# facebookresearch/robust_cvd

Hardware: AMD Instinct MI355X
Metric: GN/LM iterations/sec (and ms/iter) on 300-frame 384x224 video, 1/2/4/8 GPU (higher is better)
Workload: dtype f64

## Files before the change

include/cvd_hip_debug.h:

```cpp
#ifndef CVD_HIP_DEBUG_H
#define CVD_HIP_DEBUG_H

#include "cvd_hip.h"

#ifdef __cplusplus
extern "C" {
#endif

typedef struct cvd_debug_options {
  uint64_t struct_size;
  int32_t force_iterations;
  int32_t force_sharded_path;
  int32_t pcg_lockstep;
  int32_t stall_fused_tail_once;
  int32_t tail_no_row_staging;
} cvd_debug_options;
void cvd_debug_options_default(cvd_debug_options* o);
int32_t cvd_set_debug_options(cvd_handle* h, const cvd_debug_options* o);

int32_t cvd_set_generic_kernels(cvd_handle* h, int32_t enabled);

int32_t cvd_comm_init_local_group(cvd_handle* h, int32_t rank, int32_t world, uint64_t group_key);
int32_t cvd_comm_init_phantom(cvd_handle* h, int32_t rank, int32_t world);

int32_t cvd_block_inverse_debug(cvd_handle* h, int32_t num_blocks, int32_t block_size, const double* a, int32_t variant,
                                float* inverse, int32_t* failed);

int32_t cvd_epipolar_debug(cvd_handle* h, int32_t num_pairs, const int64_t* offsets, const float* loc, double pixel_scale,
                           double threshold_px, int32_t iterations, uint64_t seed, uint8_t* is_static_out,
                           double* fundamental_out, int32_t* best_out, int32_t* counts_out, double* hypotheses_out);
int32_t cvd_flow_masks_debug(cvd_handle* h, int32_t num_frames, int32_t height, int32_t width, int32_t channels,
                             const float* color, int32_t num_pairs, const int32_t* pair_frames, const float* flow_ab,
                             const float* flow_ba, float flow_thresh, float color_thresh, uint8_t* mask_ab, uint8_t* mask_ba,
                             int32_t* kept, float* errors, double* kernel_ms, int32_t pixels_per_thread);
int32_t cvd_dense_inverse_debug(cvd_handle* h, int32_t n, const double* a, double* inverse, int32_t* failed);
int32_t cvd_coarse_debug(cvd_handle* h, int32_t* num_unknowns, double* a_c, double* a_c_inverse, int32_t* failed);
int32_t cvd_temporal_debug(cvd_handle* h, int32_t* dims6, double* a_t, double* a_t_inverse, double* lam, int32_t* failed);
int32_t cvd_product_launch_debug(cvd_handle* h, int32_t* out6);
int32_t cvd_assembly_launch_debug(cvd_handle* h, int32_t* out6, double* cost_frame);

#ifdef __cplusplus
}
#endif
#endif
```

robust_cvd_amd/api.py:

```python
import ctypes as C
import os
import sys

from . import build as _build
from .binding import Binding
from .ctypes_types import OptParams, SolveSummary, XformDesc

_lib = None
_variant = None


class SolverOptions(C.Structure):
    _fields_ = [
        ("struct_size", C.c_uint64),
        ("pcg_relative_tolerance", C.c_double),
        ("pcg_max_iterations", C.c_int32),
        ("verbose", C.c_int32),
        ("coarse_level", C.c_int32),
        ("robust_loss", C.c_int32),
        ("dense_matrix_free", C.c_int32),
        ("block_inverse_variant", C.c_int32),
        ("coarse_dense_max_unknowns", C.c_int32),
        ("coarse_rebuild_excess", C.c_int32),
        ("coarse_update_budget", C.c_int64),
        ("coarse_dense_shift", C.c_double),
        ("constraint_order", C.c_int32),
        ("coarse_rebuild_excess_dense", C.c_int32),
        ("pcg_fused_tail", C.c_int32),
        ("coarse_dense_row_split", C.c_int32),
        ("dist_owner_update", C.c_int32),
        ("temporal_level", C.c_int32),
        ("temporal_step", C.c_int32),
        ("temporal_grid_x", C.c_int32),
        ("temporal_grid_y", C.c_int32),
        ("coarse_temporal_step", C.c_int32),
        ("coarse_over_budget", C.c_int32),
        ("coarse_temporal_min_frames", C.c_int32),
        ("temporal_weight", C.c_double),
    ]


class DebugOptions(C.Structure):
    _fields_ = [
        ("struct_size", C.c_uint64),
        ("force_iterations", C.c_int32),
        ("force_sharded_path", C.c_int32),
        ("pcg_lockstep", C.c_int32),
        ("stall_fused_tail_once", C.c_int32),
        ("tail_no_row_staging", C.c_int32),
    ]


class ConsistencyDesc(C.Structure):
    _fields_ = [
        ("struct_size", C.c_uint64),
        ("precision", C.c_int32),
        ("num_frames", C.c_int32),
        ("num_pairs", C.c_int32),
        ("height", C.c_int32),
        ("width", C.c_int32),
        ("distance_type", C.c_int32),
        ("have_warp", C.c_int32),
        ("reserved", C.c_int32),
        ("lambda_reprojection", C.c_double),
        ("lambda_disparity", C.c_double),
        ("lambda_depth_ratio", C.c_double),
        ("distance_scale", C.c_double),
        ("distance_alpha", C.c_double),
    ]


class SceneFlowDesc(C.Structure):
    _fields_ = [
        ("struct_size", C.c_uint64),
        ("precision", C.c_int32),
        ("num_frames", C.c_int32),
        ("num_pairs", C.c_int32),
        ("height", C.c_int32),
        ("width", C.c_int32),
        ("distance_type_static", C.c_int32),
        ("distance_type_smooth", C.c_int32),
        ("have_warp", C.c_int32),
        ("lambda_static", C.c_double),
        ("lambda_smooth_reprojection", C.c_double),
        ("lambda_smooth_disparity", C.c_double),
        ("lambda_smooth_depth_ratio", C.c_double),
        ("distance_scale", C.c_double),
        ("distance_alpha", C.c_double),
    ]


class SpatialDesc(C.Structure):
    _fields_ = [
        ("struct_size", C.c_uint64),
        ("precision", C.c_int32),
        ("num_frames", C.c_int32),
        ("frames_per_sample", C.c_int32),
        ("height", C.c_int32),
        ("width", C.c_int32),
        ("reserved", C.c_int32),
        ("lambda_disparity_smooth", C.c_double),
        ("sigma_color_grad", C.c_double),
        ("lambda_contrast_loss", C.c_double),
        ("contrast_thresh", C.c_double),
    ]


class ParamDesc(C.Structure):
    _fields_ = [
        ("struct_size", C.c_uint64),
        ("precision", C.c_int32),
        ("num_tensors", C.c_int32),
    ]


class ParamRecord(C.Structure):
    _fields_ = [
        ("beta1", C.c_double),
        ("beta2", C.c_double),
        ("eps", C.c_double),
        ("grad_decay", C.c_double),
        ("param_decay", C.c_double),
        ("step", C.c_double),
        ("denom_scale", C.c_double),
        ("rule", C.c_int32),
        ("reserved", C.c_int32),
    ]


class DatasetDesc(C.Structure):
    _fields_ = [
        ("struct_size", C.c_uint64),
# ... 1416 lines not shown
        with _DeviceArrays() as dev:
            dx, dw2, db2, dw4, db4 = (dev.upload(np.ascontiguousarray(v)) for v in arrays)
            do = dev.alloc(out.nbytes)
            self._check(self._fn("midas_head_device")(
                self._h, C.c_int32(B), C.c_int32(H), C.c_int32(W), C.c_int32(Cin), C.c_int32(MIDAS_HEAD_MID), dx, dw2, db2, dw4, db4,
                C.c_int32(1 if non_negative else 0), do, None))
            if _hip_runtime().hipDeviceSynchronize() != 0:
                raise RuntimeError("midas_head: the device reported an error")
            dev.download(do, out)
        return out

    def midas_decoder(self, maps, weights, biases, non_negative=True, kernel_ms=None):
        import numpy as np
        maps = [np.asarray(v) for v in maps]
        weights, biases = [np.asarray(v) for v in weights], [np.asarray(v) for v in biases]
        self._midas_f32("midas_decoder", maps + weights + biases)
        B, features, channels, heights, widths = midas_check_decoder([v.shape for v in maps], [v.shape for v in weights],
                                                                     [v.shape for v in biases])
        out = np.zeros((B, 4 * heights[0], 4 * widths[0]), np.float32)
        with _DeviceArrays() as dev:
            dm = (C.c_void_p * 4)(*[dev.upload(np.ascontiguousarray(v)).value for v in maps])
            dw = (C.c_void_p * 21)(*[dev.upload(np.ascontiguousarray(v)).value for v in weights])
            db = (C.c_void_p * 17)(*[dev.upload(np.ascontiguousarray(v)).value for v in biases])
            do = dev.alloc(out.nbytes)
            args = (self._h, C.c_int32(B), C.c_int32(features), (C.c_int32 * 4)(*channels), (C.c_int32 * 4)(*heights),
                    (C.c_int32 * 4)(*widths), dm, dw, db, C.c_int32(1 if non_negative else 0), do, None)
            if kernel_ms is None:
                self._check(self._fn("midas_decoder_device")(*args))
            else:
                ms = (C.c_double * MIDAS_TIMED_SLOTS)()
                self._check(self._fn("midas_decoder_timed")(*args, ms))
                kernel_ms[:] = list(ms)
            if _hip_runtime().hipDeviceSynchronize() != 0:
                raise RuntimeError("midas_decoder: the device reported an error")
            dev.download(do, out)
        return out

    def num_active_constraints(self):
        return int(self._lib.cvd_num_active_constraints(self._h))

    def block_inverse_debug(self, blocks, variant=0):
        import numpy as np
        a = np.ascontiguousarray(blocks, dtype=np.float64)
        n, B, B2 = a.shape
        assert B == B2
        out = np.zeros((n, B, B), dtype=np.float32)
        fl = C.c_int32(0)
        self._check(self._fn("block_inverse_debug")(self._h, C.c_int32(n), C.c_int32(B), a.ctypes.data_as(C.POINTER(C.c_double)),
                                                    C.c_int32(variant), out.ctypes.data_as(C.POINTER(C.c_float)), C.byref(fl)))
        return out, fl.value

    def dense_inverse_debug(self, a):
        import numpy as np
        a = np.ascontiguousarray(a, dtype=np.float64)
        n = a.shape[0]
        assert a.shape == (n, n)
        out = np.zeros((n, n), dtype=np.float64)
        fl = C.c_int32(0)
        self._check(self._fn("dense_inverse_debug")(self._h, C.c_int32(n), a.ctypes.data_as(C.POINTER(C.c_double)),
                                                    out.ctypes.data_as(C.POINTER(C.c_double)), C.byref(fl)))
        return out, fl.value

    def temporal_debug(self):
        import numpy as np
        dims = (C.c_int32 * 6)()
        self._check(self._fn("temporal_debug")(self._h, dims, None, None, None, None))
        if dims[0] == 0:
            return None
        n = dims[0]
        a = np.zeros((n, n))
        ai = np.zeros((n, n))
        lam = np.zeros(self.num_frames * self.block_size())
        fl = C.c_int32(0)
        dp = lambda x: x.ctypes.data_as(C.POINTER(C.c_double))
        self._check(self._fn("temporal_debug")(self._h, dims, dp(a), dp(ai), dp(lam), C.byref(fl)))
        return {"NT": n, "S": dims[1], "nn": dims[2], "step": dims[3], "Sx": dims[4], "Sy": dims[5], "a_t": a, "a_t_inverse": ai,
                "lam": lam, "failed": fl.value}

    def path_info(self):
        out = (C.c_int32 * 8)()
        self._check(self._fn("path_info")(self._h, out))
        form = {-1: "none", 0: "exact sparse factor", 1: "exact dense inverse", 2: "temporal pose level"}[out[1]]
        return {"pose_graph_level": form, "depth_grid_level": bool(out[2]), "fused_tail": bool(out[3] & 1), "tail_rows_staged": bool(out[3] & 2),
                "tail_disabled": bool(out[4]),
                "taps": out[5], "work_items": out[6], "cross_blocks": bool(out[7])}

    def product_launch_debug(self):
        out = (C.c_int32 * 6)()
        self._check(self._fn("product_launch_debug")(self._h, out))
        kind = {-1: "none", 0: "generic list", 1: "fast list", 2: "fast dense", 3: "cross blocks"}[out[3]]
        return {"threads": out[0], "spec": out[1], "kd": out[2], "kind": out[3], "kind_name": kind, "work_items": out[4],
                "num_cu": out[5]}

    def assembly_launch_debug(self):
        import numpy as np
        out = (C.c_int32 * 6)()
        cost = np.zeros(self.num_frames, dtype=np.float64)
        self._check(self._fn("assembly_launch_debug")(self._h, out, cost.ctypes.data_as(C.POINTER(C.c_double))))
        kind = {-1: "none", 0: "generic", 1: "fast list", 2: "fast dense", 3: "dense fold"}[out[3]]
        return {"threads": out[0], "spec": out[1], "kd": out[2], "kind": out[3], "kind_name": kind, "workgroups": out[4],
                "split_parts": out[5], "cost_frame": cost}

    def coarse_debug(self):
        import numpy as np
        n = C.c_int32(0)
        self._check(self._fn("coarse_debug")(self._h, C.byref(n), None, None, None))
        if n.value == 0:
            return None
        a = np.zeros((n.value, n.value))
        ai = np.zeros((n.value, n.value))
        fl = C.c_int32(0)
        self._check(self._fn("coarse_debug")(self._h, C.byref(n), a.ctypes.data_as(C.POINTER(C.c_double)),
                                             ai.ctypes.data_as(C.POINTER(C.c_double)), C.byref(fl)))
        return {"a_c": a, "a_c_inverse": ai, "failed": fl.value}
```

robust_cvd_amd/csrc/cvd_api.hip:

```cpp
#include "cvd_host.h"
#include "cvd_coarse.h"

namespace cvd {

static void poseOptimizationStep(cvd_handle* h, const cvd_opt_params& p, double depthDeformReg) {
  solve(h, p, depthDeformReg, PK_POSE_STEP);
  paramsToPoses(h, p);
}

static void poseOptimization(cvd_handle* h, const cvd_opt_params& p) {
  posesToParams(h);
  h->records.clear();
  int ctfRows = p.ctf_long, ctfCols = p.ctf_short;
  int dsoRows = p.dso_long, dsoCols = p.dso_short;
  if (h->aspect >= 1.f) {
    std::swap(ctfCols, ctfRows);
    std::swap(dsoCols, dsoRows);
  }
  int initGrid[3] = {1, 1, 1};
  if (h->ddesc.depth_type == CVD_DEPTH_GRID)
    for (int i = 0; i < 3; ++i) initGrid[i] = h->ddesc.grid_size[i];
  const int Nval = (h->ddesc.depth_type == CVD_DEPTH_IDENTITY) ? 0 : valueNumParams(h->ddesc.value_xform);
  size_t nDmax = static_cast<size_t>(h->nD());
  if (p.coarse_to_fine && h->ddesc.depth_type != CVD_DEPTH_IDENTITY && p.num_steps > 1)
// ... 172 lines not shown
  p->depth_deform_reg_initial = 1.0;
  p->depth_deform_reg_final = 0.1;
  p->spatial_deform_reg = 1.0;
  p->focal_reg = 1.0;
  p->coarse_to_fine = 1;
  p->ctf_long = 17;
  p->ctf_short = 10;
  p->dso_long = 4;
  p->dso_short = 3;
  p->focal_long = 0.3461538376301239;
  p->intr_opt = CVD_INTR_PER_FRAME;
  p->normalize_depth_from_first_frame = 1;
}

void cvd_solver_options_default(cvd_solver_options* o) {
  o->struct_size = CVD_STRUCT_STAMP(cvd_solver_options);
  o->pcg_relative_tolerance = 1e-3;
  o->pcg_max_iterations = 300;
  o->verbose = 0;
  o->coarse_level = 1;
  o->robust_loss = 0;
  o->dense_matrix_free = 0;
  o->block_inverse_variant = 0;
  o->coarse_dense_max_unknowns = 4096;
  o->coarse_rebuild_excess = 16;
  o->coarse_update_budget = 40000;
  o->coarse_dense_shift = 1e-5;
  o->constraint_order = 1;
  o->coarse_rebuild_excess_dense = 0;
  o->pcg_fused_tail = 1;
  o->coarse_dense_row_split = 5;
  o->dist_owner_update = 1;
  o->temporal_level = 1;
  o->temporal_step = 32;
  o->temporal_grid_x = 0;
  o->temporal_grid_y = 0;
  o->coarse_temporal_step = 8;
  o->coarse_over_budget = 0;
  o->coarse_temporal_min_frames = 128;
  o->temporal_weight = 0.7;
}
int32_t cvd_set_solver_options(cvd_handle* h, const cvd_solver_options* o) {
  CVD_TRY(h, {
    if (o->struct_size != CVD_STRUCT_STAMP(cvd_solver_options))
      throw std::runtime_error(fmt("cvd_solver_options: struct_size %#llx != %#llx = sizeof | revision << 32 (caller built against "
                                   "another cvd_hip.h; start from cvd_solver_options_default)",
                                   static_cast<unsigned long long>(o->struct_size),
                                   static_cast<unsigned long long>(CVD_STRUCT_STAMP(cvd_solver_options))));
    if (o->pcg_fused_tail < 0 || o->pcg_fused_tail > 1) throw std::runtime_error("pcg_fused_tail in {0, 1}");
    if (!(o->pcg_relative_tolerance > 0.0 && o->pcg_relative_tolerance < 1.0)) throw std::runtime_error("pcg_relative_tolerance must lie in (0, 1)");
    if (o->pcg_max_iterations < 1) throw std::runtime_error("pcg_max_iterations must be >= 1");
    if (!(o->coarse_dense_shift >= 0.0 && o->coarse_dense_shift < 1.0)) throw std::runtime_error("coarse_dense_shift must lie in [0, 1)");
    if (o->coarse_rebuild_excess < 0 || o->coarse_rebuild_excess_dense < -1 || o->coarse_update_budget < 0)
      throw std::runtime_error("coarse_rebuild_excess / coarse_update_budget must be >= 0, coarse_rebuild_excess_dense >= -1");
    if (o->coarse_dense_max_unknowns < 0 || o->coarse_dense_max_unknowns > kDenseCoarseMaxUnknowns)
      throw std::runtime_error(fmt("coarse_dense_max_unknowns must lie in [0, %d] (what k_dense_spd_inverse holds in registers)",
                                   kDenseCoarseMaxUnknowns));
    if (o->coarse_level < 0 || o->coarse_level > 3 || o->coarse_temporal_step < 2 || o->robust_loss < 0 || o->robust_loss > 1 || o->block_inverse_variant < 0 ||
        o->block_inverse_variant > 2)
      throw std::runtime_error("coarse_level in {0, 1, 2, 3}, coarse_temporal_step >= 2, robust_loss in {0, 1}, block_inverse_variant in {0, 1, 2}");
    if (o->coarse_over_budget < 0 || o->coarse_over_budget > 1) throw std::runtime_error("coarse_over_budget in {0, 1}");
    if (o->coarse_temporal_min_frames < 0) throw std::runtime_error("coarse_temporal_min_frames must be >= 0");
    if (!(o->temporal_weight > 0.0 && o->temporal_weight <= 2.0)) throw std::runtime_error("temporal_weight must lie in (0, 2]");
    if (o->coarse_dense_row_split < 0 || o->coarse_dense_row_split > 8) throw std::runtime_error("coarse_dense_row_split must lie in [0, 8]");
    if (o->temporal_level < 0 || o->temporal_level > 2 || o->temporal_step < 2 || o->temporal_grid_x < 0 || o->temporal_grid_y < 0 ||
        o->temporal_grid_x == 1 || o->temporal_grid_y == 1)
      throw std::runtime_error("temporal_level in {0, 1, 2}, temporal_step >= 2, temporal_grid_x / _y 0 (automatic) or >= 2");
    if (o->coarse_update_budget != h->opt.coarse_update_budget || o->coarse_dense_max_unknowns != h->opt.coarse_dense_max_unknowns ||
        (o->coarse_level == 3) != (h->opt.coarse_level == 3) || o->coarse_temporal_step != h->opt.coarse_temporal_step ||
        o->coarse_over_budget != h->opt.coarse_over_budget || o->coarse_temporal_min_frames != h->opt.coarse_temporal_min_frames ||
        o->pcg_fused_tail != h->opt.pcg_fused_tail)
      h->tableValid = false;
    if (o->constraint_order != h->opt.constraint_order) h->orderGx = h->orderGy = -1;
    h->opt = *o;
  });
}
void cvd_debug_options_default(cvd_debug_options* o) {
  o->struct_size = CVD_STRUCT_STAMP(cvd_debug_options);
  o->force_iterations = 0;
  o->force_sharded_path = 0;
  o->pcg_lockstep = 0;
  o->stall_fused_tail_once = 0;
  o->tail_no_row_staging = 0;
}
int32_t cvd_set_debug_options(cvd_handle* h, const cvd_debug_options* o) {
  CVD_TRY(h, {
    if (o->struct_size != CVD_STRUCT_STAMP(cvd_debug_options))
      throw std::runtime_error("cvd_debug_options: struct_size does not match this library's cvd_hip_debug.h (start from cvd_debug_options_default)");
    h->dbg = *o;
    h->distForced = h->world == 1 && (h->comm != nullptr || h->localGroup || h->phantom) && o->force_sharded_path != 0;
  });
}
void cvd_comm_unique_id(uint8_t* out128) {
  ncclUniqueId id;
  std::memset(&id, 0, sizeof(id));
  (void)ncclGetUniqueId(&id);
  std::memcpy(out128, &id, sizeof(id));
}
int32_t cvd_comm_init(cvd_handle* h, int32_t rank, int32_t world, const uint8_t* id128) {
  CVD_TRY(h, {
    if (world < 1 || rank < 0 || rank >= world) throw std::runtime_error("invalid rank / world size");
    if (h->comm) { NCCL_CHECK(ncclCommDestroy(h->comm)); h->comm = nullptr; }
    ncclUniqueId id;
    std::memcpy(&id, id128, sizeof(id));
    NCCL_CHECK(ncclCommInitRank(&h->comm, world, id, rank));
    h->rank = rank;
    h->world = world;
    h->localGroup.reset();
    h->distForced = world == 1 && h->dbg.force_sharded_path != 0;
    h->tableValid = false;
  });
}
int32_t cvd_comm_init_local_group(cvd_handle* h, int32_t rank, int32_t world, uint64_t group_key) {
  CVD_TRY(h, {
    if (world < 1 || rank < 0 || rank >= world) throw std::runtime_error("invalid rank / world size");
    if (h->comm) { NCCL_CHECK(ncclCommDestroy(h->comm)); h->comm = nullptr; }
    h->localGroup = joinLocalGroup(group_key, world);
    h->rank = rank;
    h->world = world;
    h->distForced = world == 1 && h->dbg.force_sharded_path != 0;
    h->tableValid = false;
  });
}
int32_t cvd_comm_init_phantom(cvd_handle* h, int32_t rank, int32_t world) {
  CVD_TRY(h, {
    if (world < 1 || rank < 0 || rank >= world) throw std::runtime_error("invalid rank / world size");
    if (h->comm) { NCCL_CHECK(ncclCommDestroy(h->comm)); h->comm = nullptr; }
    if (h->localGroup) { leaveLocalGroup(*h->localGroup); h->localGroup.reset(); }
    h->phantom = true;
    h->rank = rank;
    h->world = world;
    h->distForced = world == 1;
    h->tableValid = false;
  });
}
int32_t cvd_set_generic_kernels(cvd_handle* h, int32_t enabled) { CVD_TRY(h, h->forceGeneric = enabled != 0); }

int32_t cvd_set_video(cvd_handle* h, int32_t numFrames, int32_t width, int32_t height, float aspect, float invAspect) {
  CVD_TRY(h, {
    if (numFrames <= 0 || width <= 0 || height <= 0) throw std::runtime_error("invalid video dimensions");
    h->F = numFrames; h->W = width; h->H = height; h->aspect = aspect; h->invAspect = invAspect;
    h->haveDynMasks = false;
    h->adaptGx = h->adaptGy = 0;
    h->dDepth.ensure(static_cast<size_t>(numFrames) * width * height);
    HIP_CHECK(hipMemsetAsync(h->dDepth.p, 0, static_cast<size_t>(numFrames) * width * height * sizeof(float), h->stream));
    h->median.assign(numFrames, 0.f);
    h->medianDirty = true;
    h->poses.assign(numFrames, cvd_frame_pose{{0, 0, 0}, {0, 0, 0, 1}, 0.f, 0.f});
    h->poseParamsValid = false;
    cvd_xform_desc dd{};
    dd.type = CVD_XFORM_DEPTH;
    dd.depth_type = CVD_DEPTH_IDENTITY;
    cvd_xform_desc sd{};
    sd.type = CVD_XFORM_SPATIAL;
    sd.spatial_type = CVD_SPATIAL_IDENTITY;
    resetXforms(h, dd, false);
    resetXforms(h, sd, true);
    h->tableValid = false;
    h->P = 0;
    h->C = 0;
    h->dense = false;
    h->denseListValid = false;
    h->haveTriplets = false;
    h->tripCenter.clear();
    h->tripOff.clear();
    h->tripC = 0;
// ... 596 lines not shown
    if (num_blocks <= 0 || block_size <= 0 || block_size > kMaxFrameBlock) throw std::runtime_error("block_inverse_debug: bad sizes");
    if (variant < 0 || variant > 2) throw std::runtime_error("block_inverse_debug: variant must be 0, 1 or 2");
    const size_t n = static_cast<size_t>(num_blocks) * block_size * block_size;
    DevBuf<double> dA;
    DevBuf<double> dL;
    DevBuf<float> dM;
    DevBuf<int> dF;
    dA.ensure(n);
    dL.ensure(static_cast<size_t>(num_blocks) * block_size);
    dM.ensure(n);
    dF.ensure(1);
    hipStream_t s = h->stream;
    dA.upload(a, n, s);
    HIP_CHECK(hipMemsetAsync(dL.p, 0, static_cast<size_t>(num_blocks) * block_size * sizeof(double), s));
    HIP_CHECK(hipMemsetAsync(dM.p, 0, n * sizeof(float), s));
    HIP_CHECK(hipMemsetAsync(dF.p, 0, sizeof(int), s));
    Layout L{};
    L.F = num_blocks;
    L.B = block_size;
    launchBlockInverseRaw(h, L, dA.p, dL.p, dM.p, dF.p, variant);
    int fl = 0;
    dM.download(inverse, n, s);
    dF.download(&fl, 1, s);
    HIP_CHECK(hipStreamSynchronize(s));
    if (failed) *failed = fl;
  });
}

int32_t cvd_epipolar_debug(cvd_handle* h, int32_t num_pairs, const int64_t* offsets, const float* loc, double pixel_scale,
                           double threshold_px, int32_t iterations, uint64_t seed, uint8_t* is_static_out,
                           double* fundamental_out, int32_t* best_out, int32_t* counts_out, double* hypotheses_out) {
  CVD_TRY(h, epipolarStaticFlags(h, num_pairs, offsets, loc, pixel_scale, threshold_px, iterations, seed, is_static_out,
                                 fundamental_out, best_out, nullptr, counts_out, hypotheses_out));
}

int32_t cvd_dense_inverse_debug(cvd_handle* h, int32_t n, const double* a, double* inverse, int32_t* failed) {
  CVD_TRY(h, {
    if (n <= 0 || n > 8192) throw std::runtime_error("dense_inverse_debug: bad size");
    const size_t nn = static_cast<size_t>(n) * n;
    DevBuf<double> dA;
    DevBuf<double> dM;
    DevBuf<int> dF;
    dA.ensure(nn);
    dM.ensure(nn);
    dF.ensure(2);
    hipStream_t s = h->stream;
    dA.upload(a, nn, s);
    HIP_CHECK(hipMemsetAsync(dM.p, 0, nn * sizeof(double), s));
    HIP_CHECK(hipMemsetAsync(dF.p, 0, 2 * sizeof(int), s));
    launchDenseSpdInverse(h, n, dA.p, dM.p, dF.p, s, dF.p + 1);
    int fl[2] = {0, 0};
    dM.download(inverse, nn, s);
    dF.download(fl, 2, s);
    HIP_CHECK(hipStreamSynchronize(s));
    if (failed) *failed = fl[0];
  });
}

int32_t cvd_temporal_debug(cvd_handle* h, int32_t* dims6, double* a_t, double* a_t_inverse, double* lam, int32_t* failed) {
  CVD_TRY(h, {
    auto& T = h->temporal;
    hipStream_t s = h->stream;
    const bool on = T.on && T.built;
    const int dims[6] = {on ? T.NT : 0, T.S, T.nn, T.step, T.Sx, T.Sy};
    for (int i = 0; i < 6; ++i) dims6[i] = dims[i];
    if (on) {
      const size_t n2 = static_cast<size_t>(T.NT) * T.NT;
      if (a_t) T.A.download(a_t, n2, s);
      if (a_t_inverse) T.Ainv.download(a_t_inverse, n2, s);
      if (lam) h->dLam.download(lam, static_cast<size_t>(h->F) * h->Bsz(), s);
      int fl = 0;
      T.fail.download(&fl, 1, s);
      HIP_CHECK(hipStreamSynchronize(s));
      if (failed) *failed = fl;
    }
  });
}
int32_t cvd_path_info(cvd_handle* h, int32_t* out8) {
  CVD_TRY(h, {
    out8[0] = h->coarseOn ? 1 : 0;
    out8[1] = !h->coarseOn ? -1 : (h->coarse.temporalPose ? 2 : (h->coarse.denseMode ? 1 : 0));
    out8[2] = h->temporal.on ? 1 : 0;
    out8[3] = h->lastFusedTail ? (h->tailStageRows ? 3 : 1) : 0;
    out8[4] = h->tailDisabled ? 1 : 0;
    out8[5] = h->lastKD;
    out8[6] = static_cast<int32_t>(h->itemFa.size());
    out8[7] = h->lastCross ? 1 : 0;
  });
}
int32_t cvd_product_launch_debug(cvd_handle* h, int32_t* out6) {
  CVD_TRY(h, {
    for (int i = 0; i < 6; ++i) out6[i] = h->lastProduct[i];
  });
}
int32_t cvd_assembly_launch_debug(cvd_handle* h, int32_t* out6, double* cost_frame) {
  CVD_TRY(h, {
    for (int i = 0; i < 6; ++i) out6[i] = h->lastAssembly[i];
    const size_t F = static_cast<size_t>(h->F);
    if (cost_frame && h->lastAssembly[3] >= 0 && h->dCostFrame.n >= F) {
      h->dCostFrame.download(cost_frame, F, h->stream);
      HIP_CHECK(hipStreamSynchronize(h->stream));
    }
  });
}
int32_t cvd_coarse_debug(cvd_handle* h, int32_t* num_unknowns, double* a_c, double* a_c_inverse, int32_t* failed) {
  CVD_TRY(h, {
    auto& C = h->coarse;
    if (!C.valid || !h->coarseOn) {
      *num_unknowns = 0;
    } else if (C.temporalPose) {
      const size_t n = static_cast<size_t>(C.ptN);
      *num_unknowns = static_cast<int32_t>(n);
      hipStream_t s = h->stream;
      int fl = 0;
      C.fail.download(&fl, 1, s);
      if (a_c) C.ptMat.download(a_c, n * n, s);
      if (a_c_inverse) C.ptInv.download(a_c_inverse, n * n, s);
      HIP_CHECK(hipStreamSynchronize(s));
      if (failed) *failed = fl;
    } else {
      const int F = h->F;
      const size_t n = static_cast<size_t>(F) * kCB;
      *num_unknowns = static_cast<int32_t>(n);
      hipStream_t s = h->stream;
      int fl = 0;
      C.fail.download(&fl, 1, s);
      if (a_c_inverse) {
        std::vector<double> save(n), unit(n, 0.0);
        C.rc.download(save.data(), n, s);
        HIP_CHECK(hipStreamSynchronize(s));
        DevBuf<double> scalTmp;
        scalTmp.ensure(S_COUNT);
        HIP_CHECK(hipMemsetAsync(scalTmp.p, 0, S_COUNT * sizeof(double), s));
        for (size_t k = 0; k < n; ++k) {
          unit[k] = 1.0;
          C.rc.upload(unit.data(), n, s);
          if (C.denseMode) {
            hipLaunchKernelGGL(k_coarse_dense_apply, dim3(F), dim3(256), 0, s, F, C.denseInv.p, C.rc.p, C.c.p, C.modeActive.p,
                               C.dotPart.p, scalTmp.p, h->dCounters.p + 3, C.fail.p, 1, 0.0, static_cast<double*>(nullptr));
          } else {
            hipLaunchKernelGGL(k_coarse_apply_w, dim3(F), dim3(1024), 0, s, C.plan, C.Wb.p, C.rc.p, C.y.p, C.dotPart.p,
                               scalTmp.p, h->dCounters.p + 3, C.fail.p, 1, 0.0, static_cast<double*>(nullptr));
            hipLaunchKernelGGL(k_coarse_apply_wt, dim3(F), dim3(256), 0, s, coarseView(h, true, true), F, C.c.p,
                               scalTmp.p, 1);
          }
          C.c.download(a_c_inverse + k * n, n, s);
          HIP_CHECK(hipStreamSynchronize(s));
          unit[k] = 0.0;
        }
        C.rc.upload(save.data(), n, s);
        HIP_CHECK(hipStreamSynchronize(s));
      }
      std::vector<double> diag(static_cast<size_t>(F) * kCBB), edges(static_cast<size_t>(std::max(C.nEdges, 1)) * kCBB);
      std::vector<unsigned char> act(n);
      std::vector<int> efa(C.nEdges), efb(C.nEdges);
      C.diag.download(diag.data(), diag.size(), s);
      C.edges.download(edges.data(), static_cast<size_t>(C.nEdges) * kCBB, s);
      C.modeActive.download(act.data(), n, s);
      C.edgeFa.download(efa.data(), efa.size(), s);
      C.edgeFb.download(efb.data(), efb.size(), s);
      HIP_CHECK(hipStreamSynchronize(s));
      if (failed) *failed = fl;
      if (a_c) {
        std::fill(a_c, a_c + n * n, 0.0);
        for (int f = 0; f < F; ++f)
          for (int i = 0; i < kCB; ++i)
// ... 16 lines not shown
```

robust_cvd_amd/csrc/cvd_host.h:

```cpp
#pragma once

#include <hip/hip_runtime.h>
#include <hip/hip_ext.h>
#include <rccl/rccl.h>
#include <rocblas/rocblas.h>
#include <rocsolver/rocsolver.h>

#include <algorithm>
#include <array>
#include <atomic>
#include <chrono>
#include <condition_variable>
#include <cmath>
#include <cstdarg>
#include <cstdint>
#include <cstdio>
#include <cstdlib>
#include <cstring>
#include <functional>
#include <limits>
#include <map>
#include <memory>
#include <mutex>
#include <set>
// ... 242 lines not shown
  DevBuf<double> dStatPart;
  DevBuf<unsigned char> dDynMask;
  DevBuf<double> dAdaptW;
  int dynW = 0, dynH = 0, adaptGx = 0, adaptGy = 0;
  bool haveDynMasks = false;
  std::shared_ptr<Frontend> frontend;

  struct CoarseHost {
    bool valid = false;
    int nEdges = 0, nBlocks = 0, nLevels = 0;
    std::vector<int> itemEdge;
    DevBuf<int> order, pos, levelPtr, levelCols, lvlBlkPtr, lvlBlks, blkCol, blkRow, colPtr, rowPtr, rowBlk, updPtr, updBlk,
        updA, updB, edgeBlk, edgeFa, edgeFb, wPtr, wRow, wtPtr, wtBlk, wtCol, wtFrame, wuPtr, wuL, wuW, itemEdgeDev, wSlot;
    DevBuf<double> edges, diag, Lb, Linv, Wb, rc, qc, y, c, dotPart, fdotY, wq, dropDiag;
    bool sparsified = false;
    bool temporalPose = false;
    int ptNn = 0, ptStepFrames = 0, ptN = 0, ptBlocks = 0;
    std::vector<int> edgeFaHost, edgeFbHost;
    DevBuf<int> ptA, ptB, ptPtr, ptList;
    DevBuf<double> ptMat, ptInv, ptR, ptT, ptDot, ptRec;
    DevBuf<TlStep> ptStepDev;
    std::vector<unsigned char> ptStepHost;
    DevBuf<unsigned int> ptCounter;
    bool denseMode = false;
    int denseForB = 0;
    bool denseReady = false;
    DevBuf<double> denseA, densePanel;
    DevBuf<double> denseInv;
    DevBuf<int> denseValid;
    int nW = 0;
    DevBuf<unsigned char> modeActive;
    DevBuf<int> fail;
    DevBuf<unsigned int> barrier;
    bool ptInvPending = false;
    int* ptInvFail = nullptr;
    DevBuf<double> Wb2;
    DevBuf<int> fail2;
    CoarsePlan plan{};
  } coarse;
  bool coarseOn = false;
  struct TemporalHost {
    bool on = false;
    bool built = false;
    int S = 0, Sx = 0, Sy = 0, nn = 0, step = 0, NT = 0, width = 0, nGroups = 0, nBlocks = 0;
    std::vector<unsigned char> stepHost;
    int tabGx = 0, tabGy = 0, tabSx = 0, tabSy = 0;
    int grpF = 0, grpStep = 0;
    std::vector<int> grpFa, grpFb;
    DevBuf<float> hx, hy, elW;
    DevBuf<int> bx, by, gOff, gItems, blkA, blkB, gPtr, gather, fail, valid;
    DevBuf<float4> vW;
    DevBuf<unsigned int> vIdx, counter;
    DevBuf<unsigned char> elV;
    DevBuf<double> Cf, E, part, A, Ainv, sq, rT, t, tl, dotPart, rec;
    DevBuf<double> invPanel;
    DevBuf<unsigned int> invBarrier;
    DevBuf<TlStep> stepDev;
    hipEvent_t evIn = nullptr, evDone = nullptr;
    bool sidePending = false;
    double* sqPtr = nullptr;
  } temporal;
  hipEvent_t evRebuild[2] = {nullptr, nullptr};
  bool rebuildTimed = false;
  double coarseRebuildMs = 0.0, pcgIterMs = 0.0;
  std::vector<std::pair<int, int>> globalEdges;
  bool haveGlobalEdges = false;
  DevBuf<double> dRegJac;
  DevBuf<unsigned short> dRegCol;
  DevBuf<unsigned char> dRegCnt;
  RegCache regCache{};
  DevBuf<FrameConst> dFc;
  DevBuf<int> dFail;
  DevBuf<unsigned long long> dCount;
  double* hScal = nullptr;
  double* hStage[2] = {nullptr, nullptr};
  size_t hStageN[2] = {0, 0};
  double* hPcg = nullptr;
  hipEvent_t pcgEvent[2] = {nullptr, nullptr};

  cvd_solve_summary summary{};
  std::vector<cvd_iteration_record> records;

  bool lastFusedTail = false, lastCross = false;
  bool tailStageRows = false;
  int lastKD = 0;
  int lastProduct[6] = {0, 0, 0, -1, 0, 0};
  int lastAssembly[6] = {0, 0, 0, -1, 0, 0};
  bool tailDisabled = false;
  bool forceGeneric = false;

  int timing = 0;
  int timingStride = 1;
  long long timingCounter = 0;
  long long timingCounterKc[16] = {0};
  std::vector<std::pair<hipEvent_t, hipEvent_t>> evPool;
  std::vector<int> evClass;
  std::vector<int> evIter;
  int curPcgIter = -1;
  size_t evUsed = 0;
  double kcMs[KC_TOTAL] = {0};
  long long kcN[KC_TOTAL] = {0};

  ~cvd_handle_t() {
    for (auto& e : evPool) { (void)hipEventDestroy(e.first); (void)hipEventDestroy(e.second); }
    if (rbMain) (void)rocblas_destroy_handle(rbMain);
    if (comm) (void)ncclCommDestroy(comm);
    if (localGroup) leaveLocalGroup(*localGroup);
    if (hScal) (void)hipHostFree(hScal);
    for (auto& p : hStage) if (p) (void)hipHostFree(p);
    if (hPcg) (void)hipHostFree(hPcg);
    for (auto& e : pcgEvent) if (e) (void)hipEventDestroy(e);
    for (auto& e : evRebuild) if (e) (void)hipEventDestroy(e);
    if (temporal.evIn) (void)hipEventDestroy(temporal.evIn);
    if (temporal.evDone) (void)hipEventDestroy(temporal.evDone);
    if (evCoarseIn) (void)hipEventDestroy(evCoarseIn);
    if (evCoarseDone) (void)hipEventDestroy(evCoarseDone);
    if (evInvIn) (void)hipEventDestroy(evInvIn);
    if (evInvDone) (void)hipEventDestroy(evInvDone);
    if (stream3) (void)hipStreamDestroy(stream3);
    if (stream2) (void)hipStreamDestroy(stream2);
    if (stream) (void)hipStreamDestroy(stream);
  }

  int nD() const { return xformNumBlocks(ddesc) * xformBlockSize(ddesc); }
  int nS() const { return xformNumBlocks(sdesc) * xformBlockSize(sdesc); }
  int Bsz() const { return 7 + nD() + nS(); }

  int tBegin(int kc) {
    if (kc >= KC_COUNT ? timing == 0 : !(timing & (1 << kc))) return -1;
    if (timingStride > 1 && kc < KC_DENSE_WALK && (timingCounterKc[kc]++ % timingStride) != 0) return -1;
    if (evUsed == evPool.size()) {
      hipEvent_t a, b;
      HIP_CHECK(hipEventCreate(&a));
      HIP_CHECK(hipEventCreate(&b));
      evPool.emplace_back(a, b);
      evClass.push_back(kc);
      evIter.push_back(-1);
    }
    evClass[evUsed] = kc;
    evIter[evUsed] = curPcgIter;
    HIP_CHECK(hipEventRecord(evPool[evUsed].first, stream));
    return static_cast<int>(evUsed++);
  }
  void tEnd(int slot) {
    if (slot >= 0) HIP_CHECK(hipEventRecord(evPool[slot].second, stream));
  }
  int tReserve(int kc, hipEvent_t& start, hipEvent_t& stop) {
    start = nullptr;
    stop = nullptr;
    if (!(timing & (1 << kc))) return -1;
    if (timingStride > 1 && (timingCounter++ % timingStride) != 0) return -1;
    if (evUsed == evPool.size()) {
      hipEvent_t a, b;
      HIP_CHECK(hipEventCreate(&a));
      HIP_CHECK(hipEventCreate(&b));
      evPool.emplace_back(a, b);
      evClass.push_back(kc);
      evIter.push_back(-1);
    }
    evClass[evUsed] = kc;
    evIter[evUsed] = curPcgIter;
    start = evPool[evUsed].first;
    stop = evPool[evUsed].second;
    return static_cast<int>(evUsed++);
  }
  void tDropFrom(size_t firstSlot, int firstDeadIter) {
// ... 91 lines not shown
    } catch (...) {
      sl.m.unlock();
      throw;
    }
  }
  ~PersistentGate() {
    sl.recorded = hipEventRecord(sl.ev, s) == hipSuccess;
    sl.m.unlock();
  }
};

void commAllReduce(cvd_handle* h, void* buf, size_t count, CommType t, hipStream_t s);
void commReduceScatter(cvd_handle* h, const void* send, void* recv, size_t recvCount, CommType t, hipStream_t s);
void commAllGather(cvd_handle* h, const void* send, void* recv, size_t sendCount, CommType t, hipStream_t s);
void commGroupStart(cvd_handle* h);
void commGroupEnd(cvd_handle* h);
std::vector<int> rangeOf(const cvd_opt_params& p, int F);
void posesToParams(cvd_handle* h);
void paramsToPoses(cvd_handle* h, const cvd_opt_params& params);
void resetXforms(cvd_handle* h, const cvd_xform_desc& d, bool spatial);
void gridXformSplit(cvd_handle* h, const cvd_xform_desc& nd);
Layout makeLayout(cvd_handle* h, const cvd_opt_params& p, double depthDeformReg, ProblemKind kind);
void checkFrameBlock(size_t B, const char* what);
void tapCounts(const Layout& L, int& KD, int& KS);
bool fastLoss(const Layout& L);
Table makeTable(cvd_handle* h);
void checkDenseScope(cvd_handle* h, const Layout& L, int KS, bool trip);
bool denseFastScope(const cvd_handle* h, const Layout& L, int KS, bool trip);
bool denseFastBlockFits(long long B);
struct DenseListScope {
  cvd_handle* h;
  bool entered = false;
  DenseListScope(cvd_handle* h, bool needList);
  ~DenseListScope();
};
bool denseModeSupported(const cvd_opt_params& p, const cvd_xform_desc& dd, const cvd_xform_desc& sd, bool haveTriplets, int world,
                        bool normalize);
AsmPanels makePanels(int B, size_t capDoubles, int& panelCap);
void compileTable(cvd_handle* h, const std::vector<int>& range, bool withTriplets = false, bool ignoreStatic = false);
void orderTable(cvd_handle* h, const Layout& L, int KD);
double* pinnedStage(cvd_handle* h, int which, size_t n);
void uploadState(cvd_handle* h, const Layout& L, DevBuf<double>& dst);
void downloadState(cvd_handle* h, const Layout& L, const DevBuf<double>& src);
void buildMask(cvd_handle* h, const Layout& L, const cvd_opt_params& p, ProblemKind kind, const std::vector<int>& range);
void ensureBuffers(Ctx& c);
void refreshMedians(cvd_handle* h);
void launchFrameConsts(const Layout& L, const double* x, FrameConst* fc, hipStream_t s);
void launchFrameConsts(Ctx& c, const double* x);
void launchFlagToBool(int* flag, hipStream_t s);
void launchTlRowsInit(cvd_handle* h, const TlStep* tsp, int NT, int groups, int F, unsigned int* counter, int closeScalars, double tol2,
                      hipStream_t s);
void spinStream(hipStream_t s);
void spinEvent(hipEvent_t ev);
void readScalars(Ctx& c);
void enqueueCost(Ctx& c, const double* x);
double evalCost(Ctx& c, const double* x);
void enqueueStats(Ctx& c);
bool crossScope(cvd_handle* h, const Ctx& c);
CrossPairs crossPairs(cvd_handle* h);
void launchCrossAssemble(Ctx& c, const double* x);
double evalFull(Ctx& c, const double* x, bool withStats = false, bool noReadBack = false);
bool coarseFusedConsumers();
bool fusedExchange(cvd_handle* h, bool withCoarse);
size_t exchangeOffsetQc(const Ctx& c);
size_t exchangeOffsetPq(const Ctx& c, bool withDenseCoarse);
size_t exchangeTemporalCount(cvd_handle* h, bool withCoarse);
bool ownerShardedUpdate(cvd_handle* h, bool withCoarse);
inline int denseRowSplit(const cvd_handle* h) { return std::min(kCB, std::max(0, h->opt.coarse_dense_row_split)); }
void launchDenseSpdInverse(cvd_handle* h, int n, const double* A, double* out, int* fail, hipStream_t s, int* outValid,
                           DevBuf<double>* panelBuf = nullptr, DevBuf<unsigned int>* barrierBuf = nullptr);
struct DinvRequest {
  int n = 0;
  const double* A = nullptr;
  double* out = nullptr;
  int* fail = nullptr;
  int* outValid = nullptr;
  DevBuf<double>* panelBuf = nullptr;
  DevBuf<unsigned int>* barrierBuf = nullptr;
};
void launchDenseSpdInversePair(cvd_handle* h, const DinvRequest& a, const DinvRequest& b, hipStream_t s);
CoarseView coarseView(cvd_handle* h, bool on, bool walk);
void prepareMatvec(Ctx& c, const double* x);
void launchMatvec(Ctx& c, const double* x, const double* z, const double* pOld, double* pNew, int useBeta, const double* lam,
                  double* q, bool withCoarse = false, bool tailFused = false);
bool pcgTailScope(Ctx& c, bool coarse, int nThreads, size_t& lds, int& ldsFinish, int& ldsScratch);
void launchPcgTail(Ctx& c, const double* x, const double* pOld, double* pNew, int useBeta, const double* lam, double* q,
                   bool withCoarse, int nThreads, size_t lds, int ldsFinish, int ldsScratch, double tol2);
void launchBlockInverseRaw(cvd_handle* h, const Layout& L, const double* dH, const double* dLam, float* dMinv, int* dFail, int variant,
                           hipStream_t onStream = nullptr);
void launchBlockInverse(Ctx& c, hipStream_t onStream = nullptr);
void launchCoarseSetup(Ctx& c, const double* x, int side = 0);
bool temporalScope(const Ctx& c);
bool temporalPrepare(Ctx& c);
void launchTemporalSetup(Ctx& c, const double* x, int half);
void launchTemporalInit(Ctx& c, bool closeScalars, double tol2);
TlStep temporalStep(cvd_handle* h);
const TlStep* temporalStepDev(cvd_handle* h);
void poseTemporalPlan(cvd_handle* h);
void poseTemporalPrepare(Ctx& c);
void launchPoseTemporalBuild(Ctx& c, hipStream_t s, int* failOut, bool deferInverse = false);
void launchPoseTemporalInit(Ctx& c, double tol2);
const TlStep* poseTemporalStepDev(cvd_handle* h);
void coarseDebug(cvd_handle* h, int32_t* num_unknowns, double* a_c, double* a_c_inverse, int32_t* failed);
int runPcg(Ctx& c, const double* x, const std::function<void()>& tail = nullptr);
bool wantsTriplets(const cvd_opt_params& p, ProblemKind kind);
void bindTriplets(Ctx& c, const cvd_opt_params& p, ProblemKind kind);
void solve(cvd_handle* h, const cvd_opt_params& p, double depthDeformReg, ProblemKind kind);
void evaluate(cvd_handle* h, const cvd_opt_params& p, double depthDeformReg, const double* pose7, double* cost, int32_t* nres,
              double* gradient, double* hdiag, double* hfull);
void sampleConstraints(cvd_handle* h, bool triplet, int num, const int32_t* keyFrames, const float* corner, const float* flow,
                       const uint8_t* mask, const float* flow2, const uint8_t* mask2, const float* dyn, int dw, int dh,
                       int matchSeparation, float minDynamicDistance, int64_t* offsets);
void getSampledConstraints(cvd_handle* h, bool triplet, float* out);
void denseMaps(cvd_handle* h, int kind, int first, int count, int w, int hh, void* out, double* kernelMs);
void imageOps(cvd_handle* h, int kind, int n, int w, int hh, const void* in, float* out, double* kernelMs);
void touchModule_setup();
void touchModule_eval();
void touchModule_matvec();
void touchModule_precond();
void touchModule_solve();
void touchModule_frontend();
void touchModule_temporal();
void flowGuidedFilter(cvd_handle* h, int n, int first, int count, int w, int hh, int dw, int dh, float invAspect, const float* depth,
                      const float* cameras, const float* flowF, const uint8_t* maskF, const float* flowB, const uint8_t* maskB,
                      int frameRadius, int spatialRadius, int median, float* out, double* kernelMs);
void bilateralFilter(cvd_handle* h, int n, int first, int count, int w, int hh, const float* depth, const float* color,
                     int frameRadius, int spatialRadius, float depthSigma, float colorSigma, int median, float* out,
                     double* kernelMs);
void epipolarStaticFlags(cvd_handle* h, int numPairs, const int64_t* offsets, const float* loc, double pixelScale,
                         double thresholdPx, int iterations, uint64_t seed, uint8_t* isStatic, double* fundamental,
                         int32_t* best, double* kernelMs, int32_t* counts, double* hypotheses);
void computeTracks(cvd_handle* h, int F, int H, int W, float invAspect, const uint8_t* active, int first, int last,
                   const float* corner, const float* dyn, int dh, int dw, const float* flow, const uint8_t* mask,
                   const uint8_t* pairPresent, int spawnDistance, int pruneDistance, float minDynamicDistance,
                   int minTrackLength, int64_t* counts, double* kernelMs);
void getTracks(cvd_handle* h, int32_t* startFrame, int32_t* length, uint8_t* kept, float* loc);
void flowConsistencyMasks(cvd_handle* h, int numFrames, int hh, int w, int channels, const float* color, int numPairs,
                          const int32_t* pairFrames, const float* flowAB, const float* flowBA, float flowThresh,
                          float colorThresh, uint8_t* maskAB, uint8_t* maskBA, int32_t* kept, float* errors, double* kernelMs,
                          int pixelsPerThread);
void consistencyLoss(cvd_handle* h, const cvd_consistency_desc* d, const void* depth, const void* ext, const void* intr,
                     const void* warp, const int32_t* pairFrames, const void* flowAB, const void* flowBA, const void* weightAB,
                     const void* weightBA, double* total, double* terms, void* grad, double* kernelMs);
void consistencyLossDevice(cvd_handle* h, const cvd_consistency_desc* d, const void* depth, const void* ext, const void* intr,
                           const void* warp, const int32_t* pairFrames, const void* flowAB, const void* flowBA,
                           const void* weightAB, const void* weightBA, double* total, double* terms, void* grad, hipStream_t s);
void sceneFlowLoss(cvd_handle* h, const cvd_scene_flow_desc* d, const void* depth, const void* ext, const void* intr,
                   const void* warp, const int32_t* pairFrames, const void* const* flows, const void* const* masks,
                   const int32_t* neighborFrames, const void* const* nflows, const void* const* nmasks, const void* valid,
                   double* total, double* terms, void* grad, void* maps, double* kernelMs);
void sceneFlowLossDevice(cvd_handle* h, const cvd_scene_flow_desc* d, const void* depth, const void* ext, const void* intr,
                         const void* warp, const int32_t* pairFrames, const void* const* flows, const void* const* masks,
                         const int32_t* neighborFrames, const void* const* nflows, const void* const* nmasks, const void* valid,
                         double* total, double* terms, void* grad, void* maps, hipStream_t s);
void spatialLosses(cvd_handle* h, const cvd_spatial_desc* d, const void* depth, const void* depthOrig, const void* image,
                   double* total, double* smooth, double* contrast, void* grad, double* kernelMs);
void spatialLossesDevice(cvd_handle* h, const cvd_spatial_desc* d, const void* depth, const void* depthOrig, const void* image,
                         double* total, double* smooth, double* contrast, void* grad, hipStream_t s);
void parameterL1(cvd_handle* h, const cvd_param_desc* d, const int64_t* offsets, const int64_t* counts, int64_t flatCount,
                 const void* p, const void* p0, double lambda, double* total, void* grad, double gradOut, int accumulate,
                 double* kernelMs);
void parameterL1Device(cvd_handle* h, const cvd_param_desc* d, const void* const* p, const void* const* p0, const int64_t* counts,
                       double lambda, double* total, void* const* grad, const void* gradOut, int accumulate, hipStream_t s);
void paramStep(cvd_handle* h, const cvd_param_desc* d, const int64_t* offsets, const int64_t* counts, int64_t flatCount, void* p,
               const void* g, void* m, void* v, const cvd_param_record* records, double* kernelMs);
void paramStepDevice(cvd_handle* h, const cvd_param_desc* d, void* const* p, const void* const* g, void* const* m, void* const* v,
                     const int64_t* counts, const cvd_param_record* records, hipStream_t s);
long long paramChunkElements();
void datasetCreate(cvd_handle* h, const cvd_dataset_desc* d, const int32_t* pairFrames, const int32_t* samples);
void datasetClear(cvd_handle* h);
// ... 44 lines not shown
```

robust_cvd_amd/csrc/cvd_kernels.h:

```cpp
#pragma once

#include "cvd_device.h"

namespace cvd {

struct Table {
  const float4* ndc;
  const float2* dsrc;
  const int* pairA;
  const int* pairB;
  const long long* pairOff;
  const float2* flow;
  const unsigned char* fmask;
  const float* depth;
  int W, H;
  float sx, sy, invAspect;
};

__device__ __forceinline__ int densePixelOfLoc(const Table& T, float lx, float ly) {
  int px = static_cast<int>(__fmul_rn(lx, static_cast<float>(T.W)));
  int py = static_cast<int>(__fmul_rn(__fdiv_rn(ly, T.invAspect), static_cast<float>(T.H)));
  px = min(max(px, 0), T.W - 1);
  py = min(max(py, 0), T.H - 1);
  return py * T.W + px;
// ... 95 lines not shown
  bool candCur;
  __device__ __forceinline__ bool request(const Table& T, int pix, int fa, int fb, float2 f, float4& n, float2& d) const {
    return denseConstraintRequest(T, pix, fa, fb, f, n, d);
  }
  __device__ __forceinline__ void prime(const Table& T, long long base, int i, int step, int n, long long pixBase, int fa, int fb) {
    unsigned int m0 = 0u;
    float2 f0 = make_float2(0.f, 0.f);
    fNext = make_float2(0.f, 0.f);
    mNext = 0u;
    if (i < n) { m0 = (T.fmask + base)[i]; f0 = (T.flow + base)[i]; }
    if (i + step < n) { mNext = (T.fmask + base)[i + step]; fNext = (T.flow + base)[i + step]; }
    ndCur = make_float4(0.f, 0.f, 0.f, 0.f);
    candCur = m0 != 0u && request(T, static_cast<int>(base - pixBase) + i, fa, fb, f0, ndCur, dCur);
  }
  __device__ __forceinline__ bool take(const Table& T, long long base, int i, int step, int n, long long pixBase, int fa, int fb,
                                       float4& nd, float2& d) {
    nd = ndCur;
    d = dCur;
    const bool cand = candCur;
    const unsigned int m1 = mNext;
    const float2 f1 = fNext;
    mNext = 0u;
    if (i + 2 * step < n) { mNext = (T.fmask + base)[i + 2 * step]; fNext = (T.flow + base)[i + 2 * step]; }
    candCur = m1 != 0u && request(T, static_cast<int>(base - pixBase) + i + step, fa, fb, f1, ndCur, dCur);
    return cand && denseDepthsValid(d);
  }
};

struct alignas(64) ItemRecord {
  int fa, fb;
  int slotA, slotB;
  long long b0, e0;
  long long b1, e1;
  long long pad[2];
};
static_assert(sizeof(ItemRecord) == 64, "one record per 64-byte line");
struct Items {
  const int* fa;
  const int* fb;
  const long long* range;
  const int* slot;
  int count;
  const ItemRecord* rec;
};

constexpr int kDenseFramesPerGroup = 2;
constexpr int kAsmUnit = 128;
constexpr int kAsmUnitDense = 1024;
constexpr int kDenseRun = 16;

#ifndef CVD_DETERMINISTIC
#define CVD_DETERMINISTIC 0
#endif
constexpr int kAtomicWalkers256 = CVD_DETERMINISTIC ? 64 : 256;
constexpr int kAsmThreads = CVD_DETERMINISTIC ? 64 : 512;
struct AsmPart {
  int frame;
  int u0, u1;
  int part;
  int nParts;
  int slot0;
};
struct AsmWork {
  const AsmPart* parts;
  const int2* units;
  double* scratch;
  unsigned int* counters;
};

__host__ __device__ inline int dwRecordDoubles(int G) { return 256 + 40 * G + 8; }
struct DenseRecords {
  const double* records;
  const int* recOff;
  const int* fpOff;
  const int* fpList;
};

enum : int { S_RZ = 0, S_RZOLD = 1, S_BETA = 2, S_PQ = 3, S_ALPHA = 4, S_RR = 5, S_RZ0 = 6, S_COST = 7,
             S_DG = 8, S_DR = 9, S_DLD = 10, S_DD = 11, S_XX = 12, S_NVALID = 13, S_GMAX = 14,
             S_DONE = 15, S_TARGET = 16, S_ITERS = 17,
             S_RZPART = 18,
             S_NACTIVE = 19,
             S_COUNT = 20 };

__device__ __forceinline__ double blockSumArray(const double* __restrict__ a, int n, double* red) {
  double acc = 0.0;
  for (int i = threadIdx.x; i < n; i += blockDim.x) acc += a[i];
  acc = waveSum(acc);
  __syncthreads();
  if ((threadIdx.x & 63) == 0) red[threadIdx.x >> 6] = acc;
  __syncthreads();
  double t = 0.0;
  for (int w = 0; w < (blockDim.x >> 6); ++w) t += red[w];
  __syncthreads();
  return t;
}

__device__ __forceinline__ bool lastBlockArrives(unsigned int* counter, unsigned int total, int* flag) {
  __syncthreads();
  if (threadIdx.x == 0) {
    __builtin_amdgcn_fence(__ATOMIC_RELEASE, "agent");
    asm volatile("s_waitcnt vmcnt(0)" ::: "memory");
    const unsigned int t = __hip_atomic_fetch_add(counter, 1u, __ATOMIC_RELAXED, __HIP_MEMORY_SCOPE_AGENT);
    const bool last = (t == total - 1);
    if (last) {
      __builtin_amdgcn_fence(__ATOMIC_ACQUIRE, "agent");
      __hip_atomic_store(counter, 0u, __ATOMIC_RELAXED, __HIP_MEMORY_SCOPE_AGENT);
    }
    *flag = last ? 1 : 0;
  }
  __syncthreads();
  return *flag != 0;
}

#if defined(__HIP_DEVICE_COMPILE__) && !defined(__gfx950__) && !defined(__gfx942__)
#error "the fence-free inter-workgroup hand-off (publishPartial / readPartial / lastBlockArrivesLite) is written for gfx942 / gfx950"
#endif
__device__ __forceinline__ void publishPartial(double* p, double v) {
  __hip_atomic_store(reinterpret_cast<unsigned long long*>(p), static_cast<unsigned long long>(__double_as_longlong(v)),
                     __ATOMIC_RELAXED, __HIP_MEMORY_SCOPE_AGENT);
}
__device__ __forceinline__ double readPartial(const double* p) {
  return __longlong_as_double(static_cast<long long>(__hip_atomic_load(
      reinterpret_cast<const unsigned long long*>(p), __ATOMIC_RELAXED, __HIP_MEMORY_SCOPE_AGENT)));
}
__device__ __forceinline__ bool lastBlockArrivesLite(unsigned int* counter, unsigned int total, int* flag) {
  asm volatile("s_waitcnt vmcnt(0)" ::: "memory");
  __syncthreads();
  if (threadIdx.x == 0) {
    const unsigned int t = __hip_atomic_fetch_add(counter, 1u, __ATOMIC_RELAXED, __HIP_MEMORY_SCOPE_AGENT);
    const bool last = (t == total - 1);
    if (last) __hip_atomic_store(counter, 0u, __ATOMIC_RELAXED, __HIP_MEMORY_SCOPE_AGENT);
    *flag = last ? 1 : 0;
  }
  __syncthreads();
  return *flag != 0;
}
__device__ __forceinline__ double blockSumPartials(const double* __restrict__ a, int n, double* red) {
  double acc = 0.0;
  for (int i = threadIdx.x; i < n; i += blockDim.x) acc += readPartial(a + i);
  acc = waveSum(acc);
  __syncthreads();
  if ((threadIdx.x & 63) == 0) red[threadIdx.x >> 6] = acc;
  __syncthreads();
  double t = 0.0;
  for (int w = 0; w < (blockDim.x >> 6); ++w) t += red[w];
  __syncthreads();
  return t;
}

constexpr size_t kCoarseMaxUnknowns = 65536;
constexpr int kCBB = kCB * kCB;
struct CoarsePlan {
  int F, nBlocks, nLevels, nEdges;
  const int* order;
  const int* pos;
  const int* levelPtr;
  const int* levelCols;
  const int* lvlBlkPtr;
  const int* lvlBlks;
  const int* blkCol;
  const int* blkRow;
  const int* colPtr;
  const int* rowPtr;
  const int* rowBlk;
  const int* updPtr;
// ... 298 lines not shown
                                        double (&Rca)[3]) {
  ca[0] = pax * fxa;
  ca[1] = pay * fya;
  ca[2] = -1.0;
  Rca[0] = dot3(Ra, ca);
  Rca[1] = dot3(Ra + 3, ca);
  Rca[2] = dot3(Ra + 6, ca);
}

template <bool FAST>
__device__ __forceinline__ void fastProject(const Layout& L, const double* Rb, const double (&v)[3], double ifxb, double ifyb,
                                            double pbx, double pby, double& zz, double& iz, double& u, double& vv, double& r0,
                                            double& r1) {
  const double q0 = Rb[0] * v[0] + Rb[3] * v[1] + Rb[6] * v[2];
  const double q1 = Rb[1] * v[0] + Rb[4] * v[1] + Rb[7] * v[2];
  const double q2 = Rb[2] * v[0] + Rb[5] * v[1] + Rb[8] * v[2];
  zz = -q2;
  iz = fastRcp<FAST>(zz);
  u = q0 * iz * ifxb;
  vv = q1 * iz * ifyb;
  r0 = (u - pbx) * L.ws;
  r1 = (vv - pby) * L.ws;
}

template <bool FAST>
__device__ __forceinline__ void fastDepthResidual(const Layout& L, int lossType, double zz, double iz, double Db, double& r2,
                                                  double& dr2dA, double& dr2dDb) {
  constexpr double eps = 1e-6;
  if (lossType == kLossDisparity) {
    const bool zo = !(zz < eps), bo = !(Db < eps);
    const double bc = bo ? Db : eps;
    const double izc = zo ? iz : 1.0 / eps, ibc = fastRcp<FAST>(bc);
    r2 = (izc - ibc) * L.wd;
    dr2dA = zo ? (-L.wd * izc * izc) : 0.0;
    dr2dDb = bo ? (L.wd * ibc * ibc) : 0.0;
  } else {
    const bool zIsMax = !(zz < Db), zIsMin = !(Db < zz);
    const double mx = zIsMax ? zz : Db, mn = zIsMin ? zz : Db;
    if (lossType == kLossRatio) {
      r2 = (mx / mn - 1.0) * L.wd;
      const double dmx = 1.0 / mn, dmn = -mx / (mn * mn);
      dr2dA = ((zIsMax ? dmx : 0.0) + (zIsMin ? dmn : 0.0)) * L.wd;
      dr2dDb = ((zIsMax ? 0.0 : dmx) + (zIsMin ? 0.0 : dmn)) * L.wd;
    } else {
      r2 = log(mn / mx) * L.wd;
      const double dmn = 1.0 / mn, dmx = -1.0 / mx;
      dr2dA = ((zIsMax ? dmx : 0.0) + (zIsMin ? dmn : 0.0)) * L.wd;
      dr2dDb = ((zIsMax ? 0.0 : dmx) + (zIsMin ? 0.0 : dmn)) * L.wd;
    }
  }
}

template <int SPEC>
__device__ __forceinline__ double fastRobustRho1(const Layout& L, double sq) {
  if constexpr (SPEC == 1) return rcpFast(1.0 + sq * L.cauchyC);
  else if constexpr (SPEC == 2) {
    const bool outer = sq > L.cauchyB;
    const double irt = rsqrtFast(outer ? sq : 1.0);
    return outer ? fmax(2.2250738585072014e-308, L.robustA * irt) : 1.0;
  }
  else return robustRho1(L, sq);
}
template <int SPEC>
__device__ __forceinline__ double fastRobustRho0(const Layout& L, double sq) {
  static_assert(SPEC == 1 || SPEC == 2, "the runtime choice goes through robustRho");
  if constexpr (SPEC == 1) {
    return L.cauchyB * log(1.0 + sq * L.cauchyC);
  } else {
    const bool outer = sq > L.cauchyB;
    const double irt = rsqrtFast(outer ? sq : 1.0);
    return outer ? (2.0 * L.robustA * (sq * irt) - L.cauchyB) : sq;
  }
}

__device__ __forceinline__ void fastRows(const Layout& L, double iz, double u, double vv, double ifxb, double ifyb, double& m00,
                                         double& m11, double& m02, double& m12) {
  const double wiz = L.ws * iz;
  m00 = wiz * ifxb;
  m11 = wiz * ifyb;
  m02 = wiz * u;
  m12 = wiz * vv;
}

#ifdef CVD_MV_PROFILE
__device__ unsigned long long g_mvProf[4096 * 8];
#define MV_STAMP(slot) do { if ((threadIdx.x & 63) == 0) g_mvProf[(blockIdx.x & 4095) * 8 + (slot)] = wall_clock64(); } while (0)
#else
#define MV_STAMP(slot) do {} while (0)
#endif
constexpr int kRedVals = 15;
constexpr int kRedStride = 4 * 33 + 1;

#ifndef CVD_MV_WAVES
#define CVD_MV_WAVES 4
#endif
#ifndef CVD_MV_EARLY
#define CVD_MV_EARLY 1
#endif
template <int KD, int NT, int SPEC = 0, bool DENSE = false>
inline __global__ __launch_bounds__(NT) __attribute__((amdgpu_waves_per_eu(SPEC ? ((KD <= 4 && !DENSE) ? CVD_MV_WAVES : 3) : 2))) void k_matvec_pairs_fast(Layout L, Table T, Items it, const double* __restrict__ x,
                                                           const FrameConst* __restrict__ fc,
                                                           const double* __restrict__ mask,
                                                           const double* __restrict__ z, const double* __restrict__ pOld,
                                                           const double* __restrict__ scal, int useBeta,
                                                           double* __restrict__ qPart, CoarseView V) {
  const double sDone = scal[S_DONE];
  extern __shared__ __attribute__((aligned(16))) double sm[];
  constexpr int NV = KD == 1 ? kRedVals : 11;
  const int B = L.B;
  if (threadIdx.x == 0) MV_STAMP(0);
  double* xa = sm;
  double* xb = xa + B;
  double* pa = xb + B;
  double* pb = pa + B;
  double* qa = pb + B;
  double* qb = qa + B;
  double* fix = qb + B;
  double* red = fix + 2 * sizeof(FrameConst) / 8;
  double* W = red + 32;
  constexpr int kPriv = DENSE ? 8 : 1;
  constexpr bool kUsePriv = kPriv > 1;
  double* qpriv = W + static_cast<size_t>(kRedVals) * kRedStride;
  double* cl = W;
  const int item = blockIdx.x;
  const int tid = threadIdx.x;
  const ItemRecord* __restrict__ recp = it.rec + item;
  const int fa = recp->fa, fb = recp->fb;
  const int slotA = recp->slotA, slotB = recp->slotB;
  const long long cbD[2] = {recp->b0, recp->b1}, ceD[2] = {recp->e0, recp->e1};
  const double beta = useBeta ? scal[S_BETA] : 0.0;
  const FrameConst* __restrict__ fcF[2] = {fc + fa, fc + fb};
  constexpr bool kEarlyPrime = KD <= 4 && CVD_MV_EARLY;
  RecordStream<DENSE> rs;
  if constexpr (kEarlyPrime) rs.primeClamped(T, cbD[0], tid, static_cast<int>(ceD[0] - cbD[0]));
  constexpr int EPT = 256 / NT;
  constexpr int TLE = (2 * kTlMaxS + NT - 1) / NT;
  const bool fusedCoarse = V.Wb != nullptr;
  const bool tlOn = V.tl != nullptr;
  const size_t rowA = static_cast<size_t>(fa) * B, rowB = static_cast<size_t>(fb) * B;
  double vcf;
  {
    const int k = tid & (2 * kCB - 1);
    vcf = *(V.cF != nullptr ? V.cF + static_cast<size_t>(k < kCB ? fa : fb) * kCB + (k & (kCB - 1)) : x);
  }
  double* tls = cl + 2 * kCB;
  double vtl[TLE];
#pragma unroll
  for (int e = 0; e < TLE; ++e) {
    const int i = tid + e * NT;
    const int ic = (tlOn && i < 2 * V.tlS) ? i : 0;
    const int which = ic >= V.tlS ? 1 : 0;
    vtl[e] = *(tlOn ? V.tl + static_cast<size_t>(which ? fb : fa) * V.tlS + (ic - which * V.tlS) : x);
  }
  TlTaps tt[EPT];
#pragma unroll
  for (int e = 0; e < EPT; ++e) {
    const int i = tid + e * NT;
    const bool in = i >= 7 && i < 7 + L.nD;
    const int v = in ? i - 7 : 0;
    tt[e].w = *(tlOn ? V.tlW + v : reinterpret_cast<const float4*>(x));
    tt[e].idx = *(tlOn ? V.tlIdx + v : reinterpret_cast<const unsigned int*>(x));
    if (!in) tt[e].w = make_float4(0.f, 0.f, 0.f, 0.f);
  }
  constexpr int kFix = 13;
  static_assert(offsetof(FrameConst, fy) == offsetof(FrameConst, t) + 24 && offsetof(FrameConst, Jl) == offsetof(FrameConst, t) + 32,
                "t, fy, Jl are consecutive");
  const int fixK = NT - 1 - tid;
  double vfix;
  {
    const int k = fixK < 2 * kFix ? fixK : 0;
    vfix = (reinterpret_cast<const double*>(fc + (k >= kFix ? fb : fa)) + offsetof(FrameConst, t) / 8)[k >= kFix ? k - kFix : k];
  }
  double vxa[EPT], vxb[EPT], vza[EPT], vzb[EPT], vpa[EPT], vpb[EPT], vma[EPT], vmb[EPT];
  const double* __restrict__ pOldOrZ = useBeta ? pOld : z;
#pragma unroll
  for (int e = 0; e < EPT; ++e) {
    const int i = tid + e * NT;
    const size_t ia = rowA + (i < B ? i : 0), ib = rowB + (i < B ? i : 0);
    vxa[e] = x[ia];
    vxb[e] = x[ib];
    vza[e] = z[ia];
    vzb[e] = z[ib];
    vpa[e] = pOldOrZ[ia];
    vpb[e] = pOldOrZ[ib];
    vma[e] = mask[ia];
    vmb[e] = mask[ib];
  }
  const double z6 = z[6], po6 = pOldOrZ[6], m6 = mask[6];
  if (fusedCoarse) {
    if (tid < 64) coarseFrameCorrection(V, fa, tid, cl);
    if (NT == 64) coarseFrameCorrection(V, fb, tid, cl + kCB);
    else if (tid >= 64 && tid < 128) coarseFrameCorrection(V, fb, tid - 64, cl + kCB);
  }
  if (!fusedCoarse && tid < 2 * kCB) cl[tid] = (V.cF != nullptr) ? vcf : 0.0;
#pragma unroll
  for (int e = 0; e < TLE; ++e) {
    const int i = tid + e * NT;
    if (tlOn && i < 2 * V.tlS) tls[i] = vtl[e];
  }
  if (fixK < 2 * kFix) fix[fixK] = vfix;
#pragma unroll
  for (int e = 0; e < EPT; ++e) {
    const int i = tid + e * NT;
    if (i < B) {
      xa[i] = vxa[e];
      xb[i] = vxb[e];
      qa[i] = 0.0;
      qb[i] = 0.0;
    }
  }
  if constexpr (kUsePriv)
    for (int i = tid; i < kPriv * 2 * B; i += NT) qpriv[i] = 0.0;
  __syncthreads();
  if (sDone != 0.0) return;
#pragma unroll
  for (int e = 0; e < EPT; ++e) {
    const int i = tid + e * NT;
    if (i < B) {
      double ca = coarseAtLds(cl, L, i), cb2 = coarseAtLds(cl + kCB, L, i);
      if (tlOn) {
        ca += tlAt(tls, tt[e]);
        cb2 += tlAt(tls + V.tlS, tt[e]);
      }
      pa[i] = (vza[e] + ca + (useBeta ? beta * vpa[e] : 0.0)) * vma[e];
      pb[i] = (vzb[e] + cb2 + (useBeta ? beta * vpb[e] : 0.0)) * vmb[e];
    }
  }
  if (L.intrOpt == kIntrShared) {
    __syncthreads();
    if (tid == 0) {
      const double p06 = (z6 + (useBeta ? beta * po6 : 0.0)) * m6;
      pa[6] = p06;
      pb[6] = p06;
    }
  }
  __syncthreads();
  if (threadIdx.x == 0) MV_STAMP(1);

  const int N = SPEC ? 1 : L.N;
  const int lossType = SPEC ? static_cast<int>(kLossDisparity) : L.lossType;
  const double A = L.aspect;
  double aT[3] = {0, 0, 0}, aT0[3] = {0, 0, 0};
  double Cx[3] = {0, 0, 0};
  double aFa = 0.0, aFb = 0.0;
  double gDa[2] = {0.0, 0.0}, gDb[2] = {0.0, 0.0};
  const long long units0 = (ceD[0] - cbD[0] + 63) >> 6;
  for (int dir = 0; dir < 2; ++dir) {
  const long long cb = cbD[dir], ce = ceD[dir];
  const FrameConst& Fa = *fcF[dir];
  const FrameConst& Fb = *fcF[dir ^ 1];
  if (dir) {
    double* t;
    t = xa; xa = xb; xb = t;
    t = pa; pa = pb; pb = t;
    t = qa; qa = qb; qb = t;
#pragma unroll
    for (int i = 0; i < 3; ++i) { aT0[i] = aT[i]; aT[i] = 0.0; Cx[i] = -Cx[i]; }
    { const double o = aFa; aFa = aFb; aFb = o; }
#pragma unroll
    for (int n = 0; n < 2; ++n) { const double o = gDa[n]; gDa[n] = gDb[n]; gDb[n] = o; }
  }
  const int firstUnit = dir == 0 ? (tid >> 6) : static_cast<int>(((tid >> 6) - units0) & (NT / 64 - 1));
  const int nDir = static_cast<int>(ce - cb);
  const int iFirst = firstUnit * 64 + (tid & 63);
  if (dir || !kEarlyPrime) rs.prime(T, cb, iFirst, nDir);
  double RaU[9], RbU[9], dTU[3];
#pragma unroll
  for (int i = 0; i < 9; ++i) { RaU[i] = uniformValue(Fa.R[i]); RbU[i] = uniformValue(Fb.R[i]); }
#pragma unroll
  for (int i = 0; i < 3; ++i) dTU[i] = uniformValue(Fa.t[i] - Fb.t[i]);
  double eaU[3], ebU[3], dptU[3];
  {
    const double pwa[3] = {uniformValue(pa[3]), uniformValue(pa[4]), uniformValue(pa[5])};
    const double pwb[3] = {uniformValue(pb[3]), uniformValue(pb[4]), uniformValue(pb[5])};
#pragma unroll
    for (int k = 0; k < 3; ++k) {
      eaU[k] = uniformValue(pwa[0] * Fa.Jl[k] + pwa[1] * Fa.Jl[3 + k] + pwa[2] * Fa.Jl[6 + k]);
      ebU[k] = uniformValue(pwb[0] * Fb.Jl[k] + pwb[1] * Fb.Jl[3 + k] + pwb[2] * Fb.Jl[6 + k]);
      dptU[k] = uniformValue(pa[k] - pb[k]);
    }
  }
  const double fya = uniformValue(Fa.fy), fxa = fya * A;
  const double fyb = uniformValue(Fb.fy);
  const double ifyb = uniformValue(1.0 / fyb), ifxb = uniformValue(1.0 / (fyb * A));
  const double pfaU = uniformValue(pa[6] / fya);
  const double pfrU = uniformValue(L.ws * pb[6] * ifyb);

  const int fsrc = dir ? fb : fa, ftgt = dir ? fa : fb;
  const long long pixBase = DENSE ? (cb / (static_cast<long long>(T.W) * T.H)) * (static_cast<long long>(T.W) * T.H) : 0;
  for (int ci = iFirst; ci < nDir; ci += NT) {
    float4 nd;
    float2 d;
    if (!rs.take(T, cb, ci, NT, nDir, pixBase, fsrc, ftgt, nd, d)) continue;
    const double da = static_cast<double>(d.x), db = static_cast<double>(d.y);
    FastTaps<KD> ta, tb;
    fastGather<KD>(L, nd.x, nd.y, ta);
    fastGather<KD>(L, nd.z, nd.w, tb);
// ... 197 lines not shown
```

robust_cvd_amd/csrc/cvd_matvec.hip:

```cpp
#include "cvd_host.h"
#include "cvd_pcg.h"
#include "cvd_cross.h"
#include "cvd_triplets.h"

namespace cvd {

bool coarseFusedConsumers() {
  return false;
}
bool fusedExchange(cvd_handle* h, bool withCoarse) { return !withCoarse || h->coarse.denseMode; }
size_t exchangeOffsetQc(const Ctx& c) { return c.h->dist() ? static_cast<size_t>(c.h->framesPadded()) * c.L.B : c.n; }
size_t exchangeOffsetPq(const Ctx& c, bool withDenseCoarse) {
  return exchangeOffsetQc(c) + (withDenseCoarse ? static_cast<size_t>(c.L.F) * kCB : 0);
}
size_t exchangeTemporalCount(cvd_handle* h, bool withCoarse) {
  const TlStep ts = temporalStep(h);
  return (ts.Ainv != nullptr && h->dist() && fusedExchange(h, withCoarse)) ? static_cast<size_t>(h->F) * ts.S : 0;
}
bool ownerShardedUpdate(cvd_handle* h, bool withCoarse) {
  return h->dist() && fusedExchange(h, withCoarse) && h->opt.dist_owner_update != 0;
}
CoarseView coarseView(cvd_handle* h, bool on, bool walk) {
  auto& C = h->coarse;
  CoarseView v = on ? CoarseView{C.pos.p, C.wPtr.p, C.wRow.p, walk ? C.Wb.p : nullptr, C.y.p, C.modeActive.p, C.fail.p, C.c.p}
                    : CoarseView{nullptr, nullptr, nullptr, nullptr, nullptr, nullptr, nullptr, nullptr};
  if (h->temporal.on && h->temporal.built) {
    v.tl = h->temporal.tl.p;
    v.tlW = h->temporal.vW.p;
    v.tlIdx = h->temporal.vIdx.p;
    v.tlS = h->temporal.S;
  }
  return v;
}

void prepareMatvec(Ctx& c, const double* x) {
  cvd_handle* h = c.h;
  const Layout& L = c.L;
  launchFrameConsts(c, x);
  int nr = 0;
  if (L.scaleRegSqrt > 0.0) nr += L.sregX * L.sregY;
  if (L.focalRegSqrt > 0.0) nr += 1;
  if (L.depthDeformW > 0.0 && L.depthType == CVD_DEPTH_GRID) nr += gridNumEdges(L.gx, L.gy, L.gz) * L.N;
  if (L.spatialDeformW > 0.0) nr += L.nS;
  const int stride = std::max(2, c.KD * std::max(1, L.N));
  const size_t entries = static_cast<size_t>(L.F) * stride * std::max(nr, 1);
  h->dRegJac.ensure(entries);
  h->dRegCol.ensure(entries);
  h->dRegCnt.ensure(static_cast<size_t>(L.F) * std::max(nr, 1));
  h->regCache = RegCache{h->dRegJac.p, h->dRegCol.p, h->dRegCnt.p, nr, stride};
  HIP_CHECK(hipMemsetAsync(h->dScal.p + S_DONE, 0, sizeof(double), h->stream));
  if (nr == 0) return;
  CVD_DISPATCH_KD(c.KD, {
    hipLaunchKernelGGL((k_reg_cache<KD>), dim3(L.F), dim3(256), static_cast<size_t>(L.B) * 8, h->stream, L, x, h->dMedian.p, h->dRegOwner.p,
                       h->regCache);
  });
  HIP_CHECK(hipGetLastError());
}

void launchMatvec(Ctx& c, const double* x, const double* z, const double* pOld, double* pNew, int useBeta,
                         const double* lam, double* q, bool withCoarse, bool tailFused) {
  cvd_handle* h = c.h;
  hipStream_t s = h->stream;
  const CoarseView cF = coarseView(h, withCoarse, coarseFusedConsumers());
  const size_t B = c.L.B;
  auto recordLaunch = [h](int threads, int spec, int kd, int kind, int items) {
    const int launched[6] = {threads, spec, kd, kind, items, h->numCU};
    std::copy(launched, launched + 6, h->lastProduct);
  };
  if (c.cross) {
    hipEvent_t evStart, evStop;
    (void)h->tReserve(KC_MATVEC_PAIRS, evStart, evStop);
    const size_t ldsX = (3 * B + (kCrossThreads / 64) * B + 2 * kCB + 2 * kTlMaxS) * 8;
    const unsigned nP = static_cast<unsigned>(h->xFa.size()) + (h->xDiagRows ? static_cast<unsigned>(c.L.F) : 0u);
    const int* diagSlot = h->xDiagRows ? h->dXDiagSlot.p : nullptr;
    recordLaunch(kCrossThreads, 0, c.KD, 3, static_cast<int>(nP));
    if (evStart)
      hipExtLaunchKernelGGL(k_cross_matvec, dim3(nP), dim3(kCrossThreads), ldsX, s, evStart, evStop, 0, c.L, crossPairs(h),
                            h->dXBlocks.p, h->dH.p, diagSlot, h->dMask.p, z, pOld, h->dScal.p, useBeta, h->dQPart.p, cF);
    else
      hipLaunchKernelGGL(k_cross_matvec, dim3(nP), dim3(kCrossThreads), ldsX, s, c.L, crossPairs(h), h->dXBlocks.p, h->dH.p, diagSlot,
                         h->dMask.p, z, pOld, h->dScal.p, useBeta, h->dQPart.p, cF);
    HIP_CHECK(hipGetLastError());
  } else if (c.L.includeStatic && c.nItems > 0) {
    const size_t lds = 6 * B * 8 + 2 * sizeof(FrameConst) + (18 + 4 * 24 + 8 + 2 * kCB) * 8;
    const size_t ldsFast = 6 * B * 8 + 2 * sizeof(FrameConst) + (32 + static_cast<size_t>(kRedVals) * kRedStride) * 8;
    hipEvent_t evStart, evStop;
    (void)h->tReserve(KC_MATVEC_PAIRS, evStart, evStop);
    const bool fast = !h->forceGeneric && c.KS == 0 && fastLoss(c.L);
    const FrameConst* fcp = h->dFc.p;
    const double* maskp = h->dMask.p;
    const double* scalp = h->dScal.p;
    if (fast) {
      const int spec = (c.L.N == 1 && c.L.lossType == CVD_STATIC_REPRO_DISPARITY) ? (c.L.robustKind == 0 ? 1 : 2) : 0;
      const int wavesPerSimd = spec ? ((c.KD <= 4) ? CVD_MV_WAVES : 3) : 2;
      const long long slots256 = static_cast<long long>(wavesPerSimd) * h->numCU;
      const long long slots128 = std::min<long long>(2 * slots256, static_cast<long long>(kMaxLds / std::max<size_t>(ldsFast, 1)) * h->numCU);
#ifndef CVD_MV_NT_RULE
#define CVD_MV_NT_RULE 1
#endif
      const int nt = CVD_MV_NT_RULE ? ((c.nItems <= slots256 || c.nItems > slots128) ? 256 : 128)
                                    : (c.nItems > 2 * h->numCU && c.nItems <= 4 * h->numCU ? 128 : 256);
#define CVD_LAUNCH_PAIRS_FAST_S(NTV, SPECV)                                                                              \
      CVD_DISPATCH_KD(c.KD, {                                                                                            \
        recordLaunch(NTV, SPECV, KD, 1, c.nItems);                                                                       \
        allowLds((k_matvec_pairs_fast<KD, NTV, SPECV>), ldsFast);                                                        \
        if (evStart)                                                                                                     \
          hipExtLaunchKernelGGL((k_matvec_pairs_fast<KD, NTV, SPECV>), dim3(c.nItems), dim3(NTV), ldsFast, s, evStart, evStop, 0, \
                                c.L, c.T, c.it, x, fcp, maskp, z, pOld, scalp, useBeta, h->dQPart.p, cF);                \
        else                                                                                                             \
          hipLaunchKernelGGL((k_matvec_pairs_fast<KD, NTV, SPECV>), dim3(c.nItems), dim3(NTV), ldsFast, s, c.L, c.T, c.it, x, \
                             fcp, maskp, z, pOld, scalp, useBeta, h->dQPart.p, cF);                                      \
      })
#define CVD_LAUNCH_PAIRS_FAST(NTV) do { if (spec == 1) CVD_LAUNCH_PAIRS_FAST_S(NTV, 1); else if (spec == 2) CVD_LAUNCH_PAIRS_FAST_S(NTV, 2); else CVD_LAUNCH_PAIRS_FAST_S(NTV, 0); } while (0)
      if (h->dense) {
        const size_t ldsDense = ldsFast + 8 * 2 * B * 8;
#define CVD_LAUNCH_PAIRS_DENSE(SPECV)                                                                                     \
        CVD_DISPATCH_KD(c.KD, {                                                                                          \
          if constexpr (KD <= 4) {                                          \
            recordLaunch(256, SPECV, KD, 2, c.nItems);                                                                   \
            allowLds((k_matvec_pairs_fast<KD, 256, SPECV, true>), ldsDense);                                             \
            if (evStart)                                                                                                 \
              hipExtLaunchKernelGGL((k_matvec_pairs_fast<KD, 256, SPECV, true>), dim3(c.nItems), dim3(256), ldsDense, s, evStart, \
                                    evStop, 0, c.L, c.T, c.it, x, fcp, maskp, z, pOld, scalp, useBeta, h->dQPart.p, cF); \
            else                                                                                                         \
              hipLaunchKernelGGL((k_matvec_pairs_fast<KD, 256, SPECV, true>), dim3(c.nItems), dim3(256), ldsDense, s, c.L, c.T, \
                                 c.it, x, fcp, maskp, z, pOld, scalp, useBeta, h->dQPart.p, cF);                         \
          }                                                                                                              \
        })
        if (spec == 1) CVD_LAUNCH_PAIRS_DENSE(1);
        else if (spec == 2) CVD_LAUNCH_PAIRS_DENSE(2);
        else CVD_LAUNCH_PAIRS_DENSE(0);
#undef CVD_LAUNCH_PAIRS_DENSE
      }
#if CVD_DETERMINISTIC
      else { (void)nt; CVD_LAUNCH_PAIRS_FAST(64); }
#else
      else if (nt == 128) CVD_LAUNCH_PAIRS_FAST(128);
      else CVD_LAUNCH_PAIRS_FAST(256);
#endif
#undef CVD_LAUNCH_PAIRS_FAST_S
#undef CVD_LAUNCH_PAIRS_FAST
    } else {
      recordLaunch(256, 0, c.KD, 0, c.nItems);
      CVD_DISPATCH(c.KD, c.KS, {
        allowLds(k_matvec_pairs<KD, KS>, lds);
        if (evStart)
          hipExtLaunchKernelGGL((k_matvec_pairs<KD, KS>), dim3(c.nItems), dim3(256), lds, s, evStart, evStop, 0, c.L, c.T,
                                c.it, x, fcp, maskp, z, pOld, scalp, useBeta, h->dQPart.p, cF);
        else
          hipLaunchKernelGGL((k_matvec_pairs<KD, KS>), dim3(c.nItems), dim3(256), lds, s, c.L, c.T, c.it, x, fcp, maskp, z,
                             pOld, scalp, useBeta, h->dQPart.p, cF);
      });
    }
    HIP_CHECK(hipGetLastError());
  }
  if (c.trip && c.TT.nGroups > 0) {
    const size_t ldsT = (9 * B + 3 * kCB) * 8;
    CVD_DISPATCH(c.KD, c.KS, {
      allowLds(k_matvec_triplets<KD, KS>, ldsT);
      hipLaunchKernelGGL((k_matvec_triplets<KD, KS>), dim3(c.TT.nGroups), dim3(256), ldsT, s, c.L, c.TT, x, h->dFc.p,
                         h->dMask.p, z, pOld, h->dScal.p, useBeta, h->dQPart.p, cF);
    });
    HIP_CHECK(hipGetLastError());
  }
  if (!tailFused) {
    if (B > 512) throw std::runtime_error("frame block larger than 512 unknowns is not supported by k_matvec_finish");
    const TlStep ts = temporalStep(h);
    const size_t lds = 3 * B * 8 + (8 + kCB) * 8 + (ts.Ainv != nullptr ? (kTlMaxS + static_cast<size_t>(ts.S) * ts.width) * 8 : 0);
    const bool fusedCoarse = withCoarse && !h->coarse.denseMode;
    const bool denseFused = withCoarse && h->coarse.denseMode;
    const bool fusedX = h->dist() && fusedExchange(h, withCoarse);
    double* qcX = q + exchangeOffsetQc(c);
    double* pqX = q + exchangeOffsetPq(c, denseFused);
    const CoarseColumns cc{h->coarse.pos.p, h->coarse.wPtr.p, h->coarse.wSlot.p, fusedCoarse ? h->coarse.Wb.p : nullptr,
                           h->coarse.wq.p};
    const int slot = h->tBegin(KC_MATVEC_FINISH);
    CVD_DISPATCH_KD(c.KD, {
      hipLaunchKernelGGL((k_matvec_finish<KD>), dim3(c.L.F), dim3(256), lds, s, c.L, x, h->dMask.p, lam,
                         h->dMedian.p, h->dRegOwner.p, h->dInRange.p, c.cross ? h->dXFiOff.p : h->dFiOff.p, h->dFiList.p,
                         h->dQPart.p, z, pOld, pNew, h->dScal.p, h->dCounters.p, useBeta, q, h->dFdot.p,
                         h->dist() ? (h->rank == 0 ? 1 : 2) : 0, c.cross ? static_cast<int>(h->xFa.size()) * 2 : h->qRows,
                         h->regCache, cF,
                         fusedX ? (denseFused ? qcX : nullptr) : (((fusedCoarse || denseFused) && !h->dist()) ? h->coarse.qc.p : nullptr), cc,
                         c.cross ? h->dH.p : nullptr, fusedX ? pqX : nullptr, h->dist() ? h->ownFirst() : 0,
                         h->dist() ? h->ownCount() : ((c.cross && h->xDiagRows) ? 0 : c.L.F), ts.Ainv != nullptr ? temporalStepDev(h) : static_cast<const TlStep*>(nullptr));
    });
    HIP_CHECK(hipGetLastError());
    if (fusedX && ownerShardedUpdate(h, withCoarse)) {
      const int ct = h->tBegin(KC_COMM_PRODUCT);
      const size_t chunk = static_cast<size_t>(h->ownChunk()) * B;
      commGroupStart(h);
      commReduceScatter(h, q, q + static_cast<size_t>(h->rank) * chunk, chunk, CT_F64, s);
      commAllReduce(h, qcX, exchangeOffsetPq(c, denseFused) - exchangeOffsetQc(c) + 1 + exchangeTemporalCount(h, withCoarse), CT_F64, s);
      commGroupEnd(h);
      h->tEnd(ct);
    } else if (fusedX) {
      const int ct = h->tBegin(KC_COMM_PRODUCT);
      commAllReduce(h, q, exchangeOffsetPq(c, denseFused) + 1 + exchangeTemporalCount(h, withCoarse), CT_F64, s);
      h->tEnd(ct);
    } else if (h->dist()) {
      const int ct = h->tBegin(KC_COMM_PRODUCT);
      commAllReduce(h, q, c.n, CT_F64, s);
      h->tEnd(ct);
      hipLaunchKernelGGL(k_dot_pq, dim3(c.L.F), dim3(256), 0, s, c.L, pNew, q, h->dScal.p, h->dCounters.p, h->dFdot.p,
                         withCoarse ? h->coarse.qc.p : nullptr, h->coarse.modeActive.p, cc,
                         ts.Ainv != nullptr ? temporalStepDev(h) : static_cast<const TlStep*>(nullptr));
      HIP_CHECK(hipGetLastError());
    }
    h->tEnd(slot);
  }
}

bool pcgTailScope(Ctx& c, bool coarse, int nThreads, size_t& lds, int& ldsFinish, int& ldsScratch) {
  cvd_handle* h = c.h;
  const int F = c.L.F, B = c.L.B;
  h->tailStageRows = false;
  if (!h->opt.pcg_fused_tail || h->tailDisabled || h->dist() || B > 256 || h->forceGeneric) return false;
  if (coarse && !h->coarse.denseMode) return false;
  const int split = denseRowSplit(h);
  const TlStep ts = temporalStep(h);
  if (ts.Ainv != nullptr && (ts.S * ts.width > cgUpdatePartDoubles(B, nThreads) || tlRowsLds(ts.NT) > B + cgUpdatePartDoubles(B, nThreads)))
    return false;
  const bool poseT = coarse && h->coarse.temporalPose;
  if (poseT && tlRowsLds(h->coarse.ptN) > B + cgUpdatePartDoubles(B, nThreads)) return false;
  const int grid = F + (coarse && !poseT && split > 0 ? (F + kDenseFramesPerGroup - 1) / kDenseFramesPerGroup : 0) +
                   (ts.Ainv != nullptr ? ts.S * ts.parts : 0) + (poseT ? kCB * tlParts(h->coarse.ptNn) : 0);
  const int update = B + cgUpdatePartDoubles(B, nThreads) + 48 + 17 * kCB;
  const int finish = 3 * B + 8 + kCB + (nThreads / 256 - 1) * 256 + kTlMaxS;
  const int denseEnd = (coarse && !poseT) ? F * kCB + nThreads + 16 : 0;
  ldsFinish = update;
  const int unstaged = std::max(update + finish + (coarse && split < kCB ? denseEnd : 0), denseEnd);
  int stagedEnd = 0;
  if (ts.Ainv != nullptr) stagedEnd = std::max(stagedEnd, tlStagedLds(ts.NT));
  if (poseT) stagedEnd = std::max(stagedEnd, tlStagedLds(h->coarse.ptN));
  static std::map<std::tuple<int, int, int, size_t>, int> perCuCache;
  static std::mutex cacheMutex;
  auto resident = [&](size_t bytes) {
    if (bytes > kMaxLds) return false;
    int perCu = 0;
    std::lock_guard<std::mutex> lock(cacheMutex);
    const auto key = std::make_tuple(h->device, c.KD, nThreads, bytes);
    auto it = perCuCache.find(key);
    if (it == perCuCache.end()) {
      CVD_DISPATCH_KD(c.KD, {
        allowLds((k_pcg_tail<KD>), bytes);
        HIP_CHECK(hipOccupancyMaxActiveBlocksPerMultiprocessor(&perCu, reinterpret_cast<const void*>(&k_pcg_tail<KD>), nThreads, bytes));
      });
      perCuCache[key] = perCu;
    } else {
      perCu = it->second;
    }
    return static_cast<long long>(perCu) * h->numCU >= grid;
  };
  if (stagedEnd > 0 && h->dbg.tail_no_row_staging == 0) {
    ldsScratch = std::max(unstaged, stagedEnd);
    lds = static_cast<size_t>(ldsScratch + 24) * sizeof(double);
    if (resident(lds)) {
      h->tailStageRows = true;
      return true;
    }
  }
  ldsScratch = unstaged;
  lds = static_cast<size_t>(ldsScratch + 24) * sizeof(double);
  return resident(lds);
}

void launchPcgTail(Ctx& c, const double* x, const double* pOld, double* pNew, int useBeta, const double* lam, double* q,
                   bool withCoarse, int nThreads, size_t lds, int ldsFinish, int ldsScratch, double tol2) {
  cvd_handle* h = c.h;
  hipStream_t s = h->stream;
  const int F = c.L.F;
  const CoarseView cF = coarseView(h, withCoarse, false);
  const int split = denseRowSplit(h);
  const int finishDoubles = 3 * static_cast<int>(c.L.B) + 8 + kCB + (nThreads / 256 - 1) * 256 + kTlMaxS;
  const TlStep ts = temporalStep(h);
  const bool poseT = withCoarse && h->coarse.temporalPose;
  const DenseStep ds = (withCoarse && !poseT) ? DenseStep{h->coarse.denseInv.p, h->coarse.qc.p, h->coarse.rc.p, h->coarse.c.p, h->coarse.dotPart.p,
                                               h->coarse.modeActive.p, h->coarse.fail.p, split, ldsFinish + finishDoubles,
                                               h->coarse.dotPart.p + F}
                                  : DenseStep{nullptr, nullptr, nullptr, nullptr, nullptr, nullptr, nullptr, kCB, 0, nullptr};
  double* fd = h->dFdot.p;
  const TailUpdate U{h->dMinv.p, h->dDx.p, h->dR.p, h->dZ.p, fd + F, fd + 2 * F, tol2, h->coarse.modeActive.p, h->hPcg,
                     h->dCounters.p + 1, h->dTailBar.p, h->dFdot.p + 4 * static_cast<size_t>(F) + 32, ldsFinish, ldsScratch, ds,
                     ts.Ainv != nullptr ? temporalStepDev(h) : static_cast<const TlStep*>(nullptr),
                     poseT ? poseTemporalStepDev(h) : static_cast<const TlStep*>(nullptr),
                     (c.cross && h->xDiagRows) ? 1 : 0, h->tailStageRows ? 1 : 0};
  const int grid = F + (withCoarse && !poseT && split > 0 ? (F + kDenseFramesPerGroup - 1) / kDenseFramesPerGroup : 0) +
                   (ts.Ainv != nullptr ? ts.S * ts.parts : 0) + (poseT ? kCB * tlParts(h->coarse.ptNn) : 0);
  const int slot = h->tBegin(KC_CG_UPDATE);
  {
    std::unique_ptr<PersistentGate> gate;
    std::unique_lock<std::mutex> alone(PersistentGate::slot(h->device).m);
    if (liveHandles(h->device) > 1) {
      alone.unlock();
      gate.reset(new PersistentGate(h->device, s));
    }
    CVD_DISPATCH_KD(c.KD, {
      hipLaunchKernelGGL((k_pcg_tail<KD>), dim3(grid), dim3(nThreads), lds, s, c.L, x, h->dMask.p, lam, h->dMedian.p, h->dRegOwner.p,
                         h->dInRange.p, c.cross ? h->dXFiOff.p : h->dFiOff.p, h->dFiList.p, h->dQPart.p, pOld, pNew, h->dScal.p,
                         useBeta, q, fd, c.cross ? static_cast<int>(h->xFa.size()) * 2 : h->qRows, h->regCache, cF,
                         withCoarse ? h->coarse.qc.p : static_cast<double*>(nullptr),
                         c.cross ? static_cast<const double*>(h->dH.p) : static_cast<const double*>(nullptr), U);
    });
    HIP_CHECK(hipGetLastError());
  }
  h->tEnd(slot);
}

void touchModule_matvec() {
  hipFuncAttributes a;
  (void)hipFuncGetAttributes(&a, reinterpret_cast<const void*>(k_dot_pq));
}

}

#ifdef CVD_TAIL_PROFILE
extern "C" int32_t cvd_debug_tail_profile(unsigned long long* out) {
  (void)hipDeviceSynchronize();
  return hipMemcpyFromSymbol(out, HIP_SYMBOL(cvd::g_tailProf), sizeof(unsigned long long) * 1024 * 16) == hipSuccess ? 0 : 1;
}
#endif
#ifdef CVD_MV_PROFILE
extern "C" int32_t cvd_debug_mv_profile(unsigned long long* out) {
  (void)hipDeviceSynchronize();
  return hipMemcpyFromSymbol(out, HIP_SYMBOL(cvd::g_mvProf), sizeof(unsigned long long) * 4096 * 8) == hipSuccess ? 0 : 1;
}
#endif
```

robust_cvd_amd/csrc/cvd_pcg.h:

```cpp
#pragma once

#include "cvd_kernels.h"

namespace cvd {

inline __global__ void k_lm_diag(Layout L, const double* __restrict__ hdiag, double* __restrict__ scale,
                          int computeScale, double radius, double* __restrict__ lam) {
  const size_t n = static_cast<size_t>(L.F) * L.B;
  const size_t i = static_cast<size_t>(blockIdx.x) * blockDim.x + threadIdx.x;
  if (i >= n) return;
  const double h = hdiag[i];
  if (computeScale) scale[i] = 1.0 / (1.0 + sqrt(h));
  const double s = scale[i];
  if (h == 0.0) {
    lam[i] = 1.0;
  } else {
    const double d = fmin(fmax(s * s * h, 1e-6), 1e32);
    lam[i] = d / (radius * s * s);
  }
}

template <int KD>
inline __global__ __launch_bounds__(256) void k_reg_cache(Layout L, const double* __restrict__ x,
                                                   const float* __restrict__ median,
// ... 261 lines not shown
  }
  return true;
}

template <int KD>
inline __global__ __launch_bounds__(256) void k_matvec_finish(Layout L, const double* __restrict__ x,
                                                       const double* __restrict__ mask,
                                                       const double* __restrict__ lam, const float* __restrict__ median,
                                                       const unsigned char* __restrict__ inRange,
                                                       const unsigned char* __restrict__ rangeFlags,
                                                       const int* __restrict__ fiOff, const int* __restrict__ fiList,
                                                       const double* __restrict__ qPart, const double* __restrict__ z,
                                                       const double* __restrict__ pOld, double* __restrict__ pNew,
                                                       double* __restrict__ scal, unsigned int* __restrict__ counter,
                                                       int useBeta, double* __restrict__ q, double* __restrict__ fdot,
                                                       int distMode, int nRows, RegCache rc, CoarseView V,
                                                       double* __restrict__ qc, CoarseColumns cc,
                                                       const double* __restrict__ Hdiag, double* __restrict__ pqOut,
                                                       int ownFirst, int ownCount, const TlStep* __restrict__ tsp) {
  extern __shared__ __attribute__((aligned(16))) double sm[];
  TailCarry carry;
  (void)matvecFinishBody<KD, false>(L, x, mask, lam, median, inRange, rangeFlags, fiOff, fiList, qPart, z, pOld, pNew, scal, counter,
                                    useBeta, q, fdot, distMode, nRows, rc, V, qc, cc, Hdiag, pqOut, ownFirst, ownCount, sm, carry, tsp,
                                    sm + 3 * L.B + 8 + kCB + kTlMaxS);
}

inline __global__ __launch_bounds__(256) void k_dot_pq(Layout L, const double* __restrict__ p, const double* __restrict__ q,
                                                double* __restrict__ scal, unsigned int* __restrict__ counter,
                                                double* __restrict__ fdot, double* __restrict__ qc,
                                                const unsigned char* __restrict__ modeActive, CoarseColumns cc,
                                                const TlStep* __restrict__ tsp) {
  if (scal[S_DONE] != 0.0) return;
  __shared__ double red[8];
  __shared__ double prod[kTlMaxS * kTlMaxWidth];
  const int f = blockIdx.x, tid = threadIdx.x;
  const size_t base = static_cast<size_t>(f) * L.B;
  if (tsp != nullptr) {
    const TlStep ts = *tsp;
    const int nE = ts.S * ts.width;
    for (int e = tid; e < nE; e += 256) prod[e] = static_cast<double>(ts.elW[e]) * q[base + 7 + ts.elV[e]];
    __syncthreads();
    if (tid < ts.S) {
      double a = 0.0;
      for (int k = 0; k < ts.width; ++k) a += prod[k * ts.S + tid];
      ts.sq[static_cast<size_t>(f) * ts.S + tid] = a;
    }
  }
  if (qc != nullptr) {
    coarseRestrict(L, q + base, f, tid, modeActive, qc);
    __syncthreads();
    coarseColumnProducts(cc, qc + f * kCB, f, tid, 256);
  }
  double dot = 0.0;
  for (int i = tid; i < L.B; i += 256) dot += p[base + i] * q[base + i];
  dot = waveSum(dot);
  if ((tid & 63) == 0) red[tid >> 6] = dot;
  __syncthreads();
  if (tid == 0) publishPartial(fdot + f, red[0] + red[1] + red[2] + red[3]);
  if (lastBlockArrivesLite(counter, L.F, reinterpret_cast<int*>(red + 6))) {
    const double pq = blockSumPartials(fdot, L.F, red);
    if (tid == 0) {
      scal[S_PQ] = pq;
      scal[S_ALPHA] = scal[S_RZ] / pq;
    }
  }
}

__host__ __device__ inline int cgUpdatePartDoubles(int B, int nThreads) {
  return B > 256 ? nThreads : max(nThreads, 16 * ((B + 3) & ~3));
}

#ifdef CVD_TAIL_PROFILE
__device__ unsigned long long g_tailProf[1024 * 16];
#define TAIL_STAMP(slot) do { if (threadIdx.x == 0) g_tailProf[(blockIdx.x & 1023) * 16 + (slot)] = wall_clock64(); } while (0)
#else
#define TAIL_STAMP(slot) do {} while (0)
#endif

struct NoMid {
  __device__ bool first(double&, double&) { return true; }
  __device__ bool second(double&) { return true; }
  __device__ unsigned int generation() { return 0u; }
  __device__ bool stageRows() { return false; }
};
__host__ __device__ inline int tlStagedLds(int NT) { return tlRowsLds(NT) + (kTlSpan + 1) * NT; }
typedef unsigned int cvd_u32x4 __attribute__((ext_vector_type(4)));
template <bool FUSED, typename Mid>
__device__ __forceinline__ bool tlLevelRows(const TlStep* __restrict__ tsp, int wg, int F, double& alpha, int init, double sDone,
                                            const double* __restrict__ scal, double* __restrict__ sm, Mid& mid) {
  const TlStep ts = *tsp;
  const int tid = threadIdx.x, nThreads = blockDim.x;
  const int wv = tid >> 6, lane = tid & 63, nW = nThreads >> 6;
  const int s = wg / ts.parts, part = wg - s * ts.parts;
  const int aLo = part * ts.span, aHi = min(ts.nn - 1, aLo + ts.span), nA = aHi - aLo + 1;
  const bool ownsLast = part == ts.parts - 1;
  const int par = init ? 1 : (static_cast<int>(scal[S_ITERS]) & 1);
  const double* tin = ts.t + static_cast<size_t>(par) * ts.NT;
  double* tout = ts.t + static_cast<size_t>(par ^ 1) * ts.NT;
  double* qT = sm;
  double* tn = qT + ts.NT;
  double* red = tn + ts.span + 1;
  double rOldPre = 0.0, tOldPre = 0.0;
  if (lane == 0 && !init) {
    const int e = s * ts.nn + aLo + (wv < nA ? wv : 0);
    rOldPre = ts.rT[e];
    tOldPre = tin[e];
  }
  double* stage = sm + tlRowsLds(ts.NT);
  bool staged = false;
  if constexpr (FUSED) {
    staged = mid.stageRows();
    if (staged) {
      constexpr int kStageBatch = 8;
      for (int k = wv; k < nA; k += nW) {
        const double* row = ts.Ainv + static_cast<size_t>(s * ts.nn + aLo + k) * ts.ld;
        double* dst = stage + static_cast<size_t>(k) * ts.NT;
        for (int c0 = 0; c0 < ts.NT; c0 += 64 * kStageBatch) {
          double v[kStageBatch];
#pragma unroll
          for (int u = 0; u < kStageBatch; ++u) {
            const int c = c0 + u * 64 + lane;
            v[u] = row[min(c, ts.NT - 1)];
          }
#pragma unroll
          for (int u = 0; u < kStageBatch; ++u) {
            const int c = c0 + u * 64 + lane;
            if (c < ts.NT) dst[c] = v[u];
          }
        }
      }
    }
    TAIL_STAMP(8);
  }
  bool on = false;
  if constexpr (FUSED) {
    on = *ts.fail == 0;
    if (!mid.second(alpha)) return false;
  }
  const double inv = 1.0 / static_cast<double>(ts.step);
  bool direct = true;
  if constexpr (FUSED) {
    if (ts.rec != nullptr) {
      direct = false;
      const unsigned int gen = mid.generation() + 1u;
      cvd_u32x4* rec = reinterpret_cast<cvd_u32x4*>(ts.rec);
      for (int a = wv; a < ts.nn; a += nW) {
        const int f = (a - 1) * ts.step + 1 + lane;
        const bool in = lane < 2 * ts.step - 1 && f >= 0 && f < F;
        double v = in ? readPartial(ts.sq + static_cast<size_t>(f) * ts.S + s) : 0.0;
        v *= 1.0 - fabs(static_cast<double>(f - a * ts.step)) * inv;
        v = waveSum(in ? v : 0.0);
        if (lane == 0 && part == 0) {
          cvd_u32x4 r4;
          r4.x = gen;
          r4.y = static_cast<unsigned int>(__double2loint(v));
          r4.z = static_cast<unsigned int>(__double2hiint(v));
          r4.w = gen;
          *reinterpret_cast<volatile cvd_u32x4*>(rec + s * ts.nn + a) = r4;
        }
      }
      int* bad = reinterpret_cast<int*>(red + ts.span + 1);
      if (tid == 0) *bad = 0;
      __syncthreads();
      for (int e = tid; e < ts.NT; e += nThreads) {
        const volatile cvd_u32x4* src = reinterpret_cast<const volatile cvd_u32x4*>(rec + e);
        cvd_u32x4 r4;
        unsigned int spins = 0;
        for (;;) {
          r4 = *src;
          if (r4.x == gen && r4.w == gen) break;
          __builtin_amdgcn_s_sleep(4);
          if (++spins > (1u << 20)) {
            *bad = 1;
            break;
          }
        }
        qT[e] = __hiloint2double(static_cast<int>(r4.z), static_cast<int>(r4.y));
      }
      __syncthreads();
      if (*bad) return false;
    }
  }
  if (direct) {
    for (int e = tid; e < ts.NT; e += nThreads) {
      const int a = e / ts.S, sp = e - a * ts.S;
      const int fLo = max(0, (a - 1) * ts.step + 1), fHi = min(F - 1, (a + 1) * ts.step - 1);
      constexpr int kTlBatch = 8;
      double acc[4] = {0.0, 0.0, 0.0, 0.0};
      for (int f = fLo; f <= fHi; f += kTlBatch) {
        double v[kTlBatch];
#pragma unroll
        for (int u = 0; u < kTlBatch; ++u) {
          const double* src = ts.sq + static_cast<size_t>(min(f + u, fHi)) * ts.S + sp;
          v[u] = FUSED ? readPartial(src) : *src;
        }
#pragma unroll
        for (int u = 0; u < kTlBatch; ++u) {
          const double w = 1.0 - fabs(static_cast<double>(f + u - a * ts.step)) * inv;
          acc[u & 3] += (f + u <= fHi) ? w * v[u] : 0.0;
        }
      }
      qT[sp * ts.nn + a] = (acc[0] + acc[1]) + (acc[2] + acc[3]);
    }
    __syncthreads();
  }
  if (sDone != 0.0) return false;
  if constexpr (FUSED) TAIL_STAMP(5);
  if constexpr (!FUSED) on = *ts.fail == 0;
  for (int k = wv; k < nA; k += nW) {
    const int a = aLo + k, e = s * ts.nn + a;
    const double* row = ts.Ainv + static_cast<size_t>(e) * ts.ld;
    const bool owned = ownsLast || a < aHi;
    double rOld = rOldPre, tOld = tOldPre;
    double acc0 = 0.0, acc1 = 0.0;
    int c = lane;
    if (k != wv && lane == 0 && !init) {
      rOld = ts.rT[e];
      tOld = tin[e];
    }
    if (staged) {
      const double* srow = stage + static_cast<size_t>(k) * ts.NT;
      for (; c + 64 < ts.NT; c += 128) {
        acc0 += srow[c] * qT[c];
        acc1 += srow[c + 64] * qT[c + 64];
      }
      if (c < ts.NT) acc0 += srow[c] * qT[c];
    } else {
      for (; c + 64 < ts.NT; c += 128) {
        acc0 += row[c] * qT[c];
        acc1 += row[c + 64] * qT[c + 64];
      }
      if (c < ts.NT) acc0 += row[c] * qT[c];
    }
    const double d = ts.weight * waveSum(acc0 + acc1);
    if (lane == 0) {
      const double rn = init ? qT[e] : rOld - alpha * qT[e];
      const double tv = on ? (init ? d : tOld - alpha * d) : 0.0;
      if (owned) {
        ts.rT[e] = rn;
        tout[e] = tv;
      }
      tn[k] = tv;
      red[k] = owned ? tv * rn : 0.0;
    }
  }
  __syncthreads();
  if constexpr (FUSED) TAIL_STAMP(6);
  const int fLo = aLo * ts.step, fHi = ownsLast ? F : min(F, aHi * ts.step);
  for (int f = fLo + tid; f < fHi; f += nThreads) {
    const int a0 = f / ts.step, k0 = a0 - aLo;
    const double tau = static_cast<double>(f - a0 * ts.step) * inv;
    ts.tl[static_cast<size_t>(f) * ts.S + s] = (1.0 - tau) * tn[k0] + tau * tn[min(k0 + 1, nA - 1)];
  }
  if (tid == 0) {
    double d = 0.0;
    for (int k = 0; k < nA; ++k) d += red[k];
    publishPartial(ts.dotPart + wg, d);
  }
  if constexpr (FUSED) TAIL_STAMP(7);
  return true;
}

template <bool FUSED, typename Mid>
__device__ __forceinline__ void cgUpdateBody(const Layout& L, int init, const double* __restrict__ g,
                                             const float* __restrict__ minv, const double* __restrict__ p,
                                             const double* __restrict__ q, double* __restrict__ scal,
                                             unsigned int* __restrict__ counter, double* __restrict__ dx,
                                             double* __restrict__ r, double* __restrict__ z,
                                             double* __restrict__ fdotRZ, double* __restrict__ fdotRR,
                                             double tol2, double* __restrict__ rc,
                                             const unsigned char* __restrict__ modeActive,
                                             double* __restrict__ hostMirror, const CoarseStep& cs, const DenseStep& ds,
                                             const double* __restrict__ pqReduced, double* __restrict__ sm, Mid& mid,
                                             int f0, int nF, double* __restrict__ partOut, const TlStep* __restrict__ tsp,
                                             const TlStep* __restrict__ tpp) {
  const double sDone = (init || FUSED) ? 0.0 : scal[S_DONE];
  const int B = L.B;
  const int nThreads = blockDim.x;
  double* rf = sm;
  double* part = rf + B;
  double* red = part + cgUpdatePartDoubles(B, nThreads);
  double* ypart = red + 48;
  const bool fusedY = !init && cs.Wb != nullptr;
  const bool fusedDense = !init && ds.Ainv != nullptr;
  const int nWaves = nThreads >> 6;
  const int nExtraWg = static_cast<int>(gridDim.x) - nF;
  const int bid = FUSED ? static_cast<int>(blockIdx.x)
                        : (static_cast<int>(blockIdx.x) < nExtraWg ? nF + static_cast<int>(blockIdx.x) : static_cast<int>(blockIdx.x) - nExtraWg);
  const bool denseWg = bid >= nF;
  const int f = denseWg ? L.F + (bid - nF) : f0 + bid;
  const int nDenseWg = (fusedDense && ds.rowSplit > 0) ? (nF + kDenseFramesPerGroup - 1) / kDenseFramesPerGroup : 0;
  const bool tlOn = !init && tsp != nullptr, tpOn = !init && tpp != nullptr;
  const bool tlWg = (tlOn || tpOn) && bid >= nF + nDenseWg;
  const int tid = threadIdx.x;
  const size_t base = static_cast<size_t>(f) * B;
  double alpha = (init || FUSED) ? 0.0 : (pqReduced != nullptr ? scal[S_RZ] / *pqReduced : scal[S_ALPHA]);
  double pvCarry = 0.0, qvCarry = 0.0;
  if constexpr (FUSED) {
    if (!mid.first(pvCarry, qvCarry)) return;
  }
#ifndef CVD_DENSE_LOADS
#define CVD_DENSE_LOADS 4
#endif
  constexpr int kDenseLoads = CVD_DENSE_LOADS;
  const size_t nC = static_cast<size_t>(L.F) * kCB;
  const int n2 = static_cast<int>(nC / 2);
  auto denseRows = [&](int g, int r0, int nR, const double* qcs, double* psum, bool on0, double2 (&w)[kDenseLoads], bool preloaded,
                       double* dotSlot) {
    const int per = nThreads / nR, m = tid / per, part = tid - m * per;
    const bool active = m < nR;
    const double2* row = reinterpret_cast<const double2*>(ds.Ainv + (static_cast<size_t>(g) * kCB + r0 + (active ? m : 0)) * nC);
    const int e = g * kCB + r0 + (tid < nR ? tid : 0);
    const double qcv = qcs[e], rcOld = ds.rc[e], cOld = ds.c[e];
    const bool on = on0 && ds.modeActive[e];
    double acc0 = 0.0, acc1 = 0.0;
    for (int base = 0; base < n2; base += kDenseLoads * per) {
      if (!preloaded || base > 0) {
#pragma unroll
        for (int u = 0; u < kDenseLoads; ++u) {
          const int j = base + part + u * per;
          w[u] = row[j < n2 ? j : 0];
          if (j >= n2 || !active) w[u] = make_double2(0.0, 0.0);
        }
      }
#pragma unroll
      for (int u = 0; u < kDenseLoads; ++u) {
        const int j = base + part + u * per;
        const double2 qq = *reinterpret_cast<const double2*>(qcs + 2 * (j < n2 ? j : 0));
        acc0 += w[u].x * qq.x;
        acc1 += w[u].y * qq.y;
      }
    }
    psum[tid] = active ? acc0 + acc1 : 0.0;
    __syncthreads();
    if (tid < nR * 8) {
      const int r = tid >> 3, l = tid & 7;
      double t = 0.0;
      for (int k = l; k < per; k += 8) t += psum[r * per + k];
      t += __shfl_xor(t, 1, 64);
      t += __shfl_xor(t, 2, 64);
      t += __shfl_xor(t, 4, 64);
      if (l == 0) psum[nThreads + r] = t;
    }
    __syncthreads();
    if (tid < 8) {
      double t = 0.0;
      if (tid < nR) {
        const double d = psum[nThreads + tid];
        const double rcn = rcOld - alpha * qcv;
        const double cn = on ? cOld - alpha * d : 0.0;
        ds.rc[e] = rcn;
        ds.c[e] = cn;
        t = cn * rcn;
      }
      t += __shfl_xor(t, 1, 64);
      t += __shfl_xor(t, 2, 64);
      t += __shfl_xor(t, 4, 64);
      if (tid == 0) publishPartial(dotSlot, t);
    }
    __syncthreads();
  };
  if (f >= L.F) {
    if (tlWg) {
      const int k = bid - nF - nDenseWg, nTl = tlOn ? tsp->S * tsp->parts : 0;
      if (!tlLevelRows<FUSED>(k < nTl ? tsp : tpp, k < nTl ? k : k - nTl, L.F, alpha, 0, sDone, scal, sm, mid)) return;
    } else {
    const int nR = ds.rowSplit;
    double* qcs = sm;
    double* psum = sm + nC;
    const int g0 = f0 + (f - L.F) * kDenseFramesPerGroup;
    double2 w[kDenseLoads];
    {
      const int per = nThreads / nR, m = tid / per, part = tid - m * per;
      const double2* row = reinterpret_cast<const double2*>(ds.Ainv + (static_cast<size_t>(g0) * kCB + (m < nR ? m : 0)) * nC);
#pragma unroll
      for (int u = 0; u < kDenseLoads; ++u) {
        const int j = part + u * per;
        w[u] = row[j < n2 ? j : 0];
        if (j >= n2 || m >= nR) w[u] = make_double2(0.0, 0.0);
      }
    }
    if constexpr (FUSED) {
      if (!mid.second(alpha)) return;
      for (int i = tid; i < static_cast<int>(nC); i += nThreads) qcs[i] = readPartial(ds.qc + i);
    } else {
      for (int i = tid; i < static_cast<int>(nC); i += nThreads) qcs[i] = ds.qc[i];
    }
    const bool on0 = *ds.fail == 0;
    __syncthreads();
    if (sDone != 0.0) return;
    for (int rep = 0; rep < kDenseFramesPerGroup; ++rep) {
      const int g = g0 + rep;
      if (g >= f0 + nF) break;
      denseRows(g, 0, nR, qcs, psum, on0, w, rep == 0, ds.dotPart + g);
    }
    }
  } else {
  struct __attribute__((packed, aligned(4))) F4u { float x, y, z, w; };
  constexpr int kMinvLoads = 8;
  const bool wide = B > 256;
  const float* Mf = minv + static_cast<size_t>(f) * B * B;
  const int nQ = (B + 3) >> 2;
  const int nSeg = min(16, nThreads / nQ);
  const int q4 = tid % nQ, sg = tid / nQ;
  F4u mreg[kMinvLoads];
  if (!wide && sg < nSeg) {
    const float* col = Mf + 4 * q4;
#pragma unroll
    for (int u = 0; u < kMinvLoads; ++u) {
      const int j = sg + u * nSeg;
      if (u * nSeg < B) mreg[u] = *reinterpret_cast<const F4u*>(col + static_cast<size_t>(min(j, B - 1)) * B);
    }
  }
  {
    const int j = tid;
    double pv = 0.0, qv = 0.0, rv = 0.0, dv = 0.0;
    if (j < B) {
      if (init) {
        rv = -g[base + j];
      } else {
        if constexpr (!FUSED) {
          pv = p[base + j];
          qv = q[base + j];
        }
        rv = r[base + j];
        dv = dx[base + j];
      }
    }
    if constexpr (!FUSED) asm volatile("" : "+v"(pv), "+v"(qv), "+v"(rv), "+v"(dv));
    if constexpr (FUSED) {
      pv = pvCarry;
      qv = qvCarry;
      if (!mid.second(alpha)) return;
    } else {
      if (sDone != 0.0) return;
    }
    if (j < B) {
      if (!init) {
        dv += alpha * pv;
        rv -= alpha * qv;
      }
// ... 24 lines not shown
  const int chunk = wide ? tid >> 7 : tid >> 8, row = tid & 63, seg = wide ? (tid >> 6) & 1 : (tid >> 6) & 3;
  const int i = chunk * 64 + row;
  double acc = 0.0;
  if (wide) {
    if (i < B) {
      double a0 = 0.0, a1 = 0.0, a2 = 0.0, a3 = 0.0;
      const float* col = Mf + i;
      int j = seg;
      for (; j + 6 < B; j += 8) {
        a0 += static_cast<double>(col[static_cast<size_t>(j) * B]) * rf[j];
        a1 += static_cast<double>(col[static_cast<size_t>(j + 2) * B]) * rf[j + 2];
        a2 += static_cast<double>(col[static_cast<size_t>(j + 4) * B]) * rf[j + 4];
        a3 += static_cast<double>(col[static_cast<size_t>(j + 6) * B]) * rf[j + 6];
      }
      for (; j < B; j += 2) a0 += static_cast<double>(col[static_cast<size_t>(j) * B]) * rf[j];
      acc = (a0 + a1) + (a2 + a3);
    }
  } else {
    double a0 = 0.0, a1 = 0.0, a2 = 0.0, a3 = 0.0;
    if (sg < nSeg) {
#pragma unroll
      for (int u = 0; u < kMinvLoads; ++u) {
        const int j = sg + u * nSeg;
        if (u * nSeg < B) {
          const double rj = j < B ? rf[j] : 0.0;
          a0 += static_cast<double>(mreg[u].x) * rj;
          a1 += static_cast<double>(mreg[u].y) * rj;
          a2 += static_cast<double>(mreg[u].z) * rj;
          a3 += static_cast<double>(mreg[u].w) * rj;
        }
      }
      if (kMinvLoads * nSeg < B) {
        const float* col = Mf + 4 * q4;
#pragma unroll
        for (int u = 0; u < kMinvLoads; ++u) {
          const int j = sg + (kMinvLoads + u) * nSeg;
          if ((kMinvLoads + u) * nSeg < B) mreg[u] = *reinterpret_cast<const F4u*>(col + static_cast<size_t>(min(j, B - 1)) * B);
        }
#pragma unroll
        for (int u = 0; u < kMinvLoads; ++u) {
          const int j = sg + (kMinvLoads + u) * nSeg;
          if ((kMinvLoads + u) * nSeg < B) {
            const double rj = j < B ? rf[j] : 0.0;
            a0 += static_cast<double>(mreg[u].x) * rj;
            a1 += static_cast<double>(mreg[u].y) * rj;
            a2 += static_cast<double>(mreg[u].z) * rj;
            a3 += static_cast<double>(mreg[u].w) * rj;
          }
        }
      }
      double* dst = part + static_cast<size_t>(sg) * (4 * nQ) + 4 * q4;
      dst[0] = a0; dst[1] = a1; dst[2] = a2; dst[3] = a3;
    }
    __syncthreads();
    if (tid < B) {
      double zv = 0.0;
      for (int k2 = 0; k2 < nSeg; ++k2) zv += part[static_cast<size_t>(k2) * (4 * nQ) + tid];
      acc = zv;
    }
  }
  if (wide) part[tid] = acc;
  __syncthreads();
  double rz = 0.0, rr = 0.0;
  if (wide) {
    if (seg == 0 && i < B) {
      const int b0 = chunk * 128 + row;
      const double zv = part[b0] + part[b0 + 64];
      z[base + i] = zv;
      rz = rf[i] * zv;
      rr = rf[i] * rf[i];
    }
  } else if (tid < B) {
    z[base + tid] = acc;
    rz = rf[tid] * acc;
    rr = rf[tid] * rf[tid];
  }
  rz = waveSum(rz);
  rr = waveSum(rr);
  if ((tid & 63) == 0) { red[tid >> 6] = rz; red[16 + (tid >> 6)] = rr; }
  __syncthreads();
  if (tid == 0) {
    double a = 0.0, b = 0.0;
    for (int w = 0; w < nWaves; ++w) { a += red[w]; b += red[16 + w]; }
    publishPartial(fdotRZ + f, a);
    publishPartial(fdotRR + f, b);
  }
  if (fusedY) {
    if (tid < kCB) {
      double sy = 0.0;
      for (int w = 0; w < nWaves; ++w) sy += ypart[w * kCB + tid];
      const double yn = cs.y[f * kCB + tid] - alpha * sy;
      cs.y[f * kCB + tid] = yn;
      ypart[16 * kCB + tid] = yn * yn;
    }
    __syncthreads();
    if (tid == 0) {
      double t = 0.0;
#pragma unroll
      for (int k = 0; k < kCB; ++k) t += ypart[16 * kCB + k];
      publishPartial(cs.fdotY + f, t);
    }
  }
  if (fusedDense && ds.rowSplit < kCB) {
    double* qcs = sm + ds.ldsPsum;
    double* psum = qcs + nC;
    if constexpr (FUSED) {
      for (int i = tid; i < static_cast<int>(nC); i += nThreads) qcs[i] = readPartial(ds.qc + i);
    } else {
      for (int i = tid; i < static_cast<int>(nC); i += nThreads) qcs[i] = ds.qc[i];
    }
    const bool on0 = *ds.fail == 0;
    __syncthreads();
    double2 w[kDenseLoads];
    denseRows(f, ds.rowSplit, kCB - ds.rowSplit, qcs, psum, on0, w, false, ds.dotPart2 + f);
  }
  }
  if (lastBlockArrivesLite(counter, gridDim.x, reinterpret_cast<int*>(red + 40))) {
    double a = 0.0, b = 0.0, cY = 0.0;
    for (int k = f0 + tid; k < f0 + nF; k += nThreads) {
      a += readPartial(fdotRZ + k);
      b += readPartial(fdotRR + k);
      if (fusedY) cY += readPartial(cs.fdotY + k);
      if (fusedDense && ds.rowSplit > 0) cY += readPartial(ds.dotPart + k);
      if (fusedDense && ds.rowSplit < kCB) cY += readPartial(ds.dotPart2 + k);
    }
    double cT = 0.0;
    if (tlOn)
      for (int k = tid; k < tsp->S * tsp->parts; k += nThreads) cT += readPartial(tsp->dotPart + k);
    if (tpOn)
      for (int k = tid; k < tpp->S * tpp->parts; k += nThreads) cT += readPartial(tpp->dotPart + k);
    a = waveSum(a);
    b = waveSum(b);
    cY = waveSum(cY);
    cT = waveSum(cT);
    __syncthreads();
    if ((tid & 63) == 0) { red[tid >> 6] = a; red[16 + (tid >> 6)] = b; ypart[tid >> 6] = cY; ypart[16 + (tid >> 6)] = cT; }
    __syncthreads();
    if (tid == 0) {
      double rzs = 0.0, rrs = 0.0, ys = 0.0, tls = 0.0;
      for (int w = 0; w < nWaves; ++w) { rzs += red[w]; rrs += red[16 + w]; ys += ypart[w]; tls += ypart[16 + w]; }
      rzs += (partOut == nullptr || f0 == 0) ? tls : 0.0;
      if (partOut != nullptr) {
        partOut[0] = rzs + ((fusedY && *cs.fail != 0) ? 0.0 : ys);
        partOut[1] = rrs;
      } else if (fusedY) {
        pcgFinishScalars(scal, 0, rzs + (*cs.fail == 0 ? ys : 0.0), rrs, tol2, hostMirror);
      } else if (fusedDense) {
        pcgFinishScalars(scal, 0, rzs + ys, rrs, tol2, hostMirror);
      } else if (rc != nullptr || (init && (tsp != nullptr || tpp != nullptr))) {
        scal[S_RZPART] = rzs;
        scal[S_RR] = rrs;
      } else {
        pcgFinishScalars(scal, init, rzs, rrs, tol2, hostMirror);
      }
    }
  }
}

inline __global__ __launch_bounds__(1024) void k_cg_update(Layout L, int init, const double* __restrict__ g,
                                                    const float* __restrict__ minv, const double* __restrict__ p,
                                                    const double* __restrict__ q, double* __restrict__ scal,
                                                    unsigned int* __restrict__ counter, double* __restrict__ dx,
                                                    double* __restrict__ r, double* __restrict__ z,
                                                    double* __restrict__ fdotRZ, double* __restrict__ fdotRR,
                                                    double tol2, double* __restrict__ rc,
                                                    const unsigned char* __restrict__ modeActive,
                                                    double* __restrict__ hostMirror, CoarseStep cs, DenseStep ds,
                                                    const double* __restrict__ pqReduced, int f0, int nF,
                                                    double* __restrict__ partOut, const TlStep* __restrict__ tsp,
                                                    const TlStep* __restrict__ tpp) {
  extern __shared__ __attribute__((aligned(16))) double sm[];
  NoMid mid;
  cgUpdateBody<false>(L, init, g, minv, p, q, scal, counter, dx, r, z, fdotRZ, fdotRR, tol2, rc, modeActive, hostMirror, cs, ds,
                      pqReduced, sm, mid, f0, nF, partOut, tsp, tpp);
}

inline __global__ void k_pcg_scalars_dist(const double* __restrict__ parts, int world, double* __restrict__ scal, double tol2,
                                          double* __restrict__ hostMirror) {
  if (threadIdx.x != 0 || scal[S_DONE] != 0.0) return;
  double rz = 0.0, rr = 0.0;
  for (int r = 0; r < world; ++r) {
    rz += parts[2 * r];
    rr += parts[2 * r + 1];
  }
  pcgFinishScalars(scal, 0, rz, rr, tol2, hostMirror);
}

constexpr int kTailBarCopies = 16;
constexpr int kTailBarStride = 1024;
__device__ __forceinline__ unsigned int tailGeneration(const unsigned int* bar) {
  if (threadIdx.x != 0) return 0u;
  return *reinterpret_cast<const volatile unsigned int*>(bar + kTailBarStride * (1 + (blockIdx.x & (kTailBarCopies - 1))));
}
__device__ __forceinline__ void tailArrive(unsigned int* bar, unsigned int nGroups, unsigned int gen, const double* __restrict__ parts,
                                           int nParts, double* __restrict__ scratch) {
  asm volatile("s_waitcnt vmcnt(0)" ::: "memory");
  __syncthreads();
  if (threadIdx.x >= 64) return;
  unsigned int ticket = 0u;
// ... 1 lines not shown
  ticket = __builtin_amdgcn_readfirstlane(ticket);
  gen = __builtin_amdgcn_readfirstlane(gen);
  const bool last = ticket == nGroups - 1;
  if (last) {
    double a = 0.0;
    for (int k0 = threadIdx.x; k0 < nParts + static_cast<int>(threadIdx.x); k0 += 8 * 64) {
      double w[8];
#pragma unroll
      for (int u = 0; u < 8; ++u) w[u] = k0 + u * 64 < nParts ? readPartial(parts + k0 + u * 64) : 0.0;
#pragma unroll
      for (int u = 0; u < 8; ++u) a += w[u];
    }
    const double v = waveSum(a);
    if (threadIdx.x == 0) __hip_atomic_store(bar, 0u, __ATOMIC_RELAXED, __HIP_MEMORY_SCOPE_AGENT);
    if (threadIdx.x < kTailBarCopies) {
      cvd_u32x4 rec;
      rec.x = gen + 1u;
      rec.y = static_cast<unsigned int>(__double2loint(v));
      rec.z = static_cast<unsigned int>(__double2hiint(v));
      rec.w = gen + 1u;
      *reinterpret_cast<volatile cvd_u32x4*>(bar + kTailBarStride * (1 + threadIdx.x)) = rec;
    }
    if (threadIdx.x == 0) scratch[18] = v;
  }
  if (threadIdx.x == 0) {
    *reinterpret_cast<int*>(scratch + 16) = last ? 2 : 1;
    *reinterpret_cast<unsigned int*>(scratch + 17) = gen;
  }
}
__device__ __forceinline__ bool tailWait(unsigned int* bar, double* __restrict__ scratch, double& sum) {
  int* role = reinterpret_cast<int*>(scratch + 16);
  __syncthreads();
  const unsigned int gen = *reinterpret_cast<unsigned int*>(scratch + 17);
  if (*role == 2) {
    sum = scratch[18];
    return true;
  }
  if (threadIdx.x == 0) {
    const volatile cvd_u32x4* mine = reinterpret_cast<const volatile cvd_u32x4*>(bar + kTailBarStride * (1 + (blockIdx.x & (kTailBarCopies - 1))));
    int ok = 1;
    unsigned int spins = 0;
    cvd_u32x4 rec;
    for (;;) {
      rec = *mine;
      if (rec.x == gen + 1u && rec.w == gen + 1u) break;
      __builtin_amdgcn_s_sleep(16);
      ++spins;
      if ((spins & 63u) == 0 && __hip_atomic_load(bar + 1, __ATOMIC_RELAXED, __HIP_MEMORY_SCOPE_AGENT) != 0u) { ok = 0; break; }
      if (spins > (1u << 18)) {
        __hip_atomic_store(bar + 1, 1u, __ATOMIC_RELAXED, __HIP_MEMORY_SCOPE_AGENT);
        __hip_atomic_fetch_add(bar, 0x40000000u, __ATOMIC_RELAXED, __HIP_MEMORY_SCOPE_AGENT);
        ok = 0;
        break;
      }
    }
    scratch[18] = ok ? __hiloint2double(static_cast<int>(rec.z), static_cast<int>(rec.y)) : 0.0;
    *role = ok;
  }
  __syncthreads();
  sum = scratch[18];
  return *role != 0;
}

struct TailUpdate {
  const float* minv;
  double* dx;
  double* r;
  double* z;
  double* fdotRZ;
  double* fdotRR;
  double tol2;
  const unsigned char* modeActive;
  double* hostMirror;
  unsigned int* counter;
  unsigned int* gridBar;
  double* pqSlot;
  int ldsFinish;
  int ldsScratch;
  DenseStep ds;
  const TlStep* ts;
  const TlStep* tp;
  int diagInProduct;
  int stageRows;
};

template <int KD>
inline __global__ __launch_bounds__(1024) __attribute__((amdgpu_waves_per_eu(6))) void k_pcg_tail(Layout L, const double* __restrict__ x,
                                                    const double* __restrict__ mask,
                                                    const double* __restrict__ lam, const float* __restrict__ median,
                                                    const unsigned char* __restrict__ inRange,
                                                    const unsigned char* __restrict__ rangeFlags,
                                                    const int* __restrict__ fiOff, const int* __restrict__ fiList,
                                                    const double* __restrict__ qPart, const double* __restrict__ pOld,
                                                    double* __restrict__ pNew, double* __restrict__ scal, int useBeta,
                                                    double* __restrict__ q, double* __restrict__ fdot, int nRows, RegCache rc,
                                                    CoarseView V, double* __restrict__ qc, const double* __restrict__ Hdiag,
                                                    TailUpdate U) {
  extern __shared__ __attribute__((aligned(16))) double sm[];
  const int f = blockIdx.x;
  const CoarseColumns ccOff{nullptr, nullptr, nullptr, nullptr, nullptr};
  const CoarseStep csOff{nullptr, nullptr, nullptr, nullptr, nullptr, nullptr, nullptr, nullptr, nullptr};
  TAIL_STAMP(0);
  const unsigned int barGen = tailGeneration(U.gridBar);
  const double rzOld = scal[S_RZ];
  auto first = [&](double& pv, double& qv) -> bool {
    if (f < L.F) {
      TailCarry carry{0.0, 0.0};
      if (!matvecFinishBody<KD, true>(L, x, mask, lam, median, inRange, rangeFlags, fiOff, fiList, qPart, U.z, pOld, pNew, scal,
                                      nullptr, useBeta, q, fdot, 0, nRows, rc, V, qc, ccOff, Hdiag, nullptr, 0, U.diagInProduct ? 0 : L.F,
                                      sm + U.ldsFinish, carry, U.ts, sm + L.B))
        return false;
      pv = carry.pv;
      qv = carry.qv;
    } else if (scal[S_DONE] != 0.0) {
      return false;
    }
    TAIL_STAMP(1);
    tailArrive(U.gridBar, gridDim.x, barGen, fdot, L.F, sm + U.ldsScratch);
    TAIL_STAMP(10);
    if (f < L.F && static_cast<int>(threadIdx.x) < L.B) {
      pNew[static_cast<size_t>(f) * L.B + threadIdx.x] = pv;
      q[static_cast<size_t>(f) * L.B + threadIdx.x] = qv;
    }
    return true;
  };
  auto second = [&](double& alpha) -> bool {
    double pq;
    TAIL_STAMP(2);
    if (!tailWait(U.gridBar, sm + U.ldsScratch, pq)) return false;
    TAIL_STAMP(3);
    alpha = rzOld / pq;
    if (blockIdx.x == 0 && threadIdx.x == 0) {
      scal[S_PQ] = pq;
      scal[S_ALPHA] = alpha;
    }
    return true;
  };
  struct Mid {
    decltype(first)& f1;
    decltype(second)& f2;
    double* scratch;
    __device__ bool first(double& pv, double& qv) { return f1(pv, qv); }
    __device__ bool second(double& alpha) { return f2(alpha); }
    __device__ unsigned int generation() { return *reinterpret_cast<unsigned int*>(scratch + 17); }
    bool stage;
    __device__ bool stageRows() { return stage; }
  } mid{first, second, sm + U.ldsScratch, U.stageRows != 0};
  cgUpdateBody<true>(L, 0, nullptr, U.minv, nullptr, nullptr, scal, U.counter, U.dx, U.r, U.z, U.fdotRZ, U.fdotRR, U.tol2, nullptr,
                     U.modeActive, U.hostMirror, csOff, U.ds, nullptr, sm, mid, 0, L.F, nullptr, U.ts, U.tp);
  TAIL_STAMP(4);
}

inline __global__ void k_apply_step(Layout L, int boundDepth0, const double* __restrict__ x, const double* __restrict__ dx,
                             double* __restrict__ xc) {
  const size_t n = static_cast<size_t>(L.F) * L.B;
  const size_t i = static_cast<size_t>(blockIdx.x) * blockDim.x + threadIdx.x;
  if (i >= n) return;
  double v = x[i] + dx[i];
  if (boundDepth0) {
    const int c = static_cast<int>(i % L.B);
    if (c >= 7 && c < 7 + L.nD && ((c - 7) % L.N) == 0) v = fmax(v, 0.0);
  }
  xc[i] = v;
}

inline __global__ __launch_bounds__(1024) void k_tl_rows_init(const TlStep* __restrict__ tsp, int F, double* __restrict__ scal,
                                                       unsigned int* __restrict__ counter, int closeScalars, double tol2,
                                                       double* __restrict__ hostMirror) {
  extern __shared__ __attribute__((aligned(16))) double sm[];
  __shared__ int flag;
  NoMid mid;
  double alpha = 0.0;
  (void)tlLevelRows<false>(tsp, blockIdx.x, F, alpha, 1, 0.0, scal, sm, mid);
  if (!lastBlockArrivesLite(counter, gridDim.x, &flag)) return;
  if (threadIdx.x == 0) {
    double d = 0.0;
    for (int s = 0; s < tsp->S * tsp->parts; ++s) d += readPartial(tsp->dotPart + s);
    if (closeScalars) pcgFinishScalars(scal, 1, scal[S_RZPART] + d, scal[S_RR], tol2, hostMirror);
    else scal[S_RZPART] += d;
  }
}

}
```

robust_cvd_amd/csrc/cvd_setup.hip:

```cpp
#include "cvd_host.h"
#include "cvd_table.h"
#include "cvd_triplets.h"
#include "cvd_dense_walk.h"
#include <rocprim/device/device_segmented_radix_sort.hpp>

namespace cvd {

void launchFrameConsts(const Layout& L, const double* x, FrameConst* fc, hipStream_t s) {
  hipLaunchKernelGGL(k_frame_consts, dim3((L.F + 63) / 64), dim3(64), 0, s, L, x, fc);
}

static void quatToMatrix(const double q[4] , double R[3][3]) {
  for (int c = 0; c < 3; ++c) {
    double v[3] = {0, 0, 0};
    v[c] = 1.0;
    const double uv[3] = {2.0 * (q[1] * v[2] - q[2] * v[1]), 2.0 * (q[2] * v[0] - q[0] * v[2]),
                          2.0 * (q[0] * v[1] - q[1] * v[0])};
    R[0][c] = v[0] + q[3] * uv[0] + (q[1] * uv[2] - q[2] * uv[1]);
    R[1][c] = v[1] + q[3] * uv[1] + (q[2] * uv[0] - q[0] * uv[2]);
    R[2][c] = v[2] + q[3] * uv[2] + (q[0] * uv[1] - q[1] * uv[0]);
  }
}
static void matrixToAngleAxis(const double R[3][3], double aa[3]) {
  double q0, q1, q2, q3;
// ... 1065 lines not shown
    h->hStageN[which] = n;
  }
  return h->hStage[which];
}

void uploadState(cvd_handle* h, const Layout& L, DevBuf<double>& dst) {
  const size_t nAll = static_cast<size_t>(L.F) * L.B;
  double* x = pinnedStage(h, 1, nAll);
  const int nD = L.nD, nS = L.nS;
  for (int f = 0; f < L.F; ++f) {
    double* xf = &x[static_cast<size_t>(f) * L.B];
    for (int i = 0; i < 7; ++i) xf[i] = h->poseParams[f][i];
    for (int i = 0; i < nD; ++i) xf[7 + i] = h->dparams[static_cast<size_t>(f) * nD + i];
    for (int i = 0; i < nS; ++i) xf[7 + nD + i] = h->sparams[static_cast<size_t>(f) * nS + i];
  }
  dst.upload(x, nAll, h->stream);
  HIP_CHECK(hipStreamSynchronize(h->stream));
}

void downloadState(cvd_handle* h, const Layout& L, const DevBuf<double>& src) {
  const size_t nAll = static_cast<size_t>(L.F) * L.B;
  double* x = pinnedStage(h, 0, nAll);
  src.download(x, nAll, h->stream);
  HIP_CHECK(hipStreamSynchronize(h->stream));
  const int nD = L.nD, nS = L.nS;
  for (int f = 0; f < L.F; ++f) {
    const double* xf = &x[static_cast<size_t>(f) * L.B];
    for (int i = 0; i < 7; ++i) h->poseParams[f][i] = xf[i];
    for (int i = 0; i < nD; ++i) h->dparams[static_cast<size_t>(f) * nD + i] = xf[7 + i];
    for (int i = 0; i < nS; ++i) h->sparams[static_cast<size_t>(f) * nS + i] = xf[7 + nD + i];
  }
}

void buildMask(cvd_handle* h, const Layout& L, const cvd_opt_params& p, ProblemKind kind,
                      const std::vector<int>& range) {
  const size_t nAll = static_cast<size_t>(L.F) * L.B;
  HIP_CHECK(hipStreamSynchronize(h->stream));
  double* m = pinnedStage(h, 0, nAll);
  std::fill(m, m + nAll, 0.0);
  for (int f : range) {
    double* mf = &m[static_cast<size_t>(f) * L.B];
    const bool poseFree = (kind == PK_POSE_STEP) && !p.fix_poses;
    for (int i = 0; i < 6; ++i) mf[i] = poseFree ? 1.0 : 0.0;
    mf[6] = (kind == PK_POSE_STEP && p.intr_opt != CVD_INTR_FIXED) ? 1.0 : 0.0;
    const bool depthFree = (kind == PK_NORMALIZE) || !p.fix_depth_xforms;
    for (int i = 0; i < L.nD; ++i) mf[7 + i] = depthFree ? 1.0 : 0.0;
    const bool spatialFree = (kind == PK_POSE_STEP) && !p.fix_spatial_xforms;
    for (int i = 0; i < L.nS; ++i) mf[7 + L.nD + i] = spatialFree ? 1.0 : 0.0;
  }
  h->dMask.upload(m, nAll, h->stream);
}

void ensureBuffers(Ctx& c) {
  cvd_handle* h = c.h;
  const size_t n = c.n;
  const size_t B = c.L.B;
  h->dX.ensure(n); h->dXc.ensure(n); h->dG.ensure(n); h->dLam.ensure(n); h->dScale.ensure(n);
  const size_t nVec = static_cast<size_t>(h->framesPadded()) * B;
  if (h->dist() && (h->dDx.n < nVec || h->dZ.n < nVec)) {
    h->dDx.ensure(nVec); h->dR.ensure(nVec); h->dZ.ensure(nVec);
    HIP_CHECK(hipMemsetAsync(h->dDx.p, 0, nVec * sizeof(double), h->stream));
    HIP_CHECK(hipMemsetAsync(h->dR.p, 0, nVec * sizeof(double), h->stream));
    HIP_CHECK(hipMemsetAsync(h->dZ.p, 0, nVec * sizeof(double), h->stream));
  }
  h->dDx.ensure(nVec); h->dR.ensure(nVec); h->dR1.ensure(n); h->dZ.ensure(nVec); h->dP0.ensure(n); h->dP1.ensure(n);
  h->dQ.ensure(nVec + static_cast<size_t>(c.L.F) * (kCB + kTlMaxS) + 8);
  h->dOwnerScal.ensure(2 * static_cast<size_t>(std::max(1, h->world)));
  h->dHd.ensure(n);
  {
    const size_t nPad = static_cast<size_t>(h->framesPadded()) * B;
    const bool grow = h->dH.n < nPad * B;
    h->dH.ensure(nPad * B); h->dMinv.ensure(nPad * B + 4); h->dHd.ensure(nPad);
    if (h->dist() && (grow || nPad > n)) {
      HIP_CHECK(hipMemsetAsync(h->dH.p, 0, nPad * B * sizeof(double), h->stream));
      HIP_CHECK(hipMemsetAsync(h->dMinv.p, 0, nPad * B * sizeof(float), h->stream));
      HIP_CHECK(hipMemsetAsync(h->dHd.p, 0, nPad * sizeof(double), h->stream));
    }
  }
  h->dQPart.ensure(std::max<size_t>(1, static_cast<size_t>(std::max(std::max(h->qRows, c.nItems * 2), c.cross ? h->xRows : 0)) * B));
  h->dFdot.ensure(static_cast<size_t>(c.L.F) * 4 + 64);
  h->dCostItem.ensure(std::max(1, c.nItems));
  h->dCostFrame.ensure(c.L.F);
  h->dFocal.ensure(static_cast<size_t>(c.L.F) * 2);
  h->dScal.ensure(S_COUNT);
  h->dFc.ensure(c.L.F);
  h->dFail.ensure(1);
  if (!h->dCounters.p) {
    h->dCounters.ensure(8);
    HIP_CHECK(hipMemsetAsync(h->dCounters.p, 0, 8 * sizeof(unsigned int), h->stream));
  }
  if (!h->hScal) HIP_CHECK(hipHostMalloc(reinterpret_cast<void**>(&h->hScal), (S_COUNT + 1) * sizeof(double)));
  if (!h->hPcg) {
    HIP_CHECK(hipHostMalloc(reinterpret_cast<void**>(&h->hPcg), 16 * sizeof(double)));
    for (auto& e : h->pcgEvent) HIP_CHECK(hipEventCreateWithFlags(&e, hipEventDisableTiming));
  }
}
__global__ void k_pick_median(const float* __restrict__ sorted, size_t n, int first, int count, float* __restrict__ median) {
  const int i = blockIdx.x * blockDim.x + threadIdx.x;
  if (i < count) median[first + i] = sorted[static_cast<size_t>(i) * n + n / 2];
}
void refreshMedians(cvd_handle* h) {
  if (!h->medianDirty) return;
  hipStream_t s = h->stream;
  const size_t n = static_cast<size_t>(h->W) * h->H;
  const int F = h->F;
  h->dMedian.ensure(F);
  const int PB = static_cast<int>(std::max<size_t>(1, std::min<size_t>(F, (size_t(1) << 28) / (n * sizeof(float)))));
  if (static_cast<size_t>(PB) * n > 0xFFFFFFFFull) throw std::runtime_error("depth maps too large for the median sort");
  DevBuf<float> sorted;
  DevBuf<unsigned int> seg;
  DevBuf<unsigned char> tmp;
  sorted.ensure(static_cast<size_t>(PB) * n);
  std::vector<unsigned int> segH(PB + 1);
  for (int i = 0; i <= PB; ++i) segH[i] = static_cast<unsigned int>(static_cast<size_t>(i) * n);
  seg.upload(segH.data(), segH.size(), s);
  size_t tmpBytes = 0;
  HIP_CHECK(rocprim::segmented_radix_sort_keys(nullptr, tmpBytes, h->dDepth.p, sorted.p, static_cast<unsigned int>(PB * n),
                                               static_cast<unsigned int>(PB), seg.p, seg.p + 1, 0, 32, s));
  tmp.ensure(tmpBytes);
  for (int p0 = 0; p0 < F; p0 += PB) {
    const int nb = std::min(PB, F - p0);
    size_t tb = tmpBytes;
    HIP_CHECK(rocprim::segmented_radix_sort_keys(tmp.p, tb, h->dDepth.p + static_cast<size_t>(p0) * n, sorted.p,
                                                 static_cast<unsigned int>(nb * n), static_cast<unsigned int>(nb), seg.p,
                                                 seg.p + 1, 0, 32, s));
    hipLaunchKernelGGL(k_pick_median, dim3((nb + 63) / 64), dim3(64), 0, s, sorted.p, n, p0, nb, h->dMedian.p);
    HIP_CHECK(hipGetLastError());
  }
  HIP_CHECK(hipStreamSynchronize(s));
  h->medianDirty = false;
}

void touchModule_setup() {
  hipFuncAttributes a;
  (void)hipFuncGetAttributes(&a, reinterpret_cast<const void*>(k_pick_median));
}

}
```

robust_cvd_amd/csrc/cvd_solve.hip:

```cpp
#include <optional>

#include "cvd_host.h"
#include "cvd_lm.h"
#include "cvd_pcg.h"
#include "cvd_coarse.h"

namespace cvd {

void launchTlRowsInit(cvd_handle* h, const TlStep* tsp, int NT, int groups, int F, unsigned int* counter, int closeScalars, double tol2,
                      hipStream_t s) {
  const size_t lds = static_cast<size_t>(tlRowsLds(NT)) * 8;
  allowLds(k_tl_rows_init, lds);
  hipLaunchKernelGGL(k_tl_rows_init, dim3(groups), dim3(768), lds, s, tsp, F, h->dScal.p, counter, closeScalars, tol2, h->hPcg);
  HIP_CHECK(hipGetLastError());
}

namespace {
struct TailStalled {};
}
static int runPcgAttempt(Ctx& c, const double* x, const std::function<void()>& tail);
int runPcg(Ctx& c, const double* x, const std::function<void()>& tail) {
  const size_t firstTimerSlot = c.h->evUsed;
  try {
    return runPcgAttempt(c, x, tail);
  } catch (const TailStalled&) {
    cvd_handle* h = c.h;
    HIP_CHECK(hipStreamSynchronize(h->stream));
    HIP_CHECK(hipMemsetAsync(h->dCounters.p, 0, 8 * sizeof(unsigned int), h->stream));
    if (h->temporal.counter.p) HIP_CHECK(hipMemsetAsync(h->temporal.counter.p, 0, 4 * sizeof(unsigned int), h->stream));
    if (h->dTailBar.p)
      HIP_CHECK(hipMemsetAsync(h->dTailBar.p, 0, static_cast<size_t>(kTailBarStride) * (1 + kTailBarCopies) * sizeof(unsigned int), h->stream));
    h->curPcgIter = -1;
    h->tDropFrom(firstTimerSlot, 0);
    h->tailDisabled = true;
    fprintf(stderr, "[cvd] warning: k_pcg_tail's grid barrier was abandoned (device shared with other work?); this handle uses the "
                    "two-launch PCG tail from here on\n");
    return runPcgAttempt(c, x, tail);
  }
}
static int runPcgAttempt(Ctx& c, const double* x, const std::function<void()>& tail) {
  cvd_handle* h = c.h;
  hipStream_t s = h->stream;
  const int F = c.L.F;
  const size_t B = c.L.B;
  if (B > 512) throw std::runtime_error("frame block larger than 512 unknowns is not supported by k_cg_update");
  prepareMatvec(c, x);
  const int nChunks = static_cast<int>((B + 63) / 64);
  const int nThreads = (B > 256 ? 128 : 256) * nChunks;
  double* fd = h->dFdot.p;
  size_t ldsU = (B + cgUpdatePartDoubles(static_cast<int>(B), nThreads) + 48 + 17 * kCB) * 8;
  const double tol2 = c.h->opt.pcg_relative_tolerance * c.h->opt.pcg_relative_tolerance;
  for (int i = 0; i < 9; ++i) h->hPcg[i] = 0.0;
  const bool coarse = h->coarseOn;
  double* rc = coarse ? h->coarse.rc.p : nullptr;
  const bool denseCoarse = coarse && h->coarse.denseMode;
  const bool unfusedY = denseCoarse;
  auto coarseC = [&](int init) {
    if (c.L.positionRegSqrt > 0.0 || c.trip || !coarseFusedConsumers())
      hipLaunchKernelGGL(k_coarse_apply_wt, dim3(F), dim3(256), 0, s, coarseView(h, true, true), F, h->coarse.c.p,
                         h->dScal.p, init);
  };
  const bool poseT = denseCoarse && h->coarse.temporalPose;
  auto coarseApply = [&](int init) {
    if (poseT) {
      launchPoseTemporalInit(c, tol2);
      return;
    }
    if (denseCoarse) {
      hipLaunchKernelGGL(k_coarse_dense_apply, dim3(F), dim3(256), 0, s, F, h->coarse.denseInv.p, h->coarse.rc.p, h->coarse.c.p,
                         h->coarse.modeActive.p, h->coarse.dotPart.p, h->dScal.p, h->dCounters.p + 3, h->coarse.fail.p, init,
                         tol2, h->hPcg);
      return;
    }
    hipLaunchKernelGGL(k_coarse_apply_w, dim3(F), dim3(1024), 0, s, h->coarse.plan, h->coarse.Wb.p, h->coarse.rc.p,
                       h->coarse.y.p, h->coarse.dotPart.p, h->dScal.p, h->dCounters.p + 3, h->coarse.fail.p, init, tol2,
                       h->hPcg);
    coarseC(init);
  };
  const CoarseStep csOff{nullptr, nullptr, nullptr, nullptr, nullptr, nullptr, nullptr, nullptr, nullptr};
  const CoarseStep csOn = (coarse && !unfusedY)
                              ? CoarseStep{h->coarse.wtPtr.p, h->coarse.wtBlk.p, h->coarse.wtFrame.p, h->coarse.Wb.p,
                                           h->coarse.qc.p, h->coarse.y.p, h->coarse.fdotY.p, h->coarse.fail.p, h->coarse.wq.p}
                              : csOff;
  const DenseStep dsOff{nullptr, nullptr, nullptr, nullptr, nullptr, nullptr, nullptr, kCB, 0, nullptr};
  const bool denseFused = denseCoarse;
  const bool fusedX = h->dist() && fusedExchange(h, coarse);
  const double* pqReduced = fusedX ? h->dQ.p + exchangeOffsetPq(c, denseFused) : nullptr;
  const bool denseRows = denseFused && !poseT;
  const DenseStep dsOn = denseRows ? DenseStep{h->coarse.denseInv.p, fusedX ? h->dQ.p + exchangeOffsetQc(c) : h->coarse.qc.p, h->coarse.rc.p, h->coarse.c.p,
                                                h->coarse.dotPart.p, h->coarse.modeActive.p, h->coarse.fail.p,
                                                kCB, static_cast<int>(ldsU / 8), h->coarse.dotPart.p + F}
                                    : dsOff;
  if (denseRows) {
    const size_t dense = static_cast<size_t>(F) * kCB + nThreads + 16;
    ldsU = std::max((dsOn.rowSplit < kCB ? ldsU / 8 + dense : ldsU / 8), dense) * 8;
  }
  const TlStep tsOn = temporalStep(h);
  const int nTlWg = tsOn.Ainv != nullptr ? tsOn.S * tsOn.parts : 0;
  if (nTlWg) ldsU = std::max(ldsU, static_cast<size_t>(tlRowsLds(tsOn.NT)) * 8);
  const int nPtWg = poseT ? kCB * tlParts(h->coarse.ptNn) : 0;
  if (poseT) ldsU = std::max(ldsU, static_cast<size_t>(tlRowsLds(h->coarse.ptN)) * 8);
  const TlStep* tpDev = poseT ? poseTemporalStepDev(h) : nullptr;
  allowLds(k_cg_update, ldsU);
  hipLaunchKernelGGL(k_cg_update, dim3(F), dim3(nThreads), ldsU, s, c.L, 1, h->dG.p, h->dMinv.p, h->dP0.p, h->dQ.p,
                     h->dScal.p, h->dCounters.p + 1, h->dDx.p, h->dR.p, h->dZ.p, fd + F, fd + 2 * F, tol2, rc,
                     h->coarse.modeActive.p, h->hPcg, csOff, dsOff, static_cast<const double*>(nullptr), 0, F,
                     static_cast<double*>(nullptr), nTlWg ? temporalStepDev(h) : static_cast<const TlStep*>(nullptr),
                     static_cast<const TlStep*>(nullptr));
  if (nTlWg) launchTemporalInit(c, !coarse, tol2);
  if (coarse) coarseApply(1);
  HIP_CHECK(hipGetLastError());
  double* pOld = h->dP0.p;
  double* pNew = h->dP1.p;
  size_t ldsTail = 0;
  int ldsFinish = 0, ldsScratch = 0;
  const bool fusedTail = pcgTailScope(c, coarse, nThreads, ldsTail, ldsFinish, ldsScratch);
  h->lastFusedTail = fusedTail;
  h->lastKD = c.KD;
  h->lastCross = c.cross;
  if (fusedTail) {
    h->dTailBar.ensure(static_cast<size_t>(kTailBarStride) * (1 + kTailBarCopies));
    HIP_CHECK(hipMemsetAsync(h->dTailBar.p, 0, static_cast<size_t>(kTailBarStride) * (1 + kTailBarCopies) * sizeof(unsigned int), s));
    if (tsOn.rec != nullptr) HIP_CHECK(hipMemsetAsync(tsOn.rec, 0, 2 * static_cast<size_t>(tsOn.NT) * sizeof(double), s));
  }
  const bool ownerMode = ownerShardedUpdate(h, coarse);
  const int maxIt = std::max(1, c.h->opt.pcg_max_iterations);
  const bool lockstep = h->dbg.pcg_lockstep != 0;
  const size_t firstTimerSlot = h->evUsed;
  int enq = 0;
  auto enqueueIteration = [&](int it, int useBeta) {
    h->curPcgIter = it;
    if (fusedTail) {
      launchMatvec(c, x, h->dZ.p, pOld, pNew, useBeta, h->dLam.p, h->dQ.p, coarse, true);
      launchPcgTail(c, x, pOld, pNew, useBeta, h->dLam.p, h->dQ.p, coarse, nThreads, ldsTail, ldsFinish, ldsScratch, tol2);
      std::swap(pOld, pNew);
      return;
    }
    launchMatvec(c, x, h->dZ.p, pOld, pNew, useBeta, h->dLam.p, h->dQ.p, coarse);
    if (ownerMode) {
      const int f0 = h->ownFirst(), nOwn = h->ownCount();
      const int slotO = h->tBegin(KC_CG_UPDATE);
      if (nOwn > 0 || nTlWg || nPtWg)
        hipLaunchKernelGGL(k_cg_update, dim3((denseRows && dsOn.rowSplit > 0 ? nOwn + (nOwn + kDenseFramesPerGroup - 1) / kDenseFramesPerGroup : nOwn) + nTlWg + nPtWg),
                           dim3(nThreads), ldsU, s, c.L, 0, h->dG.p, h->dMinv.p, pNew, h->dQ.p, h->dScal.p, h->dCounters.p + 1,
                           h->dDx.p, h->dR.p, h->dZ.p, fd + F, fd + 2 * F, tol2, static_cast<double*>(nullptr),
                           h->coarse.modeActive.p, h->hPcg, csOff, dsOn, pqReduced, f0, nOwn, h->dOwnerScal.p + 2 * h->rank,
                           nTlWg ? temporalStepDev(h) : static_cast<const TlStep*>(nullptr), tpDev);
      else
        HIP_CHECK(hipMemsetAsync(h->dOwnerScal.p + 2 * h->rank, 0, 2 * sizeof(double), s));
      HIP_CHECK(hipGetLastError());
      h->tEnd(slotO);
      const int ct = h->tBegin(KC_COMM_PRODUCT);
      const size_t chunkF = static_cast<size_t>(h->ownChunk());
      commGroupStart(h);
      commAllGather(h, h->dZ.p + h->rank * chunkF * B, h->dZ.p, chunkF * B, CT_F64, s);
      if (denseRows) commAllGather(h, h->coarse.c.p + h->rank * chunkF * kCB, h->coarse.c.p, chunkF * kCB, CT_F64, s);
      commAllGather(h, h->dOwnerScal.p + 2 * h->rank, h->dOwnerScal.p, 2, CT_F64, s);
      commGroupEnd(h);
      h->tEnd(ct);
      hipLaunchKernelGGL(k_pcg_scalars_dist, dim3(1), dim3(64), 0, s, h->dOwnerScal.p, h->world, h->dScal.p, tol2, h->hPcg);
      HIP_CHECK(hipGetLastError());
      std::swap(pOld, pNew);
      return;
    }
    const int slot = h->tBegin(KC_CG_UPDATE);
    hipLaunchKernelGGL(k_cg_update, dim3((denseRows && dsOn.rowSplit > 0 ? F + (F + kDenseFramesPerGroup - 1) / kDenseFramesPerGroup : F) + nTlWg + nPtWg), dim3(nThreads), ldsU, s, c.L, 0, h->dG.p, h->dMinv.p, pNew,
                       h->dQ.p, h->dScal.p, h->dCounters.p + 1, h->dDx.p, h->dR.p, h->dZ.p, fd + F, fd + 2 * F, tol2,
                       (coarse && unfusedY && !denseFused) ? rc : nullptr, h->coarse.modeActive.p, h->hPcg, csOn, dsOn, pqReduced,
                       0, F, static_cast<double*>(nullptr), nTlWg ? temporalStepDev(h) : static_cast<const TlStep*>(nullptr), tpDev);
    if (coarse && !denseFused) { if (unfusedY) coarseApply(0); else coarseC(0); }
    HIP_CHECK(hipGetLastError());
    h->tEnd(slot);
    std::swap(pOld, pNew);
  };
  const int kRunAhead = lockstep ? 1 : 2;
  volatile double* prog = h->hPcg;
  while (enq < maxIt) {
    if (enq >= kRunAhead - 1) {
      const int need = enq - kRunAhead + 1;
      double v;
      for (unsigned long long spins = 0; static_cast<long long>((v = prog[1 + (need & 7)]) * 0.25) != need + 1; ++spins) {
        if ((spins & 0xFFFFF) == 0xFFFFF) {
          const hipError_t e = hipStreamQuery(s);
          if (e != hipErrorNotReady) {
            HIP_CHECK(e);
            if (static_cast<long long>(prog[1 + (need & 7)] * 0.25) != need + 1) {
              if (fusedTail) throw TailStalled{};
              throw std::runtime_error("PCG progress mirror stalled");
            }
          }
        }
      }
      if (v - 4.0 * (need + 1) != 0.0) break;
    }
    enqueueIteration(enq, enq > 0 ? 1 : 0);
    ++enq;
    if (fusedTail && h->dbg.stall_fused_tail_once != 0 && enq == 3) throw TailStalled{};
    if (h->opt.verbose >= 2) {
      readScalars(c);
      std::printf("    pcg %3d  rz %.6e  rzpart %.6e  alpha %.6e  beta %.6e  pq %.6e  done %g\n", enq - 1, h->hScal[S_RZ],
                  h->hScal[S_RZPART], h->hScal[S_ALPHA], h->hScal[S_BETA], h->hScal[S_PQ], h->hScal[S_DONE]);
    }
  }
  h->curPcgIter = -1;
  if (ownerMode) {
    const int ct = h->tBegin(KC_COMM_PRODUCT);
    const size_t chunk = static_cast<size_t>(h->ownChunk()) * B;
    commGroupStart(h);
    commAllGather(h, h->dDx.p + h->rank * chunk, h->dDx.p, chunk, CT_F64, s);
    commAllGather(h, h->dR.p + h->rank * chunk, h->dR.p, chunk, CT_F64, s);
    commGroupEnd(h);
    h->tEnd(ct);
  }
  if (tail) tail();
  readScalars(c);
  if (h->hScal[S_DONE] == 2.0) throw std::runtime_error("PCG produced NaN");
  const int iters = static_cast<int>(h->hScal[S_ITERS]);
  if (fusedTail && h->hScal[S_DONE] == 0.0 && iters != enq) throw TailStalled{};
  h->tDropFrom(firstTimerSlot, iters);
  return iters;
}

bool wantsTriplets(const cvd_opt_params& p, ProblemKind kind) {
  return kind == PK_POSE_STEP && (p.smooth_static_weight > 0.0 || p.smooth_dynamic_weight > 0.0);
}
void bindTriplets(Ctx& c, const cvd_opt_params& p, ProblemKind kind) {
  cvd_handle* h = c.h;
  c.trip = wantsTriplets(p, kind) && c.L.includeStatic;
  if (!c.trip) return;
  c.TT = TripletTable{h->dTNdc.p, h->dTDsrc.p, h->dTStatic.p, h->dTOff.p, h->dTCenter.p, h->dTSlot.p,
                      static_cast<int>(h->tripActive.size()),
                      static_cast<int>(p.smooth_loss_type),
                      std::sqrt(std::max(0.0, p.smooth_static_weight)), std::sqrt(std::max(0.0, p.smooth_dynamic_weight))};
}

namespace {

struct SetupPhases {
  bool on;
  double t = nowSeconds();
  void operator()(const char* what) {
    if (!on) return;
    const double now = nowSeconds();
    fprintf(stderr, "[setup] %-14s %8.1f us\n", what, (now - t) * 1e6);
    t = now;
  }
};

struct BindMode {
  bool checkBlock;
  bool staticGuards;
  bool levels;
};
struct BoundProblem {
  Ctx c;
  std::optional<DenseListScope> denseList;
};

void bindProblem(BoundProblem& b, cvd_handle* h, const cvd_opt_params& p, double depthDeformReg, ProblemKind kind,
                 const std::vector<int>& range, const BindMode& mode, SetupPhases& phase) {
  Ctx& c = b.c;
  c.h = h;
  c.L = makeLayout(h, p, depthDeformReg, kind);
  if (mode.checkBlock) checkFrameBlock(static_cast<size_t>(c.L.B), "solve");
  tapCounts(c.L, c.KD, c.KS);
  phase("layout");
  const bool guarded = !mode.staticGuards || c.L.includeStatic;
  b.denseList.emplace(h, h->dense && guarded && !denseFastScope(h, c.L, c.KS, wantsTriplets(p, kind)));
  compileTable(h, range, wantsTriplets(p, kind), kind == PK_NORMALIZE && c.L.includeStatic);
  orderTable(h, c.L, c.KD);
  phase("table");
  refreshMedians(h);
  phase("medians");
  c.T = makeTable(h);
  c.nItems = static_cast<int>(h->itemFa.size());
  c.it = Items{h->dItemFa.p, h->dItemFb.p, h->dItemRange.p, h->dItemSlot.p, c.nItems, h->dItemRec.p};
  c.n = static_cast<size_t>(c.L.F) * c.L.B;
  c.boundDepth0 = (kind == PK_NORMALIZE && c.L.N > 0) ? 1 : 0;
  bindTriplets(c, p, kind);
  if (guarded) checkDenseScope(h, c.L, c.KS, c.trip);
  c.cross = crossScope(h, c);
  h->coarseOn = mode.levels && h->opt.coarse_level != 0 && h->coarse.valid && c.L.includeStatic && h->coarse.nEdges > 0 &&
                !h->forceGeneric && kind == PK_POSE_STEP;
  ensureBuffers(c);
  phase("buffers");
  if (mode.levels) {
    h->coarse.ptInvPending = false;
// ... 338 lines not shown
```

Before: 342.1.

## Move PCG scalar closing from tail's last-block reduction into next matvec's share sum

When the fused PCG tail runs with a KD=4 static-disparity product, each tail workgroup now writes its rz/rr partials into fixed share slots and skips the last-block-arrives reduction. The next iteration's matvec kernel sums those shares itself to compute beta and the stop flag, and a small close kernel finalizes the scalars after the loop. This removes a serialized grid-wide reduction and atomic counter from every tail launch. In exchange each matvec block redundantly reads up to 1024 doubles and repeats the close logic, and an abandon flag plus a device-side host-mirror pointer are added to keep stalled-tail handling working.

```diff
diff --git a/include/cvd_hip_debug.h b/include/cvd_hip_debug.h
--- a/include/cvd_hip_debug.h
+++ b/include/cvd_hip_debug.h
@@ -14,6 +14,7 @@
   int32_t pcg_lockstep;
   int32_t stall_fused_tail_once;
   int32_t tail_no_row_staging;
+  int32_t tail_closes_scalars;
 } cvd_debug_options;
 void cvd_debug_options_default(cvd_debug_options* o);
 int32_t cvd_set_debug_options(cvd_handle* h, const cvd_debug_options* o);
diff --git a/robust_cvd_amd/api.py b/robust_cvd_amd/api.py
--- a/robust_cvd_amd/api.py
+++ b/robust_cvd_amd/api.py
@@ -48,6 +48,7 @@
         ("pcg_lockstep", C.c_int32),
         ("stall_fused_tail_once", C.c_int32),
         ("tail_no_row_staging", C.c_int32),
+        ("tail_closes_scalars", C.c_int32),
     ]
 
 
@@ -1630,6 +1631,7 @@
         self._check(self._fn("path_info")(self._h, out))
         form = {-1: "none", 0: "exact sparse factor", 1: "exact dense inverse", 2: "temporal pose level"}[out[1]]
         return {"pose_graph_level": form, "depth_grid_level": bool(out[2]), "fused_tail": bool(out[3] & 1), "tail_rows_staged": bool(out[3] & 2),
+                "product_sums_shares": bool(out[3] & 4), "rz_shares": out[3] >> 8,
                 "tail_disabled": bool(out[4]),
                 "taps": out[5], "work_items": out[6], "cross_blocks": bool(out[7])}
 
diff --git a/robust_cvd_amd/csrc/cvd_api.hip b/robust_cvd_amd/csrc/cvd_api.hip
--- a/robust_cvd_amd/csrc/cvd_api.hip
+++ b/robust_cvd_amd/csrc/cvd_api.hip
@@ -278,6 +278,7 @@
   o->pcg_lockstep = 0;
   o->stall_fused_tail_once = 0;
   o->tail_no_row_staging = 0;
+  o->tail_closes_scalars = 0;
 }
 int32_t cvd_set_debug_options(cvd_handle* h, const cvd_debug_options* o) {
   CVD_TRY(h, {
@@ -1040,6 +1041,7 @@
     out8[1] = !h->coarseOn ? -1 : (h->coarse.temporalPose ? 2 : (h->coarse.denseMode ? 1 : 0));
     out8[2] = h->temporal.on ? 1 : 0;
     out8[3] = h->lastFusedTail ? (h->tailStageRows ? 3 : 1) : 0;
+    if (h->lastFusedTail && h->lastShares) out8[3] |= 4 | (h->lastShareCount << 8);
     out8[4] = h->tailDisabled ? 1 : 0;
     out8[5] = h->lastKD;
     out8[6] = static_cast<int32_t>(h->itemFa.size());
diff --git a/robust_cvd_amd/csrc/cvd_host.h b/robust_cvd_amd/csrc/cvd_host.h
--- a/robust_cvd_amd/csrc/cvd_host.h
+++ b/robust_cvd_amd/csrc/cvd_host.h
@@ -348,6 +348,9 @@
   std::vector<cvd_iteration_record> records;
 
   bool lastFusedTail = false, lastCross = false;
+  bool lastShares = false;
+  int lastShareCount = 0;
+  int sharesF = -1, sharesN = -1;
   bool tailStageRows = false;
   int lastKD = 0;
   int lastProduct[6] = {0, 0, 0, -1, 0, 0};
@@ -605,10 +608,18 @@
 CoarseView coarseView(cvd_handle* h, bool on, bool walk);
 void prepareMatvec(Ctx& c, const double* x);
 void launchMatvec(Ctx& c, const double* x, const double* z, const double* pOld, double* pNew, int useBeta, const double* lam,
-                  double* q, bool withCoarse = false, bool tailFused = false);
+                  double* q, bool withCoarse = false, bool tailFused = false, int sharesIteration = 0);
 bool pcgTailScope(Ctx& c, bool coarse, int nThreads, size_t& lds, int& ldsFinish, int& ldsScratch);
+struct PcgShares {
+  int count = 0;
+  int levelShare0 = 0;
+  int levelWg0 = 0;
+};
+bool pcgSharesScope(Ctx& c, bool coarse, PcgShares& sh);
 void launchPcgTail(Ctx& c, const double* x, const double* pOld, double* pNew, int useBeta, const double* lam, double* q,
-                   bool withCoarse, int nThreads, size_t lds, int ldsFinish, int ldsScratch, double tol2);
+                   bool withCoarse, int nThreads, size_t lds, int ldsFinish, int ldsScratch, double tol2,
+                   const PcgShares* shares = nullptr);
+void launchPcgClose(Ctx& c, int enqueued);
 void launchBlockInverseRaw(cvd_handle* h, const Layout& L, const double* dH, const double* dLam, float* dMinv, int* dFail, int variant,
                            hipStream_t onStream = nullptr);
 void launchBlockInverse(Ctx& c, hipStream_t onStream = nullptr);
diff --git a/robust_cvd_amd/csrc/cvd_kernels.h b/robust_cvd_amd/csrc/cvd_kernels.h
--- a/robust_cvd_amd/csrc/cvd_kernels.h
+++ b/robust_cvd_amd/csrc/cvd_kernels.h
@@ -201,6 +201,9 @@
              S_RZPART = 18,
              S_NACTIVE = 19,
              S_COUNT = 20 };
+constexpr int kPcgSharesCap = 512;
+constexpr int kPcgMirrorAddressSlot = 15;
+enum : int { SH_MIRROR = 24, SH_ABANDON = 32, SH_RING = 34, SH_RZ = 64, SH_RR = SH_RZ + kPcgSharesCap, SH_END = SH_RR + kPcgSharesCap };
 
 __device__ __forceinline__ double blockSumArray(const double* __restrict__ a, int n, double* red) {
   double acc = 0.0;
@@ -665,6 +668,33 @@
   m12 = wiz * vv;
 }
 
+__device__ __forceinline__ double pcgSharesSum(const double (&w)[8]) {
+  return waveSum(((w[0] + w[1]) + (w[2] + w[3])) + ((w[4] + w[5]) + (w[6] + w[7])));
+}
+__device__ __forceinline__ void pcgCloseFromShares(double* scal, int applied, double rzs, double old, double beta, double done,
+                                                   double* hostMirror) {
+  scal[S_RZOLD] = old;
+  scal[S_BETA] = beta;
+  scal[S_ITERS] = static_cast<double>(applied);
+  scal[S_DONE] = done;
+  scal[S_RZ] = rzs;
+  scal[SH_RING + (applied & 1)] = rzs;
+  if (hostMirror != nullptr)
+    __hip_atomic_store(hostMirror + 1 + (applied & 7), 4.0 * (static_cast<double>(applied) + 1.0) + done, __ATOMIC_RELAXED,
+                       __HIP_MEMORY_SCOPE_SYSTEM);
+}
+__device__ __forceinline__ void pcgSharesClose(const double* scal, int applied, double rzs, double ctl, double& beta, double& stop) {
+  const double old = readLane(ctl, 0), target = readLane(ctl, 1), abandon = readLane(ctl, 2), mirror = readLane(ctl, 3);
+  const double sDone = readLane(ctl, 4);
+  double done = sDone;
+  if (done == 0.0) done = !(rzs == rzs) ? 2.0 : (rzs <= target ? 1.0 : 0.0);
+  beta = (old != 0.0) ? rzs / old : 0.0;
+  stop = (done != 0.0 || abandon != 0.0) ? 1.0 : 0.0;
+  if (__builtin_expect(blockIdx.x == 0 && threadIdx.x == 0 && sDone == 0.0 && abandon == 0.0, 0))
+    pcgCloseFromShares(const_cast<double*>(scal), applied, rzs, old, beta, done,
+                       reinterpret_cast<double*>(static_cast<unsigned long long>(__double_as_longlong(mirror))));
+}
+
 #ifdef CVD_MV_PROFILE
 __device__ unsigned long long g_mvProf[4096 * 8];
 #define MV_STAMP(slot) do { if ((threadIdx.x & 63) == 0) g_mvProf[(blockIdx.x & 4095) * 8 + (slot)] = wall_clock64(); } while (0)
@@ -680,14 +710,15 @@
 #ifndef CVD_MV_EARLY
 #define CVD_MV_EARLY 1
 #endif
-template <int KD, int NT, int SPEC = 0, bool DENSE = false>
+template <int KD, int NT, int SPEC = 0, bool DENSE = false, bool SHARES = false>
 inline __global__ __launch_bounds__(NT) __attribute__((amdgpu_waves_per_eu(SPEC ? ((KD <= 4 && !DENSE) ? CVD_MV_WAVES : 3) : 2))) void k_matvec_pairs_fast(Layout L, Table T, Items it, const double* __restrict__ x,
                                                            const FrameConst* __restrict__ fc,
                                                            const double* __restrict__ mask,
                                                            const double* __restrict__ z, const double* __restrict__ pOld,
                                                            const double* __restrict__ scal, int useBeta,
                                                            double* __restrict__ qPart, CoarseView V) {
-  const double sDone = scal[S_DONE];
+  double sDone = 0.0;
+  if constexpr (!SHARES) sDone = scal[S_DONE];
   extern __shared__ __attribute__((aligned(16))) double sm[];
   constexpr int NV = KD == 1 ? kRedVals : 11;
   const int B = L.B;
@@ -711,11 +742,31 @@
   const int fa = recp->fa, fb = recp->fb;
   const int slotA = recp->slotA, slotB = recp->slotB;
   const long long cbD[2] = {recp->b0, recp->b1}, ceD[2] = {recp->e0, recp->e1};
-  const double beta = useBeta ? scal[S_BETA] : 0.0;
+  double beta = 0.0;
+  if constexpr (!SHARES) beta = useBeta ? scal[S_BETA] : 0.0;
   const FrameConst* __restrict__ fcF[2] = {fc + fa, fc + fb};
-  constexpr bool kEarlyPrime = KD <= 4 && CVD_MV_EARLY;
+  constexpr bool kEarlyPrime = KD <= 4 && CVD_MV_EARLY && !(SHARES && NT == 64);
   RecordStream<DENSE> rs;
   if constexpr (kEarlyPrime) rs.primeClamped(T, cbD[0], tid, static_cast<int>(ceD[0] - cbD[0]));
+  double vsh[8] = {0.0, 0.0, 0.0, 0.0, 0.0, 0.0, 0.0, 0.0};
+  double vctl = 0.0, shBeta = 0.0, shStop = 0.0;
+  if constexpr (SHARES) {
+    if (tid < 64) {
+      const double* __restrict__ sh = scal + SH_RZ + tid;
+#pragma unroll
+      for (int u = 0; u < 8; ++u) vsh[u] = sh[u * 64];
+      const int prevAt = useBeta == 1 ? static_cast<int>(S_RZ0) : SH_RING + ((useBeta - 1) & 1);
+      vctl = scal[tid == 0 ? prevAt : (tid == 1 ? static_cast<int>(S_TARGET) : (tid == 2 ? static_cast<int>(SH_ABANDON) : (tid == 3 ? static_cast<int>(SH_MIRROR) : static_cast<int>(S_DONE))))];
+      if constexpr (NT == 64) {
+        pcgSharesClose(scal, useBeta, pcgSharesSum(vsh), vctl, shBeta, shStop);
+        if (tid == 0) {
+          red[0] = shBeta;
+          red[1] = shStop;
+        }
+        __builtin_amdgcn_sched_barrier(0);
+      }
+    }
+  }
   constexpr int EPT = 256 / NT;
   constexpr int TLE = (2 * kTlMaxS + NT - 1) / NT;
   const bool fusedCoarse = V.Wb != nullptr;
@@ -794,8 +845,24 @@
   }
   if constexpr (kUsePriv)
     for (int i = tid; i < kPriv * 2 * B; i += NT) qpriv[i] = 0.0;
-  __syncthreads();
-  if (sDone != 0.0) return;
+  if constexpr (SHARES) {
+    if (tid < 64) {
+      if constexpr (NT > 64) {
+        pcgSharesClose(scal, useBeta, pcgSharesSum(vsh), vctl, shBeta, shStop);
+        if (tid == 0) {
+          red[0] = shBeta;
+          red[1] = shStop;
+        }
+      }
+    }
+  }
+  __syncthreads();
+  if constexpr (SHARES) {
+    beta = red[0];
+    if (uniformValue(red[1]) != 0.0) return;
+  } else {
+    if (sDone != 0.0) return;
+  }
 #pragma unroll
   for (int e = 0; e < EPT; ++e) {
     const int i = tid + e * NT;
diff --git a/robust_cvd_amd/csrc/cvd_matvec.hip b/robust_cvd_amd/csrc/cvd_matvec.hip
--- a/robust_cvd_amd/csrc/cvd_matvec.hip
+++ b/robust_cvd_amd/csrc/cvd_matvec.hip
@@ -57,9 +57,20 @@
   HIP_CHECK(hipGetLastError());
 }
 
+static bool productSumsShares(const Ctx& c) {
+  const cvd_handle* h = c.h;
+  if (c.cross || !c.L.includeStatic || c.nItems <= 0 || h->dense) return false;
+  if (h->forceGeneric || c.KS != 0 || !fastLoss(c.L)) return false;
+  if (!(c.L.N == 1 && c.L.lossType == CVD_STATIC_REPRO_DISPARITY)) return false;
+  if (c.L.robustKind != 0) return false;
+  if (c.KD != 4) return false;
+  return !(c.trip && c.TT.nGroups > 0);
+}
+
 void launchMatvec(Ctx& c, const double* x, const double* z, const double* pOld, double* pNew, int useBeta,
-                         const double* lam, double* q, bool withCoarse, bool tailFused) {
-  cvd_handle* h = c.h;
+                         const double* lam, double* q, bool withCoarse, bool tailFused, int sharesIteration) {
+  cvd_handle* h = c.h;
+  if (sharesIteration > 0 && !productSumsShares(c)) throw std::runtime_error("launchMatvec: this product cannot sum the tail's shares");
   hipStream_t s = h->stream;
   const CoarseView cF = coarseView(h, withCoarse, coarseFusedConsumers());
   const size_t B = c.L.B;
@@ -103,6 +114,19 @@
 #define CVD_LAUNCH_PAIRS_FAST_S(NTV, SPECV)                                                                              \
       CVD_DISPATCH_KD(c.KD, {                                                                                            \
         recordLaunch(NTV, SPECV, KD, 1, c.nItems);                                                                       \
+        if constexpr (SPECV == 1 && KD == 4) {                                                                           \
+          if (sharesIteration > 0) {           \
+            allowLds((k_matvec_pairs_fast<KD, NTV, SPECV, false, true>), ldsFast);                                       \
+            if (evStart)                                                                                                 \
+              hipExtLaunchKernelGGL((k_matvec_pairs_fast<KD, NTV, SPECV, false, true>), dim3(c.nItems), dim3(NTV), ldsFast, s, \
+                                    evStart, evStop, 0, c.L, c.T, c.it, x, fcp, maskp, z, pOld, scalp, sharesIteration,  \
+                                    h->dQPart.p, cF);                                                                    \
+            else                                                                                                         \
+              hipLaunchKernelGGL((k_matvec_pairs_fast<KD, NTV, SPECV, false, true>), dim3(c.nItems), dim3(NTV), ldsFast, s, c.L, \
+                                 c.T, c.it, x, fcp, maskp, z, pOld, scalp, sharesIteration, h->dQPart.p, cF);             \
+            break;                                                                                                       \
+          }                                                                                                              \
+        }                                                                                                                \
         allowLds((k_matvec_pairs_fast<KD, NTV, SPECV>), ldsFast);                                                        \
         if (evStart)                                                                                                     \
           hipExtLaunchKernelGGL((k_matvec_pairs_fast<KD, NTV, SPECV>), dim3(c.nItems), dim3(NTV), ldsFast, s, evStart, evStop, 0, \
@@ -265,8 +289,29 @@
   return resident(lds);
 }
 
+bool pcgSharesScope(Ctx& c, bool coarse, PcgShares& sh) {
+  cvd_handle* h = c.h;
+  if (h->dbg.tail_closes_scalars != 0 || h->dbg.pcg_lockstep != 0 || h->opt.verbose >= 2 || !productSumsShares(c)) return false;
+  const int F = c.L.F;
+  const int split = denseRowSplit(h);
+  const TlStep ts = temporalStep(h);
+  const bool poseT = coarse && h->coarse.temporalPose;
+  const bool dense = coarse && !poseT;
+  const int nDenseWg = (dense && split > 0) ? (F + kDenseFramesPerGroup - 1) / kDenseFramesPerGroup : 0;
+  sh.levelShare0 = F + ((dense && split > 0) ? F : 0) + ((dense && split < kCB) ? F : 0);
+  sh.levelWg0 = F + nDenseWg;
+  sh.count = sh.levelShare0 + (ts.Ainv != nullptr ? ts.S * ts.parts : 0) + (poseT ? kCB * tlParts(h->coarse.ptNn) : 0);
+  return sh.count <= kPcgSharesCap;
+}
+
+void launchPcgClose(Ctx& c, int enqueued) {
+  cvd_handle* h = c.h;
+  hipLaunchKernelGGL(k_pcg_close, dim3(1), dim3(64), 0, h->stream, h->dScal.p, enqueued, h->hPcg);
+  HIP_CHECK(hipGetLastError());
+}
+
 void launchPcgTail(Ctx& c, const double* x, const double* pOld, double* pNew, int useBeta, const double* lam, double* q,
-                   bool withCoarse, int nThreads, size_t lds, int ldsFinish, int ldsScratch, double tol2) {
+                   bool withCoarse, int nThreads, size_t lds, int ldsFinish, int ldsScratch, double tol2, const PcgShares* shares) {
   cvd_handle* h = c.h;
   hipStream_t s = h->stream;
   const int F = c.L.F;
@@ -275,16 +320,22 @@
   const int finishDoubles = 3 * static_cast<int>(c.L.B) + 8 + kCB + (nThreads / 256 - 1) * 256 + kTlMaxS;
   const TlStep ts = temporalStep(h);
   const bool poseT = withCoarse && h->coarse.temporalPose;
-  const DenseStep ds = (withCoarse && !poseT) ? DenseStep{h->coarse.denseInv.p, h->coarse.qc.p, h->coarse.rc.p, h->coarse.c.p, h->coarse.dotPart.p,
+  double* sharesRz = shares != nullptr ? h->dScal.p + SH_RZ : nullptr;
+  double* densePart = shares != nullptr ? sharesRz + F : h->coarse.dotPart.p;
+  double* densePart2 = shares != nullptr ? sharesRz + F + (split > 0 ? F : 0) : h->coarse.dotPart.p + F;
+  const DenseStep ds = (withCoarse && !poseT) ? DenseStep{h->coarse.denseInv.p, h->coarse.qc.p, h->coarse.rc.p, h->coarse.c.p, densePart,
                                                h->coarse.modeActive.p, h->coarse.fail.p, split, ldsFinish + finishDoubles,
-                                               h->coarse.dotPart.p + F}
+                                               densePart2}
                                   : DenseStep{nullptr, nullptr, nullptr, nullptr, nullptr, nullptr, nullptr, kCB, 0, nullptr};
   double* fd = h->dFdot.p;
-  const TailUpdate U{h->dMinv.p, h->dDx.p, h->dR.p, h->dZ.p, fd + F, fd + 2 * F, tol2, h->coarse.modeActive.p, h->hPcg,
-                     h->dCounters.p + 1, h->dTailBar.p, h->dFdot.p + 4 * static_cast<size_t>(F) + 32, ldsFinish, ldsScratch, ds,
+  const TailUpdate U{h->dMinv.p, h->dDx.p, h->dR.p, h->dZ.p, shares != nullptr ? sharesRz : fd + F,
+                     shares != nullptr ? h->dScal.p + SH_RR : fd + 2 * F, tol2, h->coarse.modeActive.p, h->hPcg,
+                     shares != nullptr ? static_cast<unsigned int*>(nullptr) : h->dCounters.p + 1, h->dTailBar.p,
+                     h->dFdot.p + 4 * static_cast<size_t>(F) + 32, ldsFinish, ldsScratch, ds,
                      ts.Ainv != nullptr ? temporalStepDev(h) : static_cast<const TlStep*>(nullptr),
                      poseT ? poseTemporalStepDev(h) : static_cast<const TlStep*>(nullptr),
-                     (c.cross && h->xDiagRows) ? 1 : 0, h->tailStageRows ? 1 : 0};
+                     (c.cross && h->xDiagRows) ? 1 : 0, h->tailStageRows ? 1 : 0, sharesRz,
+                     shares != nullptr ? shares->levelShare0 : 0, shares != nullptr ? shares->levelWg0 : 0};
   const int grid = F + (withCoarse && !poseT && split > 0 ? (F + kDenseFramesPerGroup - 1) / kDenseFramesPerGroup : 0) +
                    (ts.Ainv != nullptr ? ts.S * ts.parts : 0) + (poseT ? kCB * tlParts(h->coarse.ptNn) : 0);
   const int slot = h->tBegin(KC_CG_UPDATE);
diff --git a/robust_cvd_amd/csrc/cvd_pcg.h b/robust_cvd_amd/csrc/cvd_pcg.h
--- a/robust_cvd_amd/csrc/cvd_pcg.h
+++ b/robust_cvd_amd/csrc/cvd_pcg.h
@@ -367,6 +367,9 @@
   __device__ bool second(double&) { return true; }
   __device__ unsigned int generation() { return 0u; }
   __device__ bool stageRows() { return false; }
+  __device__ bool closes() { return true; }
+  __device__ double* levelShare(double* fromDescriptor) { return fromDescriptor; }
+  __device__ void gaveUp() {}
 };
 __host__ __device__ inline int tlStagedLds(int NT) { return tlRowsLds(NT) + (kTlSpan + 1) * NT; }
 typedef unsigned int cvd_u32x4 __attribute__((ext_vector_type(4)));
@@ -463,7 +466,10 @@
         qT[e] = __hiloint2double(static_cast<int>(r4.z), static_cast<int>(r4.y));
       }
       __syncthreads();
-      if (*bad) return false;
+      if (*bad) {
+        mid.gaveUp();
+        return false;
+      }
     }
   }
   if (direct) {
@@ -540,7 +546,7 @@
   if (tid == 0) {
     double d = 0.0;
     for (int k = 0; k < nA; ++k) d += red[k];
-    publishPartial(ts.dotPart + wg, d);
+    storeMaybePublished(mid.levelShare(ts.dotPart + wg), d, mid.closes());
   }
   if constexpr (FUSED) TAIL_STAMP(7);
   return true;
@@ -569,6 +575,7 @@
   const bool fusedY = !init && cs.Wb != nullptr;
   const bool fusedDense = !init && ds.Ainv != nullptr;
   const int nWaves = nThreads >> 6;
+  const bool closes = mid.closes();
   const int nExtraWg = static_cast<int>(gridDim.x) - nF;
   const int bid = FUSED ? static_cast<int>(blockIdx.x)
                         : (static_cast<int>(blockIdx.x) < nExtraWg ? nF + static_cast<int>(blockIdx.x) : static_cast<int>(blockIdx.x) - nExtraWg);
@@ -641,7 +648,7 @@
       t += __shfl_xor(t, 1, 64);
       t += __shfl_xor(t, 2, 64);
       t += __shfl_xor(t, 4, 64);
-      if (tid == 0) publishPartial(dotSlot, t);
+      if (tid == 0) storeMaybePublished(dotSlot, t, closes);
     }
     __syncthreads();
   };
@@ -832,8 +839,8 @@
   if (tid == 0) {
     double a = 0.0, b = 0.0;
     for (int w = 0; w < nWaves; ++w) { a += red[w]; b += red[16 + w]; }
-    publishPartial(fdotRZ + f, a);
-    publishPartial(fdotRR + f, b);
+    storeMaybePublished(fdotRZ + f, a, closes);
+    storeMaybePublished(fdotRR + f, b, closes);
   }
   if (fusedY) {
     if (tid < kCB) {
@@ -865,6 +872,7 @@
     denseRows(f, ds.rowSplit, kCB - ds.rowSplit, qcs, psum, on0, w, false, ds.dotPart2 + f);
   }
   }
+  if (!closes) return;
   if (lastBlockArrivesLite(counter, gridDim.x, reinterpret_cast<int*>(red + 40))) {
     double a = 0.0, b = 0.0, cY = 0.0;
     for (int k = f0 + tid; k < f0 + nF; k += nThreads) {
@@ -1032,6 +1040,8 @@
   const TlStep* tp;
   int diagInProduct;
   int stageRows;
+  double* shares;
+  int levelShare0, levelWg0;
 };
 
 template <int KD>
@@ -1077,7 +1087,10 @@
   auto second = [&](double& alpha) -> bool {
     double pq;
     TAIL_STAMP(2);
-    if (!tailWait(U.gridBar, sm + U.ldsScratch, pq)) return false;
+    if (!tailWait(U.gridBar, sm + U.ldsScratch, pq)) {
+      if (U.shares != nullptr && threadIdx.x == 0) publishPartial(scal + SH_ABANDON, 1.0);
+      return false;
+    }
     TAIL_STAMP(3);
     alpha = rzOld / pq;
     if (blockIdx.x == 0 && threadIdx.x == 0) {
@@ -1095,10 +1108,41 @@
     __device__ unsigned int generation() { return *reinterpret_cast<unsigned int*>(scratch + 17); }
     bool stage;
     __device__ bool stageRows() { return stage; }
-  } mid{first, second, sm + U.ldsScratch, U.stageRows != 0};
+    double* shares;
+    double* abandonWord;
+    int levelShare0, levelWg0;
+    __device__ bool closes() { return shares == nullptr; }
+    __device__ double* levelShare(double* fromDescriptor) {
+      return shares != nullptr ? shares + levelShare0 + (static_cast<int>(blockIdx.x) - levelWg0) : fromDescriptor;
+    }
+    __device__ void gaveUp() {
+      if (shares != nullptr && threadIdx.x == 0) publishPartial(abandonWord, 1.0);
+    }
+  } mid{first, second, sm + U.ldsScratch, U.stageRows != 0, U.shares, scal + SH_ABANDON, U.levelShare0, U.levelWg0};
   cgUpdateBody<true>(L, 0, nullptr, U.minv, nullptr, nullptr, scal, U.counter, U.dx, U.r, U.z, U.fdotRZ, U.fdotRR, U.tol2, nullptr,
                      U.modeActive, U.hostMirror, csOff, U.ds, nullptr, sm, mid, 0, L.F, nullptr, U.ts, U.tp);
   TAIL_STAMP(4);
+}
+
+inline __global__ __launch_bounds__(64) void k_pcg_close(double* __restrict__ scal, int enqueued, double* __restrict__ hostMirror) {
+  const int lane = threadIdx.x;
+  double wz[8], wr[8];
+#pragma unroll
+  for (int u = 0; u < 8; ++u) {
+    wz[u] = scal[SH_RZ + lane + u * 64];
+    wr[u] = scal[SH_RR + lane + u * 64];
+  }
+  const double done0 = scal[S_DONE], abandon = scal[SH_ABANDON], old = scal[S_RZ], target = scal[S_TARGET];
+  const int applied = static_cast<int>(scal[S_ITERS]);
+  const double rz = pcgSharesSum(wz), rr = pcgSharesSum(wr);
+  if (lane != 0 || abandon != 0.0) return;
+  if (done0 == 0.0 && applied == enqueued - 1) {
+    const double done = !(rz == rz) ? 2.0 : (rz <= target ? 1.0 : 0.0);
+    pcgCloseFromShares(scal, enqueued, rz, old, (old != 0.0) ? rz / old : 0.0, done, hostMirror);
+    scal[S_RR] = rr;
+  } else if (applied >= 1) {
+    scal[S_RR] = rr;
+  }
 }
 
 inline __global__ void k_apply_step(Layout L, int boundDepth0, const double* __restrict__ x, const double* __restrict__ dx,
diff --git a/robust_cvd_amd/csrc/cvd_setup.hip b/robust_cvd_amd/csrc/cvd_setup.hip
--- a/robust_cvd_amd/csrc/cvd_setup.hip
+++ b/robust_cvd_amd/csrc/cvd_setup.hip
@@ -1171,7 +1171,8 @@
   h->dCostItem.ensure(std::max(1, c.nItems));
   h->dCostFrame.ensure(c.L.F);
   h->dFocal.ensure(static_cast<size_t>(c.L.F) * 2);
-  h->dScal.ensure(S_COUNT);
+  const bool newScal = h->dScal.p == nullptr;
+  h->dScal.ensure(SH_END);
   h->dFc.ensure(c.L.F);
   h->dFail.ensure(1);
   if (!h->dCounters.p) {
@@ -1182,6 +1183,12 @@
   if (!h->hPcg) {
     HIP_CHECK(hipHostMalloc(reinterpret_cast<void**>(&h->hPcg), 16 * sizeof(double)));
     for (auto& e : h->pcgEvent) HIP_CHECK(hipEventCreateWithFlags(&e, hipEventDisableTiming));
+  }
+  if (newScal) {
+    HIP_CHECK(hipMemsetAsync(h->dScal.p, 0, SH_END * sizeof(double), h->stream));
+    std::memcpy(h->hPcg + kPcgMirrorAddressSlot, &h->hPcg, sizeof(double*));
+    HIP_CHECK(hipMemcpyAsync(h->dScal.p + SH_MIRROR, h->hPcg + kPcgMirrorAddressSlot, sizeof(double), hipMemcpyHostToDevice, h->stream));
+    h->sharesF = h->sharesN = -1;
   }
 }
 __global__ void k_pick_median(const float* __restrict__ sorted, size_t n, int first, int count, float* __restrict__ median) {
diff --git a/robust_cvd_amd/csrc/cvd_solve.hip b/robust_cvd_amd/csrc/cvd_solve.hip
--- a/robust_cvd_amd/csrc/cvd_solve.hip
+++ b/robust_cvd_amd/csrc/cvd_solve.hip
@@ -27,6 +27,8 @@
     cvd_handle* h = c.h;
     HIP_CHECK(hipStreamSynchronize(h->stream));
     HIP_CHECK(hipMemsetAsync(h->dCounters.p, 0, 8 * sizeof(unsigned int), h->stream));
+    HIP_CHECK(hipMemsetAsync(h->dScal.p + SH_ABANDON, 0, (SH_END - SH_ABANDON) * sizeof(double), h->stream));
+    h->sharesF = h->sharesN = -1;
     if (h->temporal.counter.p) HIP_CHECK(hipMemsetAsync(h->temporal.counter.p, 0, 4 * sizeof(unsigned int), h->stream));
     if (h->dTailBar.p)
       HIP_CHECK(hipMemsetAsync(h->dTailBar.p, 0, static_cast<size_t>(kTailBarStride) * (1 + kTailBarCopies) * sizeof(unsigned int), h->stream));
@@ -123,6 +125,15 @@
     HIP_CHECK(hipMemsetAsync(h->dTailBar.p, 0, static_cast<size_t>(kTailBarStride) * (1 + kTailBarCopies) * sizeof(unsigned int), s));
     if (tsOn.rec != nullptr) HIP_CHECK(hipMemsetAsync(tsOn.rec, 0, 2 * static_cast<size_t>(tsOn.NT) * sizeof(double), s));
   }
+  PcgShares sharesLayout;
+  const bool shares = fusedTail && pcgSharesScope(c, coarse, sharesLayout);
+  h->lastShares = shares;
+  h->lastShareCount = shares ? sharesLayout.count : 0;
+  if (shares && (h->sharesF != F || h->sharesN != sharesLayout.count)) {
+    HIP_CHECK(hipMemsetAsync(h->dScal.p + SH_RZ, 0, 2 * static_cast<size_t>(kPcgSharesCap) * sizeof(double), s));
+    h->sharesF = F;
+    h->sharesN = sharesLayout.count;
+  }
   const bool ownerMode = ownerShardedUpdate(h, coarse);
   const int maxIt = std::max(1, c.h->opt.pcg_max_iterations);
   const bool lockstep = h->dbg.pcg_lockstep != 0;
@@ -131,8 +142,9 @@
   auto enqueueIteration = [&](int it, int useBeta) {
     h->curPcgIter = it;
     if (fusedTail) {
-      launchMatvec(c, x, h->dZ.p, pOld, pNew, useBeta, h->dLam.p, h->dQ.p, coarse, true);
-      launchPcgTail(c, x, pOld, pNew, useBeta, h->dLam.p, h->dQ.p, coarse, nThreads, ldsTail, ldsFinish, ldsScratch, tol2);
+      launchMatvec(c, x, h->dZ.p, pOld, pNew, useBeta, h->dLam.p, h->dQ.p, coarse, true, shares ? it : 0);
+      launchPcgTail(c, x, pOld, pNew, useBeta, h->dLam.p, h->dQ.p, coarse, nThreads, ldsTail, ldsFinish, ldsScratch, tol2,
+                    shares ? &sharesLayout : nullptr);
       std::swap(pOld, pNew);
       return;
     }
@@ -203,6 +215,7 @@
     }
   }
   h->curPcgIter = -1;
+  if (shares && enq > 0) launchPcgClose(c, enq);
   if (ownerMode) {
     const int ct = h->tBegin(KC_COMM_PRODUCT);
     const size_t chunk = static_cast<size_t>(h->ownChunk()) * B;
```

Result: faster. 357.1, median of 6 (+4.4%).
